# imkaywu/MVSKit

Hardware: AMD Instinct MI355X
Metric: patches/s (propagate+optim iteration), 12-view 1080p (higher is better)
Workload: dtype f32

## Files before the change

include/mvskit_engine.h:

```cpp
#ifndef MVSKIT_ENGINE_H
#define MVSKIT_ENGINE_H

#include <stddef.h>
#include <stdint.h>

#ifdef __cplusplus
extern "C" {
#endif

#ifndef MVS_MAX_IMAGES
#define MVS_MAX_IMAGES 32
#endif
#define MVS_LIST_CAP 16

typedef enum mvs_status {
    MVS_OK = 0,
    MVS_ERR_ARG = -1,
    MVS_ERR_STATE = -2,
    MVS_ERR_HIP = -3,
    MVS_ERR_CAPACITY = -4,
    MVS_ERR_NO_DEVICE = -5
} mvs_status;

typedef struct mvs_patch {
// ... 218 lines not shown
    int64_t neighbor_visited;
    int64_t neighbor_accepted;
    int64_t neighbor_retried;
    int64_t exchange_bytes;
} mvs_filter_stats;
int mvs_engine_filter_stats(mvs_engine* e, mvs_filter_stats* out);

int mvs_engine_pass(mvs_engine* e, int iter, int pass, mvs_counters* out);
int mvs_engine_export_counts(mvs_engine* e, int64_t* n_new, int64_t* n_kill, int32_t* per_view_new );
int mvs_engine_export_device(mvs_engine* e, void* d_new_records, int64_t cap_new, void* d_kill_ids, int64_t cap_kill);
int mvs_engine_commit_device(mvs_engine* e, const void* d_new_records, int64_t n_new, const void* d_kill_ids, int64_t n_kill);
int mvs_engine_commit_local(mvs_engine* e);

#define MVS_COMM_ID_BYTES 128
int mvs_comm_unique_id(void* id_out );
int mvs_engine_comm_init(mvs_engine* e, const void* id , int rank, int world);
int mvs_engine_comm_attach(mvs_engine* e, void* nccl_comm , int rank, int world);
int mvs_engine_comm_release(mvs_engine* e);
int mvs_engine_exchange(mvs_engine* e);
int mvs_engine_comm_info(mvs_engine* e, int* rank, int* world, int* comm_count, int* comm_rank);

int mvs_engine_depth_normal_map(mvs_engine* e, int view, int kind, float* depth, float* normal, int32_t* ids);

typedef enum mvs_probe_op {
    MVS_PROBE_NCC = 0,
    MVS_PROBE_PREPROCESS = 1,
    MVS_PROBE_REFINE = 2,
    MVS_PROBE_POSTPROCESS = 3,
    MVS_PROBE_COST = 4,
    MVS_PROBE_MATH = 5,
    MVS_PROBE_REFINE_X = 6
} mvs_probe_op;
int mvs_engine_probe(mvs_engine* e, int op, int64_t n, const mvs_patch* in_rec, const float* in_f,
                     mvs_patch* out_rec, float* out_f, int32_t* out_i);

typedef struct mvs_timing {
    float index_ms;
    float sweep_ms;
    float commit_ms;
    int32_t sweep_launches;
    float exchange_ms;
    int32_t sweep_jobs_listed;
    int64_t exchange_bytes;
    int64_t check_retried_cells;
} mvs_timing;
int mvs_engine_last_timing(mvs_engine* e, mvs_timing* t);

int mvs_engine_sweep_pairs(mvs_engine* e, int64_t out[6]);

int mvs_engine_sweep_repeats(mvs_engine* e, int64_t out[2]);

int mvs_engine_sweep_kernels(mvs_engine* e, int64_t out[2]);

#ifdef __cplusplus
}
#endif
#endif
```

mvskit_amd/csrc/mvs_device.cuh:

```cuda
#pragma once
#include <hip/hip_runtime.h>
#include <limits.h>
#include "mvs_types.h"

namespace mvsdev {

struct F3 { float x, y, z; };
struct F4 { float x, y, z, w; };

#define DEV __device__ __forceinline__

DEV int lane_id() { return (int)(threadIdx.x & 63u); }
DEV float fma_(float a, float b, float c) { return __builtin_fmaf(a, b, c); }
DEV int rli(int x, int l) { return __builtin_amdgcn_readlane(x, l); }
DEV float rlf(float x, int l) { return __int_as_float(__builtin_amdgcn_readlane(__float_as_int(x), l)); }
DEV int rfl(int x) { return __builtin_amdgcn_readfirstlane(x); }
DEV unsigned long long ballot(bool p) { return __ballot(p); }
#if MVS_LISTCAP > 32
typedef unsigned long long vmask_t;
DEV int vpop(vmask_t m) { return __popcll(m); }
#define MVS_VBITS 64
#else
typedef unsigned vmask_t;
DEV int vpop(vmask_t m) { return __popc(m); }
// ... 199 lines not shown
    const float fz = norm4(sub4(coord, ld4(vw->center)));
    const float ips = vw->ipscale;
    if (ips == 0.0f) return 1.0f;
    return div_rn(2.0f * fz * (float)(1 << prm.level), ips);
}
DEV void cell_of(const DParams& prm, const DView* vw, F4 coord, int& ix, int& iy) {
    float P[12];
    load_P(vw, prm.level, P);
    const F3 ic = project_regs(P, coord);
    ix = ((int)floorf(ic.x + 0.5f)) / prm.csize;
    iy = ((int)floorf(ic.y + 0.5f)) / prm.csize;
}
template <int LANE> DEV float row_bcast_f(float x) {
    return __int_as_float(__builtin_amdgcn_update_dpp(0, __float_as_int(x), 0x150 + LANE, 0xf, 0xf, false));
}
template <int LANE, int BANKS> DEV float row_bcast_banks_f(float old, float x) {
    return __int_as_float(__builtin_amdgcn_update_dpp(__float_as_int(old), __float_as_int(x), 0x150 + LANE, 0xf, BANKS, false));
}
template <int LANE, bool PAIR> DEV float half_bcast_f(float x) {
    if constexpr (PAIR) return row_bcast_banks_f<8 + LANE, 0xC>(row_bcast_banks_f<LANE, 0x3>(x, x), x);
    else return row_bcast_f<LANE>(x);
}
template <bool PAIR = false>
DEV void get_paxes(const DParams& prm, const DView* vw, F4 coord, F4 normal, F4& px, F4& py) {
    const F4 ctr = ld4(vw->center);
    const float ips = vw->ipscale;
    const F3 xax = ld3(vw->xaxis);
    float P[12];
    load_P(vw, prm.level, P);
    float pscale = 1.0f;
    if (ips != 0.0f) pscale = div_rn(2.0f * norm4(sub4(coord, ctr)) * (float)(1 << prm.level), ips);
    F3 n3{normal.x, normal.y, normal.z};
    F3 y3 = cross3(n3, xax);
    y3 = nrm3(y3);
    F3 x3 = cross3(y3, n3);
    px = {x3.x * pscale, x3.y * pscale, x3.z * pscale, 0.0f};
    py = {y3.x * pscale, y3.y * pscale, y3.z * pscale, 0.0f};
    const int j = lane_id() & (PAIR ? 7 : 15);
    const float a = j == 1 ? 1.0f : 0.0f, b = j == 2 ? 1.0f : 0.0f;
    const F4 X{fma_(b, py.x, fma_(a, px.x, coord.x)), fma_(b, py.y, fma_(a, px.y, coord.y)), fma_(b, py.z, fma_(a, px.z, coord.z)), coord.w};
    const F3 ic = project_regs(P, X);
    const F3 c0{half_bcast_f<0, PAIR>(ic.x), half_bcast_f<0, PAIR>(ic.y), half_bcast_f<0, PAIR>(ic.z)};
    const float inv = rcp_rn(norm3(sub3(ic, c0)));
    px = scl4(px, half_bcast_f<1, PAIR>(inv));
    py = scl4(py, half_bcast_f<2, PAIR>(inv));
}
DEV float robustincc(float incc) { return div_rn(incc, 1 + 3 * incc); }
DEV float unrobustincc(float r) { return div_rn(r, 1 - 3 * r); }

struct Frame {
    float tlx, tly, dxx, dxy, dyx, dyy;
    int w;
    int ok;
    unsigned img_lo, img_hi;
};
DEV int level_diff(const DParams& prm, float ratio) {
    static_assert(0x3504F3 == (0x3FB504F3 & 0x7FFFFF), "mantissa of 1.414213562373095f");
    const int k = ((__float_as_int(ratio) + (0x800000 - 0x3504F3)) >> 23) - 127;
    const int ld = max(-4, min(2, k));
    return max(-prm.level, min(2, ld));
}
DEV float pow2_level(int ld) { return __int_as_float((127 + ld) << 23); }
DEV Frame make_frame(const DParams& prm, F4 coord, F4 px, F4 py, F4 pz, int v, bool active) {
    const DView* vw = prm.views + (active ? v : 0);
    const F4 ctr = ld4(vw->center);
    float P[12];
#pragma unroll
    for (int k = 0; k < 12; ++k) P[k] = vw->P[prm.level][k];
    const int W0 = vw->W[0], H0 = vw->H[0];
    const unsigned long long base_level = (unsigned long long)vw->img[prm.level];
    const F4 ray = nrm4(sub4(ctr, coord));
    const float weight = fmaxf(0.0f, dot4(ray, pz));
    F3 center = project_regs(P, coord);
    F3 dx = sub3(project_regs(P, add4(coord, px)), center);
    F3 dy = sub3(project_regs(P, add4(coord, py)), center);
    const float ratio = (norm3(dx) + norm3(dy)) / 2.0f;
    const int ld = level_diff(prm, ratio);
    const float iscale = pow2_level(-ld);
    const int newLevel = prm.level + ld;
    const unsigned long long base_new = (unsigned long long)vw->img[newLevel];
    center = scl3(center, iscale);
    dx = scl3(dx, iscale);
    dy = scl3(dy, iscale);
    const float m = (float)(prm.wsize / 2);
    const float ax = dx.x * m, bx = dy.x * m, ay = dx.y * m, by = dy.y * m;
    const float tlx = (center.x - ax) - bx, tly = (center.y - ay) - by;
    const float minx = (center.x - fabsf(ax)) - fabsf(bx), maxx = (center.x + fabsf(ax)) + fabsf(bx);
    const float miny = (center.y - fabsf(ay)) - fabsf(by), maxy = (center.y + fabsf(ay)) + fabsf(by);
    const int margin2 = 2;
    const int W = W0 >> newLevel, H = H0 >> newLevel;
    const bool inside = !(minx < margin2 || W - 1 - margin2 <= maxx || miny < margin2 || H - 1 - margin2 <= maxy);
    const bool ok = active && !(weight < prm.cosAngle1) && inside;
    Frame f;
    f.tlx = ok ? tlx : 0.0f; f.tly = ok ? tly : 0.0f;
    f.dxx = ok ? dx.x : 0.0f; f.dxy = ok ? dx.y : 0.0f; f.dyx = ok ? dy.x : 0.0f; f.dyy = ok ? dy.y : 0.0f;
    f.w = ok ? W : (W0 >> prm.level);
    f.ok = ok ? 1 : 0;
    const unsigned long long a = ok ? base_new : base_level;
    f.img_lo = (unsigned)(a & 0xffffffffull); f.img_hi = (unsigned)(a >> 32);
    return f;
}

struct __attribute__((packed, aligned(4))) Texel2 { uint32_t a, b; };

struct ClsConst {
    unsigned cs[3];
    int fb;
    int xbase, nx;
    unsigned xcs;
};
struct ClsLayout { int njx, lim, xbase, nx; };
__host__ __device__ inline ClsLayout cls_layout(int wsz) {
    const int nj = wsz >> 4, rem = wsz & 15;
    return {nj + (rem > 1 ? 1 : 0), rem > 1 ? wsz : 16 * nj, 16 * nj, rem == 1 ? 1 : 0};
}
__host__ __device__ inline bool cls_full_window(int wsz) {
    const ClsLayout l = cls_layout(wsz);
    return l.njx >= 3 && l.lim >= 48 && l.nx == 1;
}
struct WaveCtx {
    int lane;
    ClsConst cc;
    unsigned evals, view_evals;
#ifdef MVS_STAGE_TIMING
    unsigned long long st_acc[8];
    unsigned long long st_t;
#endif
};
struct WaveCtxFull : WaveCtx {};
template <class WC> struct wc_full_window { static constexpr bool value = false; };
template <> struct wc_full_window<WaveCtxFull> { static constexpr bool value = true; };
#ifdef MVS_STAGE_TIMING
#define WC_T0(wc) { (wc).st_t = (unsigned long long)__builtin_amdgcn_s_memtime(); }
#define WC_ADD(wc, k) { const unsigned long long t1_ = (unsigned long long)__builtin_amdgcn_s_memtime(); (wc).st_acc[k] += t1_ - (wc).st_t; (wc).st_t = t1_; }
#else
#define WC_T0(wc)
#define WC_ADD(wc, k)
#endif

#define MVS_PIVOT_LDS4 192
#define MVS_FRAME_LDS_BYTES (64 * 48 + 16 * 16)
#define MVS_FRAME1_LDS_BYTES (48 * (MVS_LISTCAP > 16 ? MVS_LISTCAP : 16))
extern __shared__ float4 mvs_dyn_lds4[];
DEV void frames_publish(const WaveCtx& wc, const Frame& f, int nlanes) {
    __syncthreads();
    if (wc.lane < nlanes) {
        float4* d = mvs_dyn_lds4 + 3 * wc.lane;
        d[0] = make_float4(f.tlx, f.tly, f.dxx, f.dxy);
        d[1] = make_float4(f.dyx, f.dyy, __int_as_float(f.w), __int_as_float(f.ok));
        d[2] = make_float4(__int_as_float((int)f.img_lo), __int_as_float((int)f.img_hi), 0.0f, 0.0f);
    }
    __syncthreads();
}
DEV float inv_msd(const DParams& prm, float ssd) {
    float msd = sqrt_rn(ssd * prm.inv_3sz);
    if (msd == 0.0f) msd = 1.0f;
    return rcp_rn(msd);
}

struct ClsPend { Texel2 q0, q1; float dx1, dy1; };
DEV ClsConst make_cls(const DParams& prm, int lane) {
    ClsConst cc;
    const ClsLayout l = cls_layout(prm.wsz);
    const int row = lane >> 4, c = lane & 15;
    cc.fb = 16 * row;
#pragma unroll
    for (int j = 0; j < 3; ++j) {
        const int q = c + 16 * j;
        const bool valid = j < l.njx && q < l.lim;
        cc.cs[j] = valid ? (unsigned)(q % prm.wsize) | ((unsigned)(q / prm.wsize) << 8) | (1u << 16) : 0u;
    }
    cc.xbase = l.xbase; cc.nx = l.nx;
    cc.xcs = (unsigned)(l.xbase % prm.wsize) | ((unsigned)(l.xbase / prm.wsize) << 8) | (1u << 16);
    return cc;
}
DEV float cvt_ub0(unsigned x) { return (float)(x & 255u); }
DEV float cvt_ub1(unsigned x) { return (float)((x >> 8) & 255u); }
DEV float cvt_ub2(unsigned x) { return (float)((x >> 16) & 255u); }
DEV unsigned cls_opaque(unsigned x) { asm volatile("" : "+v"(x)); return x; }
struct ClsFrame { float tlx, tly, dxx, dxy, dyx, dyy; int w; unsigned long long base; };
DEV ClsFrame cls_frame(int fidx) {
    const float4* s = mvs_dyn_lds4 + 3 * fidx;
    const float4 A = s[0], B = s[1];
    const float2 Cc = *reinterpret_cast<const float2*>(s + 2);
    ClsFrame f;
    f.tlx = A.x; f.tly = A.y; f.dxx = A.z; f.dxy = A.w; f.dyx = B.x; f.dyy = B.y; f.w = __float_as_int(B.z);
    f.base = ((unsigned long long)(unsigned)__float_as_int(Cc.y) << 32) | (unsigned long long)(unsigned)__float_as_int(Cc.x);
    return f;
}
DEV ClsPend cls_issue(const ClsFrame& f, unsigned cs) {
    typedef const __attribute__((address_space(1))) uint32_t* GlobalTexels;
    const float fx = cvt_ub0(cs), fy = cvt_ub1(cs);
    const float sx = fma_(f.dyx, fy, fma_(f.dxx, fx, f.tlx));
    const float sy = fma_(f.dyy, fy, fma_(f.dxy, fx, f.tly));
    const int lx = (int)sx, ly = (int)sy;
    const unsigned long long a0 = f.base + 4ull * (unsigned long long)(unsigned)(ly * f.w + lx);
    const GlobalTexels t0 = (GlobalTexels)a0, t1 = (GlobalTexels)(a0 + 4ull * (unsigned long long)(unsigned)f.w);
    ClsPend p;
    p.q0.a = t0[0]; p.q0.b = t0[1];
    p.q1.a = t1[0]; p.q1.b = t1[1];
    p.dx1 = __builtin_amdgcn_fractf(sx); p.dy1 = __builtin_amdgcn_fractf(sy);
    return p;
}
template <bool FULL = false>
DEV void cls_colour(const ClsPend& p, unsigned cs, float pr, float pg, float pb, float& r, float& g, float& b) {
    const Texel2 q0 = p.q0, q1 = p.q1;
    const float fm = FULL ? 1.0f : cvt_ub2(cs);
    const float dx1 = FULL ? p.dx1 : p.dx1 * fm, dx0 = fm - dx1, dy1 = p.dy1, dy0 = 1.0f - dy1;
    const float f00 = dx0 * dy0, f01 = dx0 * dy1, f10 = dx1 * dy0, f11 = dx1 * dy1;
    r = fma_((float)(q1.b & 255u), f11, fma_((float)(q0.b & 255u), f10, fma_((float)(q1.a & 255u), f01, (float)(q0.a & 255u) * f00)));
    g = fma_((float)((q1.b >> 8) & 255u), f11, fma_((float)((q0.b >> 8) & 255u), f10, fma_((float)((q1.a >> 8) & 255u), f01, (float)((q0.a >> 8) & 255u) * f00)));
    b = fma_((float)((q1.b >> 16) & 255u), f11, fma_((float)((q0.b >> 16) & 255u), f10, fma_((float)((q1.a >> 16) & 255u), f01, (float)((q0.a >> 16) & 255u) * f00)));
    if (FULL) { r = r - pr; g = g - pg; b = b - pb; }
    else { r = fma_(-pr, fm, r); g = fma_(-pg, fm, g); b = fma_(-pb, fm, b); }
}
DEV float bperm_f(int addr, float x) { return __int_as_float(__builtin_amdgcn_ds_bpermute(addr, __float_as_int(x))); }
#define MVS_ROW_STEP(x, C) x = x + dpp_f<C>(x);
#define MVS_ROW_STEP5(C) { const float t0 = dpp0_f<C>(s1r), t1 = dpp0_f<C>(s1g), t2 = dpp0_f<C>(s1b), t3 = dpp0_f<C>(s2), t4 = dpp0_f<C>(s01); \
                           s1r = s1r + t0; s1g = s1g + t1; s1b = s1b + t2; s2 = s2 + t3; s01 = s01 + t4; }
#define MVS_ROW_STEP4(C) { const float t0 = dpp0_f<C>(s1r), t1 = dpp0_f<C>(s1g), t2 = dpp0_f<C>(s1b), t3 = dpp0_f<C>(s2); \
                           s1r = s1r + t0; s1g = s1g + t1; s1b = s1b + t2; s2 = s2 + t3; }
template <class WC>
DEV void eval_steps4(const DParams& prm, WC& wc, const ClsConst& cc, const Frame& f, int n, unsigned (&okm)[4], float& incc_l) {
    constexpr bool FULL = wc_full_window<WC>::value;
    const bool has_x = cc.nx > 0;
    frames_publish(wc, f, 64);
    const unsigned long long okb = ballot(f.ok != 0);
#pragma unroll
    for (int g = 0; g < 4; ++g) okm[g] = (unsigned)((okb >> (16 * g)) & 0xffffull);
#pragma unroll
    for (int g = 0; g < 4; ++g) wc.view_evals += (okm[g] & 1u) ? (unsigned)__popc(okm[g]) : 0u;
    const int fb = cc.fb;
    const int lc = wc.lane & 15;
    float c0[3][3];
    ClsPend pend[3];
    float P1r, P1g, P1b, P2, P01 = 0.0f;
    const int vlast = max(n - 1, 0);
    {
        const ClsFrame fr = cls_frame(fb);
#pragma unroll
        for (int j = 0; j < 3; ++j) pend[j] = cls_issue(fr, cls_opaque(cc.cs[j]));
    }
    {
        const float4 pv = mvs_dyn_lds4[MVS_PIVOT_LDS4];
        const ClsFrame fn = cls_frame(fb + min(1, vlast));
        float s1r = 0.0f, s1g = 0.0f, s1b = 0.0f, s2 = 0.0f;
#pragma unroll
        for (int j = 0; j < 3; ++j) {
            const unsigned cs = cls_opaque(cc.cs[j]);
            float r, g, b;
            cls_colour<FULL>(pend[j], cs, pv.x, pv.y, pv.z, r, g, b);
            pend[j] = cls_issue(fn, cs);
            c0[j][0] = r; c0[j][1] = g; c0[j][2] = b;
            s1r += r; s1g += g; s1b += b;
            s2 = fma_(r, r, s2); s2 = fma_(g, g, s2); s2 = fma_(b, b, s2);
        }
        MVS_ROW_STEP4(0xB1) MVS_ROW_STEP4(0x4E) MVS_ROW_STEP4(0x141) MVS_ROW_STEP4(0x140)
        P1r = s1r; P1g = s1g; P1b = s1b; P2 = s2;
    }
    for (int k = 1; k < n; ++k) {
        const float4 pv = mvs_dyn_lds4[MVS_PIVOT_LDS4 + k];
        const ClsFrame fn = cls_frame(fb + min(k + 1, vlast));
        float s1r = 0.0f, s1g = 0.0f, s1b = 0.0f, s2 = 0.0f, s01 = 0.0f;
#pragma unroll
        for (int j = 0; j < 3; ++j) {
            const unsigned cs = cls_opaque(cc.cs[j]);
            float r, g, b;
            cls_colour<FULL>(pend[j], cs, pv.x, pv.y, pv.z, r, g, b);
            pend[j] = cls_issue(fn, cs);
            s1r += r; s1g += g; s1b += b;
            s2 = fma_(r, r, s2); s2 = fma_(g, g, s2); s2 = fma_(b, b, s2);
            s01 = fma_(r, c0[j][0], s01); s01 = fma_(g, c0[j][1], s01); s01 = fma_(b, c0[j][2], s01);
        }
        MVS_ROW_STEP5(0xB1) MVS_ROW_STEP5(0x4E) MVS_ROW_STEP5(0x141) MVS_ROW_STEP5(0x140)
        if (lc == k) { P1r = s1r; P1g = s1g; P1b = s1b; P2 = s2; P01 = s01; }
    }
    const int a0 = (wc.lane & 48) << 2;
    if (has_x) {
        const float4 pv = mvs_dyn_lds4[MVS_PIVOT_LDS4 + lc];
        ClsFrame fr;
        fr.tlx = f.tlx; fr.tly = f.tly; fr.dxx = f.dxx; fr.dxy = f.dxy; fr.dyx = f.dyx; fr.dyy = f.dyy; fr.w = f.w;
        fr.base = ((unsigned long long)f.img_hi << 32) | (unsigned long long)f.img_lo;
        {
            const unsigned cs = cc.xcs;
            const ClsPend pe = cls_issue(fr, cs);
            float r, g, b;
            cls_colour<FULL>(pe, cs, pv.x, pv.y, pv.z, r, g, b);
            const float r0 = bperm_f(a0, r), g0 = bperm_f(a0, g), b0 = bperm_f(a0, b);
            P1r += r; P1g += g; P1b += b;
            P2 = fma_(r, r, P2); P2 = fma_(g, g, P2); P2 = fma_(b, b, P2);
            P01 = fma_(r, r0, P01); P01 = fma_(g, g0, P01); P01 = fma_(b, b0, P01);
        }
    }
    const float m_r = P1r * prm.inv_sz, m_g = P1g * prm.inv_sz, m_b = P1b * prm.inv_sz;
    const float ssd = fmaxf(P2 - fma_(P1b, m_b, fma_(P1g, m_g, P1r * m_r)), 0.0f);
    const float inv_l = inv_msd(prm, ssd);
    const float m0r = bperm_f(a0, m_r), m0g = bperm_f(a0, m_g), m0b = bperm_f(a0, m_b), inv0 = bperm_f(a0, inv_l);
    const float dot = P01 - fma_(P1b, m0b, fma_(P1g, m0g, P1r * m0r));
    incc_l = 1.0f - (dot * (inv0 * inv_l)) * prm.inv_3sz;
}

template <class WC>
DEV unsigned long long eval_steps4_pair(const DParams& prm, WC& wc, const ClsConst& cc, const Frame& f, int n0, int n1, unsigned (&okm)[2][4], float& incc_l) {
    constexpr bool FULL = wc_full_window<WC>::value;
    const bool has_x = FULL || cc.nx > 0;
    frames_publish(wc, f, 64);
    const unsigned long long okb = ballot(f.ok != 0);
#pragma unroll
    for (int g = 0; g < 4; ++g) { okm[0][g] = (unsigned)((okb >> (16 * g)) & 0xffull); okm[1][g] = (unsigned)((okb >> (16 * g + 8)) & 0xffull); }
#pragma unroll
    for (int g = 0; g < 4; ++g)
        wc.view_evals += ((okm[0][g] & 1u) ? (unsigned)__popc(okm[0][g]) : 0u) + ((okm[1][g] & 1u) ? (unsigned)__popc(okm[1][g]) : 0u);
    const int lc = wc.lane & 15;
    float P1r = 0.0f, P1g = 0.0f, P1b = 0.0f, P2 = 0.0f, P01 = 0.0f;
#pragma nounroll
    for (int s = 0; s < 2; ++s) {
        const int n = s ? n1 : n0;
        const int fb = cc.fb + 8 * s, pb = MVS_PIVOT_LDS4 + 8 * s, lb = 8 * s;
        float c0[3][3];
        ClsPend pend[3];
        const int vlast = max(n - 1, 0);
        {
            const ClsFrame fr = cls_frame(fb);
#pragma unroll
            for (int j = 0; j < 3; ++j) pend[j] = cls_issue(fr, cls_opaque(cc.cs[j]));
        }
        {
            const float4 pv = mvs_dyn_lds4[pb];
            const ClsFrame fn = cls_frame(fb + min(1, vlast));
            float s1r = 0.0f, s1g = 0.0f, s1b = 0.0f, s2 = 0.0f;
#pragma unroll
            for (int j = 0; j < 3; ++j) {
                const unsigned cs = cls_opaque(cc.cs[j]);
                float r, g, b;
                cls_colour<FULL>(pend[j], cs, pv.x, pv.y, pv.z, r, g, b);
                pend[j] = cls_issue(fn, cs);
                c0[j][0] = r; c0[j][1] = g; c0[j][2] = b;
                s1r += r; s1g += g; s1b += b;
                s2 = fma_(r, r, s2); s2 = fma_(g, g, s2); s2 = fma_(b, b, s2);
            }
            MVS_ROW_STEP4(0xB1) MVS_ROW_STEP4(0x4E) MVS_ROW_STEP4(0x141) MVS_ROW_STEP4(0x140)
            if (lc >= lb) { P1r = s1r; P1g = s1g; P1b = s1b; P2 = s2; }
        }
        for (int k = 1; k < n; ++k) {
            const float4 pv = mvs_dyn_lds4[pb + k];
            const ClsFrame fn = cls_frame(fb + min(k + 1, vlast));
            float s1r = 0.0f, s1g = 0.0f, s1b = 0.0f, s2 = 0.0f, s01 = 0.0f;
#pragma unroll
            for (int j = 0; j < 3; ++j) {
                const unsigned cs = cls_opaque(cc.cs[j]);
                float r, g, b;
                cls_colour<FULL>(pend[j], cs, pv.x, pv.y, pv.z, r, g, b);
                pend[j] = cls_issue(fn, cs);
                s1r += r; s1g += g; s1b += b;
                s2 = fma_(r, r, s2); s2 = fma_(g, g, s2); s2 = fma_(b, b, s2);
                s01 = fma_(r, c0[j][0], s01); s01 = fma_(g, c0[j][1], s01); s01 = fma_(b, c0[j][2], s01);
            }
            MVS_ROW_STEP5(0xB1) MVS_ROW_STEP5(0x4E) MVS_ROW_STEP5(0x141) MVS_ROW_STEP5(0x140)
            if (lc == lb + k) { P1r = s1r; P1g = s1g; P1b = s1b; P2 = s2; P01 = s01; }
        }
    }
    const int a0 = (wc.lane & 56) << 2;
    if (has_x) {
        const float4 pv = mvs_dyn_lds4[MVS_PIVOT_LDS4 + lc];
        ClsFrame fr;
        fr.tlx = f.tlx; fr.tly = f.tly; fr.dxx = f.dxx; fr.dxy = f.dxy; fr.dyx = f.dyx; fr.dyy = f.dyy; fr.w = f.w;
        fr.base = ((unsigned long long)f.img_hi << 32) | (unsigned long long)f.img_lo;
        {
            const unsigned cs = cc.xcs;
            const ClsPend pe = cls_issue(fr, cs);
            float r, g, b;
            cls_colour<FULL>(pe, cs, pv.x, pv.y, pv.z, r, g, b);
            const float r0 = bperm_f(a0, r), g0 = bperm_f(a0, g), b0 = bperm_f(a0, b);
            P1r += r; P1g += g; P1b += b;
            P2 = fma_(r, r, P2); P2 = fma_(g, g, P2); P2 = fma_(b, b, P2);
            P01 = fma_(r, r0, P01); P01 = fma_(g, g0, P01); P01 = fma_(b, b0, P01);
        }
    }
    const float m_r = P1r * prm.inv_sz, m_g = P1g * prm.inv_sz, m_b = P1b * prm.inv_sz;
    const float ssd = fmaxf(P2 - fma_(P1b, m_b, fma_(P1g, m_g, P1r * m_r)), 0.0f);
    const float inv_l = inv_msd(prm, ssd);
    const float m0r = bperm_f(a0, m_r), m0g = bperm_f(a0, m_g), m0b = bperm_f(a0, m_b), inv0 = bperm_f(a0, inv_l);
    const float dot = P01 - fma_(P1b, m0b, fma_(P1g, m0g, P1r * m0r));
    incc_l = 1.0f - (dot * (inv0 * inv_l)) * prm.inv_3sz;
    return okb;
}

template <bool FULL = false>
DEV void cls_raw(const ClsPend& p, unsigned cs, float& r, float& g, float& b) {
    const Texel2 q0 = p.q0, q1 = p.q1;
    const float fm = FULL ? 1.0f : cvt_ub2(cs);
    const float dx1 = FULL ? p.dx1 : p.dx1 * fm, dx0 = fm - dx1, dy1 = p.dy1, dy0 = 1.0f - dy1;
    const float f00 = dx0 * dy0, f01 = dx0 * dy1, f10 = dx1 * dy0, f11 = dx1 * dy1;
    r = fma_((float)(q1.b & 255u), f11, fma_((float)(q0.b & 255u), f10, fma_((float)(q1.a & 255u), f01, (float)(q0.a & 255u) * f00)));
    g = fma_((float)((q1.b >> 8) & 255u), f11, fma_((float)((q0.b >> 8) & 255u), f10, fma_((float)((q1.a >> 8) & 255u), f01, (float)((q0.a >> 8) & 255u) * f00)));
    b = fma_((float)((q1.b >> 16) & 255u), f11, fma_((float)((q0.b >> 16) & 255u), f10, fma_((float)((q1.a >> 16) & 255u), f01, (float)((q0.a >> 16) & 255u) * f00)));
}
#define MVS_ROW_STEP3(C) { const float t0 = dpp0_f<C>(s1r), t1 = dpp0_f<C>(s1g), t2 = dpp0_f<C>(s1b); s1r = s1r + t0; s1g = s1g + t1; s1b = s1b + t2; }
#define MVS_ROW_STEP2(C) { const float t0 = dpp0_f<C>(sq), t1 = dpp0_f<C>(dt); sq = sq + t0; dt = dt + t1; }

#define MVS_PAIR_MFMA (MVS_LISTCAP > 16)
#if MVS_PAIR_MFMA
#define MVS_GRAM_SCRATCH (MVS_LISTCAP > 32 ? 2 : 1)
#define MVS_GRAM_CH 16
#define MVS_GRAM_NCH (MVS_LISTCAP / 16)
#define MVS_GRAM_NT (MVS_GRAM_NCH * (MVS_GRAM_NCH + 1) / 2)
#define MVS_GRAM_KSP 40
#define MVS_GRAM_T(p, c) ((c) * ((c) + 1) / 2 + (p))
#define MVS_GRAM_KK 4
#define MVS_GRAM_KS ((147 + MVS_GRAM_KK - 1) / MVS_GRAM_KK)
#define MVS_GRAM_NACC 4
typedef float gram_acc_t __attribute__((ext_vector_type(MVS_GRAM_NACC)));
DEV gram_acc_t gram_mfma(float a, float b, gram_acc_t c) { return __builtin_amdgcn_mfma_f32_16x16x4f32(a, b, c, 0, 0, 0); }
DEV int gram_col(int lane) { return lane & 15; }
DEV int gram_row(int lane, int r) { return (lane >> 4) * 4 + r; }
template <int N> struct GramIC { static constexpr int value = N; };
#endif
template <bool PIV = false, class WC>
DEV void eval_views(const DParams& prm, WC& wc, const Frame& f, int n, vmask_t (&okm)[1], float& incc_l, float* piv = nullptr,
                    float* texs = nullptr, int tstride = 0, float* ssd_out = nullptr) {
#if MVS_PAIR_MFMA
#if MVS_GRAM_SCRATCH == 2
    float gops[MVS_GRAM_NCH * MVS_GRAM_KSP];
#elif MVS_GRAM_SCRATCH
    gram_acc_t gacc[MVS_GRAM_NT];
    float gops[(MVS_GRAM_NCH - 1) * MVS_GRAM_KSP];
#pragma unroll
    for (int q = 0; q < MVS_GRAM_NT; ++q)
#pragma unroll
        for (int r = 0; r < MVS_GRAM_NACC; ++r) gacc[q][r] = 0.0f;
#endif
    const int gK = 3 * prm.wsz, gtp = 3 * tstride;
    const int gk0 = wc.lane / MVS_GRAM_CH;
    const float* const grow = texs + (wc.lane & (MVS_GRAM_CH - 1)) * gtp;
#endif
    constexpr bool FULL = wc_full_window<WC>::value;
    const ClsConst& cc = wc.cc;
    const bool has_x = FULL || cc.nx > 0;
    frames_publish(wc, f, MVS_LISTCAP > 16 ? MVS_LISTCAP : 16);
    okm[0] = vballot(f.ok != 0);
    wc.view_evals += (okm[0] & 1u) ? (unsigned)vpop(okm[0]) : 0u;
    const int row = wc.lane >> 4, lc = wc.lane & 15;
    float fxr = 0.0f, fxg = 0.0f, fxb = 0.0f;
    unsigned xcs = 0u;
    ClsPend pe;
    if (has_x) {
        ClsFrame fr;
        fr.tlx = f.tlx; fr.tly = f.tly; fr.dxx = f.dxx; fr.dxy = f.dxy; fr.dyx = f.dyx; fr.dyy = f.dyy; fr.w = f.w;
        fr.base = ((unsigned long long)f.img_hi << 32) | (unsigned long long)f.img_lo;
        xcs = cc.xcs;
        pe = cls_issue(fr, xcs);
    }
    float d0[3][3], d0x[3] = {0.0f, 0.0f, 0.0f};
    float ssd_l = 1.0f, dot_l = 0.0f, mr_l = 128.0f, mg_l = 128.0f, mb_l = 128.0f;
    ClsPend pend[3];
    {
        const int last = max(n - 1, 0);
        const ClsFrame fr = cls_frame(min(row, last));
#pragma unroll
        for (int j = 0; j < 3; ++j) pend[j] = cls_issue(fr, cls_opaque(cc.cs[j]));
    }
    if (has_x) cls_raw<FULL>(pe, xcs, fxr, fxg, fxb);
    const int rounds = (n + 3) >> 2;
    auto round_body = [&](const int t) {
        const int v = 4 * t + row, vq = min(v, max(n - 1, 0));
        const ClsFrame fn = cls_frame(min(v + 4, max(n - 1, 0)));
        float cr[3], cg[3], cb[3];
        float s1r = 0.0f, s1g = 0.0f, s1b = 0.0f;
#pragma unroll
        for (int j = 0; j < 3; ++j) {
            const unsigned cs = cls_opaque(cc.cs[j]);
            cls_raw<FULL>(pend[j], cs, cr[j], cg[j], cb[j]);
            pend[j] = cls_issue(fn, cs);
            s1r += cr[j]; s1g += cg[j]; s1b += cb[j];
        }
        MVS_ROW_STEP3(0xB1) MVS_ROW_STEP3(0x4E) MVS_ROW_STEP3(0x141) MVS_ROW_STEP3(0x140)
        float xr = 0.0f, xg = 0.0f, xb = 0.0f;
        if (has_x) {
            xr = bperm_f(4 * vq, fxr); xg = bperm_f(4 * vq, fxg); xb = bperm_f(4 * vq, fxb);
            s1r += xr; s1g += xg; s1b += xb;
        }
        const float mr = s1r * prm.inv_sz, mg = s1g * prm.inv_sz, mb = s1b * prm.inv_sz;
        float er[3], eg[3], eb[3];
#pragma unroll
        for (int j = 0; j < 3; ++j) {
            if (FULL) { er[j] = cr[j] - mr; eg[j] = cg[j] - mg; eb[j] = cb[j] - mb; }
            else {
                const float fm = cvt_ub2(cls_opaque(cc.cs[j]));
                er[j] = fma_(-mr, fm, cr[j]); eg[j] = fma_(-mg, fm, cg[j]); eb[j] = fma_(-mb, fm, cb[j]);
            }
        }
        const float exr = xr - mr, exg = xg - mg, exb = xb - mb;
        if (t == 0) {
            const int a0 = 4 * lc;
#pragma unroll
            for (int j = 0; j < 3; ++j) { d0[j][0] = bperm_f(a0, er[j]); d0[j][1] = bperm_f(a0, eg[j]); d0[j][2] = bperm_f(a0, eb[j]); }
            if (has_x) { d0x[0] = bperm_f(0, exr); d0x[1] = bperm_f(0, exg); d0x[2] = bperm_f(0, exb); }
        }
        float sq = 0.0f, dt = 0.0f;
#pragma unroll
        for (int j = 0; j < 3; ++j) {
            sq += fma_(eb[j], eb[j], fma_(eg[j], eg[j], er[j] * er[j]));
            dt += fma_(d0[j][2], eb[j], fma_(d0[j][1], eg[j], d0[j][0] * er[j]));
        }
        MVS_ROW_STEP2(0xB1) MVS_ROW_STEP2(0x4E) MVS_ROW_STEP2(0x141) MVS_ROW_STEP2(0x140)
        if (has_x) {
            sq += fma_(exb, exb, fma_(exg, exg, exr * exr));
            dt += fma_(d0x[2], exb, fma_(d0x[1], exg, d0x[0] * exr));
        }
        if (lc == t) { ssd_l = sq; dot_l = dt; if (PIV) { mr_l = mr; mg_l = mg; mb_l = mb; } }
#if MVS_PAIR_MFMA
        if (texs) {
            float* tv = texs + (3 * (v & (MVS_GRAM_CH - 1))) * tstride;
            const bool have = v < n;
#pragma unroll
            for (int j = 0; j < 3; ++j)
                if (cc.cs[j] >> 16) { const int q = 3 * (lc + 16 * j); tv[q] = have ? er[j] : 0.0f; tv[q + 1] = have ? eg[j] : 0.0f; tv[q + 2] = have ? eb[j] : 0.0f; }
            if (has_x && lc == 0) { tv[3 * cc.xbase] = have ? exr : 0.0f; tv[3 * cc.xbase + 1] = have ? exg : 0.0f; tv[3 * cc.xbase + 2] = have ? exb : 0.0f; }
        }
#else
        if (texs && v < n) {
            float* tv = texs + (3 * v) * tstride;
#pragma unroll
            for (int j = 0; j < 3; ++j)
                if (cc.cs[j] >> 16) { const int q = 3 * (lc + 16 * j); tv[q] = er[j]; tv[q + 1] = eg[j]; tv[q + 2] = eb[j]; }
            if (has_x && lc == 0) { tv[3 * cc.xbase] = exr; tv[3 * cc.xbase + 1] = exg; tv[3 * cc.xbase + 2] = exb; }
// ... 126 lines not shown
        for (int t = 0; t < rounds; ++t) round_body(t);
#else
    for (int t = 0; t < rounds; ++t) round_body(t);
#endif
    const float inv_l = inv_msd(prm, ssd_l);
    const float inv0 = rlf(inv_l, 0);
    const float incc_v = 1.0f - (dot_l * (inv0 * inv_l)) * prm.inv_3sz;
    const int src = 4 * (16 * (wc.lane & 3) + ((wc.lane >> 2) & 15));
    incc_l = bperm_f(src, incc_v);
    if (ssd_out) *ssd_out = bperm_f(src, ssd_l);
    if (PIV) {
        const bool okk = (okm[0] >> (wc.lane & (MVS_VBITS - 1))) & 1u;
        const float a0 = bperm_f(src, mr_l), a1 = bperm_f(src, mg_l), a2 = bperm_f(src, mb_l);
        piv[0] = (wc.lane < MVS_VBITS && okk) ? a0 : 128.0f; piv[1] = (wc.lane < MVS_VBITS && okk) ? a1 : 128.0f; piv[2] = (wc.lane < MVS_VBITS && okk) ? a2 : 128.0f;
    }
}

struct Cand {
    F4 coord, normal;
    float ncc, dscale, ascale, tmp;
    int nimg, nvimg;
    int img, gx, gy;
    int vimg, vgx, vgy;
};

DEV float compute_weights(const DParams& prm, const WaveCtx& wc, F4 coord, F4 normal, int img, int n) {
    float unit = 1.0f;
    {
        const DView* vw = prm.views + (wc.lane < n ? img : 0);
        const F4 ctr = ld4(vw->center);
        const float ips = vw->ipscale;
        const F4 dc = sub4(coord, ctr);
        float u = 1.0f;
        if (ips != 0.0f) u = div_rn(2.0f * norm4(dc) * (float)(1 << prm.level), ips);
        const F4 ray = nrm4(sub4(ctr, coord));
        const float d = dot4(ray, normal);
        u = (0.0f < d) ? div_rn(u, d) : (float)(INT_MAX / 2);
        if (wc.lane < n) unit = u;
    }
    const float w0 = rlf(unit, 0);
    float w = fminf(1.0f, div_rn(w0, unit));
    if (wc.lane == 0) w = 1.0f;
    return w;
}

template <class WC>
DEV float compute_incc(const DParams& prm, WC& wc, F4 coord, F4 normal, int img, int n, float weights, int robust) {
    if (n < 2) return 2.0f;
    const int ref = rli(img, 0);
    F4 px, py;
    get_paxes(prm, prm.views + ref, coord, normal, px, py);
    const int sz = min(prm.tau, n);
    wc.evals++;
    const Frame f = make_frame(prm, coord, px, py, normal, img, wc.lane < sz);
    vmask_t okm[1];
    float incc_l;
    eval_views(prm, wc, f, sz, okm, incc_l);
    if (!(okm[0] & 1u)) return 2.0f;
    const float val_l = robust ? robustincc(incc_l) : incc_l;
    float score = 0.0f, total = 0.0f;
    for (int i = 1; i < sz; ++i) {
        if (!((okm[0] >> i) & 1u)) continue;
        const float w = rlf(weights, i);
        total += w;
        score += rlf(val_l, i) * w;
    }
    if (total == 0.0f) return 2.0f;
    return div_rn(score, total);
}
DEV float weighted_incc(const DParams& prm, vmask_t okm, float val_l, float weights, int n) {
    if (n < 2 || !(okm & 1u)) return 2.0f;
    const int sz = min(prm.tau, n);
    float score = 0.0f, total = 0.0f;
    for (int i = 1; i < sz; ++i) {
        if (!((okm >> i) & 1u)) continue;
        const float w = rlf(weights, i);
        total += w;
        score += rlf(val_l, i) * w;
    }
    if (total == 0.0f) return 2.0f;
    return div_rn(score, total);
}
template <class WC>
DEV float compute_ncc(const DParams& prm, WC& wc, F4 coord, F4 normal, int img, int n) {
    const float w = compute_weights(prm, wc, coord, normal, img, n);
    return 1.0f - unrobustincc(compute_incc(prm, wc, coord, normal, img, n, w, 1));
}

template <class WC>
DEV float set_inccs(const DParams& prm, WC& wc, F4 coord, F4 normal, int img, int n, int robust, vmask_t* okm_out = nullptr,
                    float* texs = nullptr, int tstride = 0, float* ssd_out = nullptr) {
    const int ref = rli(img, 0);
    F4 px, py;
    get_paxes(prm, prm.views + ref, coord, normal, px, py);
    wc.evals++;
    const Frame f = make_frame(prm, coord, px, py, normal, img, wc.lane < n);
    vmask_t okm[1];
    float incc_l;
    eval_views(prm, wc, f, n, okm, incc_l, nullptr, texs, tstride, ssd_out);
    if (okm_out) *okm_out = okm[0];
    if (!(okm[0] & 1u)) return 2.0f;
    float incc = robust ? robustincc(incc_l) : incc_l;
    if (wc.lane >= MVS_LISTCAP || !((okm[0] >> (wc.lane & (MVS_VBITS - 1))) & 1u)) incc = 2.0f;
    if (wc.lane == 0) incc = 0.0f;
    return incc;
}

DEV int compact1(int* scratch, const WaveCtx& wc, bool keep, int& a) {
    const unsigned long long m = ballot(keep);
    const int pos = __popcll(m & ((1ull << wc.lane) - 1ull));
    __syncthreads();
    if (keep) scratch[pos] = a;
    __syncthreads();
    a = scratch[wc.lane];
    return __popcll(m);
}

DEV void add_images(const DParams& prm, const WaveCtx& wc, int* scratch, Cand& c) {
    const int ref = rli(c.img, 0);
    bool visib = false;
    for (int j = 0; j < c.nimg; ++j) visib |= (rli(c.img, j) == wc.lane);
    bool q = false;
    if (wc.lane < prm.nviews && wc.lane != ref && !visib) {
        const DView* vw = prm.views + wc.lane;
        float P[12];
        load_P(vw, prm.level, P);
        const int W = vw->W[prm.level], H = vw->H[prm.level];
        const F4 ctr = ld4(vw->center);
        const F3 ic = project_regs(P, c.coord);
        const F4 ray = nrm4(sub4(ctr, c.coord));
        q = !(ic.x < 0.0f || W - 1 <= ic.x || ic.y < 0.0f || H - 1 <= ic.y) && prm.cosAngle0 <= dot4(ray, c.normal);
    }
    const unsigned long long m = ballot(q);
    const int pos = c.nimg + __popcll(m & ((1ull << wc.lane) - 1ull));
    __syncthreads();
    if (wc.lane < c.nimg) scratch[wc.lane] = c.img;
    if (q && pos < MVS_LISTCAP) scratch[pos] = wc.lane;
    __syncthreads();
    c.nimg = min(MVS_LISTCAP, c.nimg + (int)__popcll(m));
    c.img = scratch[wc.lane];
}

struct KeptTex {
    float* texs; int tstride;
    float ssd;
    vmask_t okm;
    int orig;
    int n_eval;
};
// ... 118 lines not shown
    if (cosb == 0.0f) a1 = 0.0f;
    else {
        const float sina = fx / cosb, cosa = -fz / cosb;
        a1 = pm_acosf(fmaxf(-1.0f, fminf(1.0f, cosa)));
        if (sina < 0.0f) a1 = -a1;
    }
    x[1] = a1 / rc.ascale;
    x[2] = a2 / rc.ascale;
}
DEV void decode(const DParams& prm, const RefineCtx& rc, float x0, float x1, float x2, F4& coord, F4& normal) {
    const float t = rc.dscale * x0;
    coord = {fma_(t, rc.ray.x, rc.center.x), fma_(t, rc.ray.y, rc.center.y), fma_(t, rc.ray.z, rc.center.z), fma_(t, rc.ray.w, rc.center.w)};
    const float angle1 = x1 * rc.ascale, angle2 = x2 * rc.ascale;
    float s1, c1, s2, c2;
    pm_sincosf(angle1, s1, c1);
    pm_sincosf(angle2, s2, c2);
    const float fx = s1 * c2, fy = s2, fz = -c1 * c2;
    const DView* vw = prm.views + rc.ref;
    normal = {fma_(vw->zaxis[0], fz, fma_(vw->yaxis[0], fy, vw->xaxis[0] * fx)),
              fma_(vw->zaxis[1], fz, fma_(vw->yaxis[1], fy, vw->xaxis[1] * fx)),
              fma_(vw->zaxis[2], fz, fma_(vw->yaxis[2], fy, vw->xaxis[2] * fx)), 0.0f};
}
DEV void sum_of_group(const WaveCtx& wc, unsigned okm, float val_l, int g, int sz, double& ans, int& denom) {
    ans = 0.0;
    denom = 0;
    for (int i = 1; i < sz; ++i) {
        if (!((okm >> i) & 1u)) continue;
        ans += (double)rlf(val_l, 16 * g + i);
        denom++;
    }
}
DEV double rld(double x, int l) {
    const long long b = __double_as_longlong(x);
    const unsigned lo = (unsigned)rli((int)(b & 0xffffffffll), l), hi = (unsigned)rli((int)(b >> 32), l);
    return __longlong_as_double((long long)(((unsigned long long)hi << 32) | lo));
}
DEV double cost_of_group(const DParams& prm, const WaveCtx& wc, unsigned okm, float val_l, int g, int sz, int minimum) {
    if (!(okm & 1u)) return 2.0;
    double ans;
    int denom;
    sum_of_group(wc, okm, val_l, g, sz, ans, denom);
    if (denom < minimum - 1) return 2.0;
    return ans / (double)denom;
}
template <class WC>
DEV void cost_func4(const DParams& prm, WC& wc, const RefineCtx& rc, int imgx, int n, bool four, float x0, float x1, float x2,
                    double (&fv)[4], float* piv = nullptr, const ClsConst* cc = nullptr, unsigned rows = 0xFu) {
    F4 coord, normal, px, py;
    decode(prm, rc, x0, x1, x2, coord, normal);
    get_paxes(prm, prm.views + rc.ref, coord, normal, px, py);
    const int sz = min(prm.tau, n);
    const int minimum = min(prm.minImageNum, sz);
    const int g = wc.lane >> 4, i = wc.lane & 15;
    const Frame f = make_frame(prm, coord, px, py, normal, imgx, (four ? ((rows >> g) & 1u) != 0u : g < 1) && i < sz);
    float incc_l;
    fv[1] = fv[2] = fv[3] = 2.0;
    if (four) {
        wc.evals += (unsigned)__popc(rows);
        unsigned okm[4];
        eval_steps4(prm, wc, *cc, f, sz, okm, incc_l);
        const float val_l = robustincc(incc_l);
        const int gl = wc.lane & 3;
        const unsigned okl = gl == 1 ? okm[1] : (gl == 2 ? okm[2] : (gl == 3 ? okm[3] : okm[0]));
        double num = 0.0;
        int den = 0;
        for (int i = 1; i < sz; ++i) {
            const float v = bperm_f(4 * (16 * gl + i), val_l);
            const bool ok = (okl >> i) & 1u;
            num = ok ? num + (double)v : num;
            den += ok ? 1 : 0;
        }
        const double q = num / (double)den;
#pragma unroll
        for (int j = 0; j < 4; ++j) fv[j] = ((okm[j] & 1u) && rli(den, j) >= minimum - 1) ? rld(q, j) : 2.0;
    } else {
        wc.evals += 1;
        vmask_t okm[1];
        if (piv) eval_views<true>(prm, wc, f, sz, okm, incc_l, piv);
        else eval_views(prm, wc, f, sz, okm, incc_l);
        const float val_l = robustincc(incc_l);
        fv[0] = cost_of_group(prm, wc, (unsigned)okm[0], val_l, 0, sz, minimum);
    }
}
template <class WC>
DEV void refine_patch(const DParams& prm, WC& wc, Cand& c, uint32_t k0, uint32_t k1, uint32_t k2, uint32_t k3, float* w_out = nullptr) {
    RefineCtx rc;
    rc.center = c.coord;
    rc.ref = rli(c.img, 0);
    rc.ray = nrm4(sub4(c.coord, ld4((prm.views + rc.ref)->center)));
    rc.dscale = c.dscale;
    rc.ascale = prm.ascaleConst;
    const float w = compute_weights(prm, wc, c.coord, c.normal, c.img, c.nimg);
    const int imgx = __shfl(c.img, wc.lane & 15);
    float x[3];
    encode(prm, rc, c.coord, c.normal, x);
    const float amin = -23.99999f, amax = 23.99999f;
    x[1] = fmaxf(fminf(x[1], amax), amin);
    x[2] = fmaxf(fminf(x[2], amax), amin);
    float bx0 = x[0], bx1 = x[1], bx2 = x[2];
    double fv[4];
    float piv[3] = {128.0f, 128.0f, 128.0f};
    cost_func4(prm, wc, rc, imgx, c.nimg, false, bx0, bx1, bx2, fv, piv);
    __syncthreads();
    if (wc.lane < 16) mvs_dyn_lds4[MVS_PIVOT_LDS4 + wc.lane] = make_float4(piv[0], piv[1], piv[2], 0.0f);
    __syncthreads();
    double fbest = fv[0];
    const ClsConst cc = wc.cc;
// ... 15 lines not shown
        }
        cost_func4(prm, wc, rc, imgx, c.nimg, true, cx0, cx1, cx2, fv, nullptr, &cc);
        int jb = 0;
        double fstep = fv[0];
#pragma unroll
        for (int j = 1; j < 4; ++j) if (fv[j] < fstep) { fstep = fv[j]; jb = j; }
        if (fstep < fbest) { fbest = fstep; bx0 = rlf(cx0, 16 * jb); bx1 = rlf(cx1, 16 * jb); bx2 = rlf(cx2, 16 * jb); }
        rd *= 0.5f; ra *= 0.5f;
    }
    x[0] = bx0; x[1] = bx1; x[2] = bx2;
    decode(prm, rc, x[0], x[1], x[2], c.coord, c.normal);
    c.normal.w = 0.0f;
    if (w_out) *w_out = w;
    else c.ncc = 1.0f - unrobustincc(compute_incc(prm, wc, c.coord, c.normal, c.img, c.nimg, w, 1));
}

#define MVS_PEND_IMG 16
#define MVS_PEND_GX 80
#define MVS_PEND_GY 144
#define MVS_PEND_W 208
#define MVS_PEND_CTX 272
#define MVS_PEND_XIMG 304
#define MVS_PEND_INTS 320
DEV float rff(float x) { return __int_as_float(rfl(__float_as_int(x))); }
DEV void pend_store(int* st, const WaveCtx& wc, const Cand& c, float w) {
    __syncthreads();
    if (wc.lane == 0) {
        float* f = reinterpret_cast<float*>(st);
        f[0] = c.coord.x; f[1] = c.coord.y; f[2] = c.coord.z; f[3] = c.coord.w;
        f[4] = c.normal.x; f[5] = c.normal.y; f[6] = c.normal.z; f[7] = c.normal.w;
        f[8] = c.ncc; f[9] = c.dscale; f[10] = c.ascale; f[11] = c.tmp;
        st[12] = c.nimg; st[13] = c.nvimg;
    }
    st[MVS_PEND_IMG + wc.lane] = c.img; st[MVS_PEND_GX + wc.lane] = c.gx; st[MVS_PEND_GY + wc.lane] = c.gy;
    st[MVS_PEND_W + wc.lane] = __float_as_int(w);
    __syncthreads();
}
DEV void pend_load(const int* st, const WaveCtx& wc, Cand& c, float& w) {
    const float* f = reinterpret_cast<const float*>(st);
    c.coord = {rff(f[0]), rff(f[1]), rff(f[2]), rff(f[3])};
    c.normal = {rff(f[4]), rff(f[5]), rff(f[6]), rff(f[7])};
    c.ncc = rff(f[8]); c.dscale = rff(f[9]); c.ascale = rff(f[10]); c.tmp = rff(f[11]);
    c.nimg = rfl(st[12]); c.nvimg = rfl(st[13]);
    c.img = st[MVS_PEND_IMG + wc.lane]; c.gx = st[MVS_PEND_GX + wc.lane]; c.gy = st[MVS_PEND_GY + wc.lane];
    c.vimg = 0; c.vgx = 0; c.vgy = 0;
    w = __int_as_float(st[MVS_PEND_W + wc.lane]);
}
template <class WC>
DEV void cost_func4_pair(const DParams& prm, WC& wc, const RefineCtx& rc, int imgx, int sz0, int sz1, int szl, float x0, float x1, float x2,
                         double (&fv)[2][4], const ClsConst& cc) {
    F4 coord, normal, px, py;
    decode(prm, rc, x0, x1, x2, coord, normal);
    get_paxes<true>(prm, prm.views + rc.ref, coord, normal, px, py);
    const Frame f = make_frame(prm, coord, px, py, normal, imgx, (wc.lane & 7) < szl);
    wc.evals += 8u;
    unsigned okm[2][4];
    float incc_l;
    const unsigned long long okb = eval_steps4_pair(prm, wc, cc, f, sz0, sz1, okm, incc_l);
    const float val_l = robustincc(incc_l);
    const int src = (int)(((cls_opaque((unsigned)wc.lane) & 3u) << 4) | ((cls_opaque((unsigned)wc.lane) & 4u) << 1));
    const unsigned okl = (unsigned)(okb >> src) & 0xffu;
    double num = 0.0;
    int den = 0;
    const int szm = max(sz0, sz1);
    for (int i = 1; i < szm; ++i) {
        const float v = bperm_f(4 * (src + i), val_l);
        const bool ok = (okl >> i) & 1u;
        num = ok ? num + (double)v : num;
        den += ok ? 1 : 0;
    }
    const double q = num / (double)den;
    const int min0 = min(prm.minImageNum, sz0), min1 = min(prm.minImageNum, sz1);
#pragma unroll
    for (int j = 0; j < 4; ++j) {
        fv[0][j] = ((okm[0][j] & 1u) && rli(den, j) >= min0 - 1) ? rld(q, j) : 2.0;
        fv[1][j] = ((okm[1][j] & 1u) && rli(den, 4 + j) >= min1 - 1) ? rld(q, 4 + j) : 2.0;
    }
}
template <class WC>
DEV void refine_patch_pair(const DParams& prm, WC& wc, int* st, Cand& c1, uint32_t k0, uint32_t k1, uint32_t k2, uint32_t k3a, uint32_t k3b, float& w1) {
    float* const ctx = reinterpret_cast<float*>(st + MVS_PEND_CTX);
    int* const ximg = st + MVS_PEND_XIMG;
    const float amin = -23.99999f, amax = 23.99999f;
    double fbest0 = 2.0, fbest1 = 2.0;
    int sz0 = 0, sz1 = 0;
    w1 = 0.0f;
#pragma nounroll
    for (int s = 0; s < 2; ++s) {
        F4 coord = c1.coord, normal = c1.normal;
        float dscale = c1.dscale;
        int img = c1.img, nimg = c1.nimg;
        if (s == 0) {
            const float* f = reinterpret_cast<const float*>(st);
            coord = {rff(f[0]), rff(f[1]), rff(f[2]), rff(f[3])};
            normal = {rff(f[4]), rff(f[5]), rff(f[6]), rff(f[7])};
            dscale = rff(f[9]); nimg = rfl(st[12]);
            img = st[MVS_PEND_IMG + wc.lane];
        }
        RefineCtx rc;
        rc.center = coord;
        rc.ref = rli(img, 0);
        rc.ray = nrm4(sub4(coord, ld4((prm.views + rc.ref)->center)));
        rc.dscale = dscale;
        rc.ascale = prm.ascaleConst;
        const float w = compute_weights(prm, wc, coord, normal, img, nimg);
        if (s == 0) st[MVS_PEND_W + wc.lane] = __float_as_int(w);
        else w1 = w;
// ... 179 lines not shown
        cost_func4(prm, wc, rc, imgx, c.nimg, true, vx0, vx1, vx2, fv, nullptr, &cc, 0xFu & ~(1u << b));
        evals += 3;
        if (g != b) vf = g == 0 ? fv[0] : (g == 1 ? fv[1] : (g == 2 ? fv[2] : fv[3]));
    }
    const float xb0 = rlf(vx0, 16 * b), xb1 = rlf(vx1, 16 * b), xb2 = rlf(vx2, 16 * b);
    if (x_out) { x_out[0] = xb0; x_out[1] = xb1; x_out[2] = xb2; }
    if (f_out) *f_out = rld(vf, 16 * b);
    if (ok) {
        decode(prm, rc, xb0, xb1, xb2, c.coord, c.normal);
        c.normal.w = 0.0f;
        if (!w_out) c.ncc = 1.0f - unrobustincc(compute_incc(prm, wc, c.coord, c.normal, c.img, c.nimg, w, 1));
    }
    if (w_out) *w_out = w;
    return ok ? evals : -evals;
}

DEV void filter_images_by_angle(const DParams& prm, const WaveCtx& wc, int* scratch, Cand& c, KeptTex* kt = nullptr) {
    bool bad = false;
    if (wc.lane < c.nimg) {
        const F4 ray = nrm4(sub4(ld4((prm.views + c.img)->center), c.coord));
        bad = dot4(ray, c.normal) < prm.cosAngle1;
    }
    const unsigned long long bm = ballot(bad);
    if (bm & 1ull) { c.nimg = 0; return; }
    if (kt) (void)compact1(scratch, wc, wc.lane < c.nimg && !bad, kt->orig);
    c.nimg = compact1(scratch, wc, wc.lane < c.nimg && !bad, c.img);
}
DEV void set_grids(const DParams& prm, const WaveCtx& wc, Cand& c) {
    c.gx = 0; c.gy = 0;
    if (wc.lane < c.nimg) cell_of(prm, prm.views + c.img, c.coord, c.gx, c.gy);
}
DEV int pair_index(int a, int b, int n) { return a * (2 * n - a - 1) / 2 + (b - a - 1); }
template <class WC>
DEV void set_ref_image(const DParams& prm, WC& wc, float* texs, int tstride, Cand& c, const KeptTex* kt = nullptr, const Frame* pre = nullptr) {
    if (c.nimg == 0) return;
    const int n = c.nimg;
    const int ref = rli(c.img, 0);
    WC_T0(wc)
    vmask_t okmask = 0;
    float ssd_l = 1.0f;
    int orig = wc.lane;
    if (kt) {
        texs = kt->texs;
        orig = wc.lane < n ? kt->orig : 0;
        ssd_l = __shfl(kt->ssd, orig);
        okmask = vballot(wc.lane < n && ((kt->okm >> orig) & 1u));
        __syncthreads();
    } else {
    Frame f;
    if (pre) f = *pre;
    else {
        F4 px, py;
        get_paxes(prm, prm.views + ref, c.coord, c.normal, px, py);
        f = make_frame(prm, c.coord, px, py, c.normal, c.img, wc.lane < n);
    }
    wc.evals++;
    WC_ADD(wc, 1)
    texs += MVS_FRAME1_LDS_BYTES / 4;
    vmask_t okm1[1];
    float incc_unused;
    eval_views(prm, wc, f, n, okm1, incc_unused, nullptr, texs, tstride, &ssd_l);
    okmask = okm1[0];
    if (!(okmask & 1u)) wc.view_evals += (unsigned)vpop(okmask);
    }
    const float inv_l = inv_msd(prm, ssd_l);
    WC_ADD(wc, 2)
    __syncthreads();
#if !MVS_PAIR_MFMA
    const int npairs = n * (n - 1) / 2;
    float* pairv = texs + prm.list_n * 3 * tstride;
#endif
#if MVS_PAIR_MFMA
    {
        const int MVS_GRAM_LD = prm.gram_ld;
        const int ne = kt ? kt->n_eval : n;
        const float inv_e = kt ? inv_msd(prm, kt->ssd) : inv_l;
        const vmask_t ok_e = kt ? kt->okm : okmask;
        const bool okb = wc.lane < ne && ((ok_e >> (wc.lane & (MVS_VBITS - 1))) & 1u);
        for (int a = 0; a + 1 < ne; ++a) {
            const float inva = rlf(inv_e, a);
            const bool oka = (ok_e >> a) & 1u;
            if (wc.lane > a && wc.lane < ne) {
                float val = robustincc(1.0f - (texs[a * MVS_GRAM_LD + wc.lane] * (inva * inv_e)) * prm.inv_3sz);
                if (!(oka && okb)) val = 2.0f;
                texs[a * MVS_GRAM_LD + wc.lane] = val;
                texs[wc.lane * MVS_GRAM_LD + a] = val;
            }
        }
    }
#else
    for (int r = 0; r * 64 < npairs; ++r) {
        const int q0 = wc.lane + 64 * r;
        int q = q0;
        const bool act = q < npairs;
        int a = 0;
        if (act) { while (q >= n - 1 - a) { q -= n - 1 - a; ++a; } }
        const int b = act ? a + 1 + q : 1;
        const float* ta = texs + (__shfl(orig, a) * 3) * tstride;
        const float* tb = texs + (__shfl(orig, b) * 3) * tstride;
        float acc = 0.0f;
        for (int i = 0; i < 3 * prm.wsz; i += 3) {
            acc = fma_(ta[i], tb[i], acc); acc = fma_(ta[i + 1], tb[i + 1], acc); acc = fma_(ta[i + 2], tb[i + 2], acc);
        }
        const float inva = __shfl(inv_l, a), invb = __shfl(inv_l, b);
        float val = robustincc(1.0f - (acc * (inva * invb)) * prm.inv_3sz);
        if (!(act && ((okmask >> a) & 1u) && ((okmask >> b) & 1u))) val = 2.0f;
        if (act) pairv[q0] = val;
// ... 178 lines not shown
```

mvskit_amd/csrc/mvs_engine.cpp:

```cpp
#include <dlfcn.h>

#include <cmath>
#include <cstring>

#include "mvs_engine_impl.h"

using namespace mvseng;

static_assert(sizeof(mvs_patch) == sizeof(DPatch), "mvs_patch and DPatch must be the same bytes");
static_assert((MVS_LISTCAP == 16 || MVS_LISTCAP == 32 || MVS_LISTCAP == 64) && MVS_LISTCAP <= MVS_MAXI && MVS_MAX_IMAGES == MVS_MAXI, "limits out of sync");

namespace mvseng {

thread_local std::string g_err;

Roctx& roctx() {
    static Roctx r;
    static bool tried = false;
    if (tried) return r;
    tried = true;
    void* h = nullptr;
    const char* names[] = {"libroctx64.so", "libroctx64.so.4", "/opt/rocm/lib/libroctx64.so.4"};
    for (const char* n : names) if (!h) h = dlopen(n, RTLD_NOW | RTLD_NOLOAD);
    for (const char* n : names) if (!h) h = dlopen(n, RTLD_NOW | RTLD_LOCAL);
    if (!h) return r;
    r.push = reinterpret_cast<int (*)(const char*)>(dlsym(h, "roctxRangePushA"));
    r.pop = reinterpret_cast<int (*)()>(dlsym(h, "roctxRangePop"));
    if (!r.push || !r.pop) { r.push = nullptr; r.pop = nullptr; }
    return r;
}

RefineSel refine_sel(const mvs_engine* e) {
    return RefineSel{e->refiner.mode == MVS_REFINE_CONVERGED ? 1 : 0, e->refiner.max_evals, e->refiner.xtol};
}

DParams current_params(mvs_engine* e) {
    DParams p = e->prm;
    p.views = e->dviews.p;
    p.pool = e->pool.p;
    p.pool_n = e->pool_n;
    p.total_cells = e->total_cells;
    p.csr_start = e->start.p; p.csr_cnt = e->cnt_alive.p; p.csr_key = e->key.p; p.csr_id32 = e->id32.p;
    p.vcsr_start = e->vstart.p; p.vcsr_cnt = e->vcnt_alive.p; p.vcsr_id32 = e->vid32.p;
    p.dpgrid = e->dpgrid.p;
    p.geo = e->geo_valid ? e->geo.p : nullptr;
    p.geo_ref = e->geo_valid ? e->geo_ref.p : nullptr;
    return p;
}

bool want_vgrid(const mvs_engine* e) { return e->prm.depth >= 2 && e->prm.enable_check; }

int need_state(const mvs_engine* e, Need need, const char* who) {
    if (!e) { g_err = std::string(who) + ": no engine"; return MVS_ERR_ARG; }
    if (need >= NEED_VIEWS && !e->have_views) { g_err = std::string(who) + ": views not set"; return MVS_ERR_STATE; }
    if (need >= NEED_IDLE && e->staged) { g_err = std::string(who) + ": a pass is waiting for its commit"; return MVS_ERR_STATE; }
    return MVS_OK;
}

int scan_total(mvs_engine* e, const int32_t* flags, int32_t* base, int32_t* scan, int64_t n, int64_t* count) {
    mvsk_exclusive_scan(flags, base, n, scan, e->stream);
    int32_t total = 0;
    if (int r = read_back(e, base + n, &total)) return r;
    HIPCHK(hipGetLastError());
    *count = total;
    return MVS_OK;
}

}

namespace {

void derive_params(mvs_engine* e) {
    const mvs_config& c = e->cfg;
    DParams& p = e->prm;
    p.nviews = c.nviews; p.level = c.level; p.csize = c.csize; p.wsize = c.wsize; p.wsz = c.wsize * c.wsize;
    p.minImageNum = c.minImageNum;
    p.tau = std::min(c.minImageNum * 2, c.nviews);
    p.max_propag = c.max_propag;
    p.cap = c.max_propag * c.csize * c.csize;
    p.depth = c.depth; p.enable_check = c.enable_check; p.view_propagation = c.view_propagation ? 1 : 0;
    p.seed = c.seed; p.refine_steps = c.refine_steps; p.rd0 = c.refine_rd0; p.ra0 = c.refine_ra0;
    p.nccThreshold = c.nccThreshold;
    p.nccThresholdBefore = c.nccThreshold - 0.3f;
    volatile float a0 = (float)(60.0f * M_PI / 180.0f), a1 = (float)(60.0f * M_PI / 180.0f);
    volatile double amin = (double)c.maxAngleThreshold, amax = (double)a1;
    volatile float typo = (float)(120.0f / M_PI * 180.0f);
    volatile double d120 = 120.0f * M_PI / 180.0f, d10 = 10.0f * M_PI / 180.0f;
    p.cosAngle0 = cosf(a0);
    p.cosAngle1 = cosf(a1);
    p.cosMinAngle = (float)cos(amin);
    p.cosMaxAngle = (float)cos(amax);
// ... 90 lines not shown
void mvs_default_config(mvs_config* c) {
    memset(c, 0, sizeof *c);
    c->level = 1; c->csize = 2; c->wsize = 7; c->minImageNum = 3; c->max_propag = 2;
    c->nccThreshold = 0.7f; c->maxAngleThreshold = (float)(10.0f * M_PI / 180.0f); c->quadThreshold = 2.5f;
    c->depth = 1; c->seed = 1; c->refine_steps = 6; c->refine_rd0 = 4.0f; c->refine_ra0 = 4.0f; c->enable_check = 1;
    c->view_begin = 0; c->view_stride = 1; c->device = 0; c->max_patches = 0;
}

int mvs_engine_create(const mvs_config* cfg, mvs_engine** out) {
    if (!cfg || !out) { g_err = "mvs_engine_create: null argument"; return MVS_ERR_ARG; }
    if (cfg->shard_count > 1 && (cfg->shard_index < 0 || cfg->shard_index >= cfg->shard_count)) { g_err = "mvs_engine_create: bad shard_index"; return MVS_ERR_ARG; }
    if (cfg->nviews < 1 || cfg->nviews > MVS_MAXVIEWS || cfg->wsize < 1 || cfg->wsize > 7 || cfg->csize < 1 || cfg->level < 0 ||
        cfg->level > 4 || cfg->max_propag < 1 || cfg->max_propag > 16 || cfg->max_propag * cfg->csize * cfg->csize > MVS_CAPMAX ||
        cfg->view_stride < 1 || cfg->view_begin < 0 || cfg->minImageNum < 1 ||
        std::min(cfg->minImageNum * 2, cfg->nviews) > 16 ) {
        g_err = "mvs_engine_create: configuration out of range (nviews <= 64, wsize <= 7, min(2 minImageNum, nviews) <= 16, max_propag*csize^2 <= 32)";
        return MVS_ERR_ARG;
    }
    int ndev = 0;
    if (hipGetDeviceCount(&ndev) != hipSuccess || ndev < 1) { g_err = "mvs_engine_create: no HIP device (the engine has no CPU path)"; return MVS_ERR_NO_DEVICE; }
    if (cfg->device < 0 || cfg->device >= ndev) { g_err = "mvs_engine_create: bad device ordinal"; return MVS_ERR_ARG; }
    HIPCHK(hipSetDevice(cfg->device));
    mvs_engine* e = new mvs_engine();
    e->cfg = *cfg;
    derive_params(e);
    hipError_t he = hipStreamCreate(&e->stream);
    if (he != hipSuccess) { g_err = std::string("hipStreamCreate: ") + hipGetErrorString(he); delete e; return MVS_ERR_HIP; }
    for (auto& ev : e->ev) (void)hipEventCreate(&ev);
    for (auto& ev : e->fev) (void)hipEventCreate(&ev);
    if (e->misc.ensure(misc::words) || e->counters.ensure(MVS_COUNTER_SLOTS) || e->error_flag.ensure(1)) { delete e; return MVS_ERR_HIP; }
    (void)hipMemset(e->misc.p, 0, misc::words * sizeof(unsigned long long));
    (void)hipMemset(e->error_flag.p, 0, sizeof(int32_t));
    *out = e;
    return MVS_OK;
}

int mvs_engine_destroy(mvs_engine* e) {
    if (!e) return MVS_OK;
    (void)hipSetDevice(e->cfg.device);
    (void)hipStreamSynchronize(e->stream);
    (void)mvs_engine_comm_release(e);
    for (auto& ev : e->ev) if (ev) (void)hipEventDestroy(ev);
    for (auto& ev : e->fev) if (ev) (void)hipEventDestroy(ev);
    (void)hipStreamDestroy(e->stream);
    delete e;
    return MVS_OK;
}

int mvs_engine_set_views(mvs_engine* e, int nviews, const mvs_view_desc* views) {
    if (!e || !views || nviews != e->cfg.nviews) { g_err = "mvs_engine_set_views: nviews must equal the configured number of views"; return MVS_ERR_ARG; }
    HIPCHK(hipSetDevice(e->cfg.device));
    hipStream_t st = e->stream;
    Range rg("mvs:set_views (upload + pyramids)");
    e->img_bufs.clear(); e->mask_bufs.clear();
    e->have_views = false;
    const int maxLevel = e->cfg.level + 3;
    e->hviews.assign(nviews, DView{});
    int cell_base = 0;
    size_t max_bytes = 0;
    for (int v = 0; v < nviews; ++v) {
        if (views[v].width < 8 || views[v].height < 8 || !views[v].rgb) { g_err = "mvs_engine_set_views: bad view"; return MVS_ERR_ARG; }
        max_bytes = std::max(max_bytes, (size_t)views[v].width * views[v].height * 3);
    }
    if (int r = e->tmp_bytes.ensure((int64_t)max_bytes)) return r;
    for (int v = 0; v < nviews; ++v) {
        DView& vw = e->hviews[v];
        vw.W[0] = views[v].width; vw.H[0] = views[v].height;
        for (int l = 1; l < maxLevel; ++l) { vw.W[l] = vw.W[l - 1] / 2; vw.H[l] = vw.H[l - 1] / 2; }
        setup_camera(e, vw, views[v].P);
        const size_t n0 = (size_t)vw.W[0] * vw.H[0];
        HIPCHK(hipMemcpyAsync(e->tmp_bytes.p, views[v].rgb, n0 * 3, hipMemcpyHostToDevice, st));
        for (int l = 0; l < maxLevel; ++l) {
            e->img_bufs.emplace_back();
            if (int r = e->img_bufs.back().ensure(std::max<int64_t>((int64_t)vw.W[l] * vw.H[l], 1))) return r;
            uint32_t* buf = e->img_bufs.back().p;
            vw.img[l] = buf;
            if (l == 0) mvsk_rgb_to_rgba(e->tmp_bytes.p, buf, (int64_t)n0, st);
            else mvsk_pyr_down(vw.img[l - 1], vw.W[l - 1], vw.H[l - 1], buf, vw.W[l], vw.H[l], st);
        }
        vw.mask = nullptr;
        if (views[v].mask) {
            HIPCHK(hipStreamSynchronize(st));
            uint8_t* prev = nullptr;
            for (int l = 0; l <= e->cfg.level; ++l) {
                e->mask_bufs.emplace_back();
                if (int r = e->mask_bufs.back().ensure(std::max<int64_t>((int64_t)vw.W[l] * vw.H[l], 1))) return r;
                uint8_t* m = e->mask_bufs.back().p;
                if (l == 0) {
                    HIPCHK(hipMemcpyAsync(m, views[v].mask, n0, hipMemcpyHostToDevice, st));
                    mvsk_mask_binarise(m, (int64_t)n0, st);
                } else mvsk_mask_down(prev, vw.W[l - 1], vw.H[l - 1], m, vw.W[l], vw.H[l], st);
                prev = m;
            }
            vw.mask = prev;
        }
        HIPCHK(hipStreamSynchronize(st));
        vw.gh = (vw.H[e->cfg.level] + e->cfg.csize - 1) / e->cfg.csize;
        vw.gw = (vw.W[e->cfg.level] + e->cfg.csize - 1) / e->cfg.csize;
        vw.cell_base = cell_base;
        cell_base += vw.gw * vw.gh;
    }
    e->total_cells = cell_base;
    if (int r = e->dviews.ensure(nviews)) return r;
    HIPCHK(hipMemcpyAsync(e->dviews.p, e->hviews.data(), sizeof(DView) * nviews, hipMemcpyHostToDevice, st));
    const int64_t nc = e->total_cells;
    if (e->cnt.ensure(nc + 2) || e->start.ensure(nc + 2) || e->cursor.ensure(nc + 2) || e->vcnt.ensure(nc + 2) || e->vstart.ensure(nc + 2) ||
        e->vcursor.ensure(nc + 2) || e->start_raw.ensure(nc + 2) || e->dpgrid.ensure(nc + 2) || e->best.ensure(nc + 2) || e->cnt_alive.ensure(nc + 2) || e->vcnt_alive.ensure(nc + 2))
        return MVS_ERR_HIP;
    int64_t pool_cap = e->cfg.max_patches > 0 ? e->cfg.max_patches : 4 * nc;
    if (e->cfg.max_patches <= 0) {
        size_t free_b = 0, total_b = 0;
        if (hipMemGetInfo(&free_b, &total_b) == hipSuccess && total_b > 0) {
            pool_cap = std::max<int64_t>(std::min<int64_t>(pool_cap, (int64_t)(total_b / 6 / sizeof(DPatch))), std::min<int64_t>(pool_cap, nc));
            const double per_patch = 2.5 * (double)sizeof(DPatch) + 17.0;
            const int64_t fit = (int64_t)(0.6 * (double)free_b / per_patch);
            if (fit < pool_cap) pool_cap = std::max<int64_t>(fit, std::min<int64_t>(pool_cap, nc / 4 + 1024));
        }
    }
    e->ids.headroom = e->key.headroom = e->id32.headroom = e->id32_raw.headroom = e->vid32.headroom = true;
    e->geo.headroom = e->geo_ref.headroom = true;
    if (e->pool.ensure(pool_cap) || e->pool_alt.ensure(pool_cap) || e->kill.ensure(pool_cap) || e->kill_cnt.ensure(pool_cap + 2) || e->kill_base.ensure(pool_cap + 2)) return MVS_ERR_HIP;
    HIPCHK(hipMemsetAsync(e->kill.p, 0, (size_t)pool_cap, st));
    int64_t njobs_max = 0;
    for (int v = 0; v < nviews; ++v) njobs_max += (int64_t)((e->hviews[v].gw + 1) / 2) * e->hviews[v].gh;
    const int maxstage = (e->prm.view_propagation ? 3 : 2) * e->prm.cap * e->prm.max_propag;
    if (e->job_stage.ensure(njobs_max * maxstage) || e->job_nstage.ensure(njobs_max + 2) || e->job_cnt.ensure(njobs_max + misc::job_list_pad) ||
        e->job_base_scan.ensure(njobs_max + misc::job_list_pad) || e->job_list.ensure(std::max<int64_t>(njobs_max, 16)))
        return MVS_ERR_HIP;
    const int64_t scan_n = std::max<int64_t>(std::max<int64_t>(nc, pool_cap), njobs_max);
// ... 88 lines not shown
        return MVS_OK;
    };
    if (take(e->ids, n + 16) || take(e->key, n + 16) || take(e->id32, n + 16) || take(e->id32_raw, n + 16) || take(e->vid32, n + 16)) return MVS_ERR_HIP;
    HIPCHK(hipStreamSynchronize(e->stream));
    return MVS_OK;
}

int mvs_engine_clear_patches(mvs_engine* e) {
    if (!e) return MVS_ERR_ARG;
    HIPCHK(hipSetDevice(e->cfg.device));
    if (e->kill.p) HIPCHK(hipMemsetAsync(e->kill.p, 0, (size_t)e->kill.cap, e->stream));
    e->pool_n = 0; e->staged = false; e->counted = false;
    return MVS_OK;
}

int mvs_engine_num_patches(mvs_engine* e, int64_t* n_alive) {
    if (!e || !n_alive) return MVS_ERR_ARG;
    HIPCHK(hipSetDevice(e->cfg.device));
    return count_pool(e, Count::alive, n_alive);
}

int mvs_engine_download_patches(mvs_engine* e, int64_t cap, mvs_patch* out, int64_t* n) {
    if (!e || !n) return MVS_ERR_ARG;
    int64_t alive = 0;
    if (int r = mvs_engine_num_patches(e, &alive)) return r;
    *n = alive;
    if (!out || alive == 0) return MVS_OK;
    const int64_t m = std::min(cap, alive);
    if (int r = e->tmp_rec_out.ensure(alive)) return r;
    mvsk_alive_gather(e->pool.p, e->pool_n, e->kill_base.p, e->tmp_rec_out.p, alive, e->stream);
    HIPCHK(hipMemcpyAsync(out, e->tmp_rec_out.p, (size_t)m * sizeof(mvs_patch), hipMemcpyDeviceToHost, e->stream));
    HIPCHK(hipStreamSynchronize(e->stream));
    return MVS_OK;
}

int mvs_engine_sweep_pairs(mvs_engine* e, int64_t out[6]) {
    if (!e || !out) return MVS_ERR_ARG;
    for (int k = 0; k < 6; ++k) out[k] = e->sweep_pairs[k];
    return MVS_OK;
}

int mvs_engine_sweep_repeats(mvs_engine* e, int64_t out[2]) {
    if (!e || !out) return MVS_ERR_ARG;
    for (int k = 0; k < 2; ++k) out[k] = e->sweep_repeats[k];
    return MVS_OK;
}

int mvs_engine_sweep_kernels(mvs_engine* e, int64_t out[2]) {
    if (!e || !out) return MVS_ERR_ARG;
    for (int k = 0; k < 2; ++k) out[k] = e->sweep_kernels[k];
    return MVS_OK;
}

int mvs_engine_last_timing(mvs_engine* e, mvs_timing* t) {
    if (!e || !t) return MVS_ERR_ARG;
    *t = e->timing;
    return MVS_OK;
}

int mvs_engine_depth_normal_map(mvs_engine* e, int view, int kind, float* depth, float* normal, int32_t* ids) {
    if (!e || !e->have_views || view < 0 || view >= e->cfg.nviews || kind < 0 || kind > 1) { g_err = "mvs_engine_depth_normal_map: bad argument"; return MVS_ERR_ARG; }
    HIPCHK(hipSetDevice(e->cfg.device));
    hipStream_t st = e->stream;
    const DView& vw = e->hviews[view];
    const int ncells = vw.gw * vw.gh;
    const DParams p = current_params(e);
    const unsigned long long* sel = nullptr;
    if (kind == 0) {
        HIPCHK(hipMemsetAsync(e->dpgrid.p, 0xff, (size_t)e->total_cells * sizeof(unsigned long long), st));
        mvsk_depth_maps(p, e->dpgrid.p, nullptr, st);
        sel = e->dpgrid.p + vw.cell_base;
    } else {
        HIPCHK(hipMemsetAsync(e->best.p, 0, (size_t)ncells * sizeof(unsigned long long), st));
        mvsk_best_ncc_map(p, view, e->best.p, st);
        sel = e->best.p;
    }
    if (e->tmp_f_out.ensure((int64_t)ncells * 4) || e->tmp_i.ensure(ncells)) return MVS_ERR_HIP;
    mvsk_map_extract(p, view, kind, sel, e->tmp_f_out.p, e->tmp_f_out.p + ncells, e->tmp_i.p, ncells, st);
    if (depth) HIPCHK(hipMemcpyAsync(depth, e->tmp_f_out.p, (size_t)ncells * sizeof(float), hipMemcpyDeviceToHost, st));
    if (normal) HIPCHK(hipMemcpyAsync(normal, e->tmp_f_out.p + ncells, (size_t)ncells * 3 * sizeof(float), hipMemcpyDeviceToHost, st));
    if (ids) HIPCHK(hipMemcpyAsync(ids, e->tmp_i.p, (size_t)ncells * sizeof(int32_t), hipMemcpyDeviceToHost, st));
    HIPCHK(hipStreamSynchronize(st));
    return MVS_OK;
}

int mvs_engine_probe(mvs_engine* e, int op, int64_t n, const mvs_patch* in_rec, const float* in_f, mvs_patch* out_rec, float* out_f, int32_t* out_i) {
    if (!e || !e->have_views || n < 0 || op < 0 || op > 6) { g_err = "mvs_engine_probe: bad argument / views not set"; return MVS_ERR_ARG; }
    const RefineSel rs = refine_sel(e);
    if (op == MVS_PROBE_REFINE_X && !rs.simplex) { g_err = "mvs_engine_probe: MVS_PROBE_REFINE_X needs the CONVERGED refiner"; return MVS_ERR_STATE; }
    if (n == 0) return MVS_OK;
    HIPCHK(hipSetDevice(e->cfg.device));
    hipStream_t st = e->stream;
    if (op == MVS_PROBE_POSTPROCESS && e->prm.depth > 0) if (int r = build_index(e, nullptr)) return r;
    const int64_t nf_out = op == MVS_PROBE_MATH ? 5 * n : ((op == MVS_PROBE_REFINE || op == MVS_PROBE_REFINE_X) && rs.simplex ? 4 * n : n);
    if (e->tmp_rec_in.ensure(n) || e->tmp_rec_out.ensure(n) || e->tmp_f_in.ensure(n) || e->tmp_f_out.ensure(nf_out) || e->tmp_i.ensure(n + 1)) return MVS_ERR_HIP;
    if (op == MVS_PROBE_MATH) {
        if (!in_f || !out_f) return MVS_ERR_ARG;
        HIPCHK(hipMemcpyAsync(e->tmp_f_in.p, in_f, (size_t)n * sizeof(float), hipMemcpyHostToDevice, st));
    } else {
        if (!in_rec) return MVS_ERR_ARG;
        HIPCHK(hipMemcpyAsync(e->tmp_rec_in.p, in_rec, (size_t)n * sizeof(mvs_patch), hipMemcpyHostToDevice, st));
    }
    HIPCHK(hipMemsetAsync(e->tmp_i.p, 0, (size_t)(n + 1) * sizeof(int32_t), st));
    const DParams p = current_params(e);
    mvsk_probe(p, op, n, e->tmp_rec_in.p, e->tmp_f_in.p, e->tmp_rec_out.p, e->tmp_f_out.p, e->tmp_i.p, rs, st);
    if (out_rec && (op == MVS_PROBE_PREPROCESS || op == MVS_PROBE_REFINE || op == MVS_PROBE_POSTPROCESS || op == MVS_PROBE_REFINE_X))
        HIPCHK(hipMemcpyAsync(out_rec, e->tmp_rec_out.p, (size_t)n * sizeof(mvs_patch), hipMemcpyDeviceToHost, st));
    if (out_f && (op == MVS_PROBE_NCC || op == MVS_PROBE_COST || op == MVS_PROBE_MATH || op == MVS_PROBE_REFINE_X))
        HIPCHK(hipMemcpyAsync(out_f, e->tmp_f_out.p, (size_t)nf_out * sizeof(float), hipMemcpyDeviceToHost, st));
    if (out_i) HIPCHK(hipMemcpyAsync(out_i, e->tmp_i.p, (size_t)n * sizeof(int32_t), hipMemcpyDeviceToHost, st));
    HIPCHK(hipStreamSynchronize(st));
    HIPCHK(hipGetLastError());
    return MVS_OK;
}

}
```

mvskit_amd/csrc/mvs_engine_impl.h:

```cpp
#pragma once
#include <hip/hip_runtime.h>
#include <rccl/rccl.h>

#include <algorithm>
#include <cstdint>
#include <string>
#include <vector>

#include "mvskit_engine.h"
#include "mvs_kernels.h"
#include "mvs_types.h"

namespace mvseng {
extern thread_local std::string g_err;
}

#define HIPCHK(expr)                                                                                       \
    do {                                                                                                   \
        hipError_t _e = (expr);                                                                            \
        if (_e != hipSuccess) {                                                                            \
            mvseng::g_err = std::string(#expr) + ": " + hipGetErrorString(_e);                             \
            return MVS_ERR_HIP;                                                                            \
        }                                                                                                  \
    } while (0)
// ... 44 lines not shown
constexpr int sweep_cursor_words = MVS_SWEEP_QUEUES * MVS_SWEEP_CURSOR_STRIDE * (int)sizeof(uint32_t) / (int)sizeof(unsigned long long);
constexpr int sweep_list_bounds = sweep_cursors + sweep_cursor_words;
constexpr int sweep_list_bound_words = (MVS_SWEEP_QUEUES + 1 + 1) / 2;
constexpr int words = sweep_list_bounds + sweep_list_bound_words;
constexpr int64_t job_list_pad = 1024 + 2;
}
namespace fstat {
constexpr int neighbor_parts = 0;
constexpr int neighbor_cycles = 4096;
constexpr int exact_evals = 4112;
constexpr int words = exact_evals + 2048;
}

struct Rccl {
    void* h = nullptr;
    ncclResult_t (*GetUniqueId)(ncclUniqueId*) = nullptr;
    ncclResult_t (*CommInitRank)(ncclComm_t*, int, ncclUniqueId, int) = nullptr;
    ncclResult_t (*CommDestroy)(ncclComm_t) = nullptr;
    ncclResult_t (*CommCount)(const ncclComm_t, int*) = nullptr;
    ncclResult_t (*CommUserRank)(const ncclComm_t, int*) = nullptr;
    ncclResult_t (*AllGather)(const void*, void*, size_t, ncclDataType_t, ncclComm_t, hipStream_t) = nullptr;
    ncclResult_t (*Broadcast)(const void*, void*, size_t, ncclDataType_t, int, ncclComm_t, hipStream_t) = nullptr;
    ncclResult_t (*GroupStart)() = nullptr;
    ncclResult_t (*GroupEnd)() = nullptr;
    const char* (*GetErrorString)(ncclResult_t) = nullptr;
    bool ok = false;
};
Rccl& rccl();

struct Roctx {
    int (*push)(const char*) = nullptr;
    int (*pop)() = nullptr;
};
Roctx& roctx();
struct Range {
    bool on;
    explicit Range(const char* name) : on(roctx().push != nullptr) { if (on) roctx().push(name); }
    ~Range() { if (on) roctx().pop(); }
    Range(const Range&) = delete;
    Range& operator=(const Range&) = delete;
};

}

using mvseng::DevBuf;
struct mvs_engine {
    mvs_config cfg{};
    mvs_refiner refiner{MVS_REFINE_HALVING, 500, 1e-4f};
    DParams prm{};
    hipStream_t stream = nullptr;
    bool have_views = false;
    std::vector<DView> hviews;
    DevBuf<DView> dviews;
    std::vector<DevBuf<uint32_t>> img_bufs;
    std::vector<DevBuf<uint8_t>> mask_bufs;
    int total_cells = 0;
    DevBuf<DPatch> pool, pool_alt;
    DevBuf<uint8_t> kill;
    int64_t pool_n = 0;
    bool ncc_dirty = false;
    DevBuf<int32_t> cnt, cursor, vcnt, vcursor;
    DevBuf<csr_off_t> start, vstart;
    DevBuf<csr_off_t> start_raw;
    DevBuf<int32_t> id32_raw;
    DevBuf<int64_t> scan_tmp;
    DevBuf<unsigned long long> ids;
    DevBuf<ListKey> key;
    DevBuf<int32_t> id32, vid32;
    DevBuf<int32_t> uf_parent, uf_size;
    DevBuf<int32_t> group_edges;
    DevBuf<int32_t> cnt_alive, vcnt_alive;
    DevBuf<unsigned long long> dpgrid, best;
    DevBuf<uint32_t> dirty;
    bool dirty_marked = false;
    DevBuf<float4> geo;
    DevBuf<uint8_t> geo_ref;
    bool geo_valid = false;
    bool lists_dense[2] = {false, false};
    DevBuf<DPatch> staging;
    DevBuf<int32_t> job_stage, job_nstage, job_cnt, job_base_scan, kill_cnt, kill_base;
    DevBuf<unsigned long long> misc;
    DevBuf<DCounters> counters;
    DevBuf<int32_t> error_flag;
    DevBuf<int32_t> big_tables, retry_jobs;
    DevBuf<int32_t> job_list;
    int64_t sweep_pairs[6] = {0, 0, 0, 0, 0, 0};
    int64_t sweep_repeats[2] = {0, 0};
    int64_t sweep_kernels[2] = {0, 0};
    int64_t retried_cells = 0;
    int64_t pass_retried = 0;
    SweepArgs sa{};
    bool staged = false;
    bool counted = false;
    int64_t n_new = 0, n_kill = 0;
    std::vector<int32_t> h_per_view;
    DevBuf<DPatch> tmp_rec_in, tmp_rec_out;
    DevBuf<float> tmp_f_in, tmp_f_out;
    DevBuf<int32_t> tmp_i;
    DevBuf<uint8_t> tmp_bytes;
    hipEvent_t ev[6] = {nullptr, nullptr, nullptr, nullptr, nullptr, nullptr};
    mvs_timing timing{};
    mvs_filter_stats fstats{};
    int64_t fstats_exchange_bytes = 0;
    DevBuf<unsigned long long> fstat_buf;
    hipEvent_t fev[10] = {nullptr, nullptr, nullptr, nullptr, nullptr, nullptr, nullptr, nullptr, nullptr, nullptr};
    ncclComm_t comm = nullptr;
    bool comm_owned = false;
    int comm_rank = 0, comm_world = 1;
    DevBuf<int64_t> comm_counts;
    DevBuf<int32_t> comm_kill_ids;
    int pass_status = MVS_OK;
    std::string pass_error;
    bool fault_fired = false;
};

namespace mvseng {

RefineSel refine_sel(const mvs_engine* e);
DParams current_params(mvs_engine* e);
bool want_vgrid(const mvs_engine* e);
enum Need { NEED_ENGINE, NEED_VIEWS, NEED_IDLE };
int need_state(const mvs_engine* e, Need need, const char* who);
int scan_total(mvs_engine* e, const int32_t* flags, int32_t* base, int32_t* scan, int64_t n, int64_t* count);

int build_list(mvs_engine* e, bool vgrid, bool trim, bool unordered = false);
int build_depth(mvs_engine* e);
int build_index(mvs_engine* e, unsigned long long* trimmed_out);
enum class Count { alive, kills, apply_kills };
int count_pool(mvs_engine* e, Count what, int64_t* total);
int ensure_counts(mvs_engine* e);
int compact_pool(mvs_engine* e);
void discard_pass(mvs_engine* e);

template <typename T> int read_back(mvs_engine* e, const T* dev, T* host) {
    HIPCHK(hipMemcpyAsync(host, dev, sizeof(T), hipMemcpyDeviceToHost, e->stream));
    HIPCHK(hipStreamSynchronize(e->stream));
    return MVS_OK;
}

template <typename Apply> int commit_pool(mvs_engine* e, Apply&& apply) {
    hipStream_t st = e->stream;
// ... 27 lines not shown
```

mvskit_amd/csrc/mvs_engine_pass.cpp:

```cpp
#include <climits>
#include <cstdio>
#include <cstdlib>
#include <cstring>

#include "mvs_engine_impl.h"

using namespace mvseng;

namespace mvseng {

int build_list(mvs_engine* e, bool vgrid, bool trim, bool unordered) {
    hipStream_t st = e->stream;
    const int64_t nc = e->total_cells;
    DParams p = current_params(e);
    DevBuf<int32_t>& cnt = vgrid ? e->vcnt : e->cnt;
    DevBuf<csr_off_t>& start = vgrid ? e->vstart : e->start;
    DevBuf<int32_t>& cursor = vgrid ? e->vcursor : e->cursor;
    DevBuf<unsigned long long>& ids = e->ids;
    DevBuf<int32_t>& id32 = vgrid ? e->vid32 : e->id32;
    DevBuf<int32_t>& cnt_alive = vgrid ? e->vcnt_alive : e->cnt_alive;
    HIPCHK(hipMemsetAsync(cnt.p, 0, (size_t)(nc + 1) * sizeof(int32_t), st));
    mvsk_index_count(p, vgrid ? nullptr : cnt.p, vgrid ? cnt.p : nullptr, nullptr, st);
    const bool direct = unordered && !trim;
    DevBuf<csr_off_t>& raw = e->start_raw;
// ... 151 lines not shown
        std::vector<int32_t> cuts(N + 1, -1);
        int64_t total_work = 0;
        if (split_mode > 0 && nj > 0) {
            const DParams p0 = current_params(e);
            int shift = 0;
            while ((((int64_t)3 * e->prm.cap * e->prm.max_propag * 32 * nj) >> shift) + nj >= (int64_t)INT32_MAX) ++shift;
            mvsk_job_work(p0, a, split_mode, shift, e->job_cnt.p, st);
            mvsk_exclusive_scan(e->job_cnt.p, e->job_base_scan.p, nj, reinterpret_cast<int32_t*>(e->scan_tmp.p), st);
            if (int r = e->tmp_i.ensure(N + 1)) return r;
            HIPCHK(hipMemsetAsync(e->tmp_i.p, 0xff, (size_t)(N + 1) * sizeof(int32_t), st));
            mvsk_job_cuts(e->job_base_scan.p, nj, N, e->tmp_i.p, st);
            int32_t tw = 0;
            HIPCHK(hipMemcpyAsync(cuts.data(), e->tmp_i.p, (size_t)(N + 1) * sizeof(int32_t), hipMemcpyDeviceToHost, st));
            HIPCHK(hipMemcpyAsync(&tw, e->job_base_scan.p + nj, sizeof tw, hipMemcpyDeviceToHost, st));
            HIPCHK(hipStreamSynchronize(st));
            total_work = tw;
        }
        cuts[0] = 0; cuts[N] = (int32_t)nj;
        for (int r = 1; r < N; ++r) {
            if (total_work <= 0 || cuts[r] < 0) cuts[r] = (int32_t)(nj * r / N);
            cuts[r] = std::max(cuts[r], cuts[r - 1]);
        }
        a.job_lo = cuts[R];
        a.job_hi = cuts[R + 1];
    }
    a.staging = e->staging.p; a.staging_cap = e->staging.cap;
    a.stage_counter = e->misc.p + misc::stage_counter;
    a.job_stage = e->job_stage.p; a.job_nstage = e->job_nstage.p;
    a.maxstage = (e->prm.view_propagation ? 3 : 2) * e->prm.cap * e->prm.max_propag;
    a.kill = e->kill.p;
    a.counters = e->counters.p;
    a.error_flag = e->error_flag.p;
    if (want_vgrid(e)) {
        if (int r = e->big_tables.ensure((int64_t)256 * 16384)) return r;
        if (int r = e->retry_jobs.ensure(std::max<int64_t>(nj, 16))) return r;
    }
    a.big_tables = e->big_tables.p; a.retry_jobs = e->retry_jobs.p; a.nretry = reinterpret_cast<int32_t*>(e->misc.p + misc::sweep_retry);
    HIPCHK(hipMemsetAsync(e->misc.p + misc::sweep_retry, 0, sizeof(unsigned long long), st));
    HIPCHK(hipMemsetAsync(e->misc.p + misc::stage_counter, 0, sizeof(unsigned long long), st));
    a.cursors = reinterpret_cast<uint32_t*>(e->misc.p + misc::sweep_cursors);
    HIPCHK(hipMemsetAsync(e->misc.p + misc::sweep_cursors, 0, (misc::sweep_cursor_words + misc::sweep_list_bound_words) * sizeof(unsigned long long), st));
    HIPCHK(hipMemsetAsync(e->counters.p, 0, MVS_COUNTER_SLOTS * sizeof(DCounters), st));
    HIPCHK(hipMemsetAsync(e->error_flag.p, 0, sizeof(int32_t), st));
    const DParams p = current_params(e);
    const RefineSel rs = refine_sel(e);
    if (int r = e->job_list.ensure(std::max<int64_t>(nj, 16))) return r;
    if (e->job_cnt.ensure(nj + misc::job_list_pad) || e->job_base_scan.ensure(nj + misc::job_list_pad)) return MVS_ERR_HIP;
    int32_t* list_bounds = reinterpret_cast<int32_t*>(e->misc.p + misc::sweep_list_bounds);
    a.job_list = e->job_list.p; a.list_bounds = list_bounds;
    mvsk_job_list(p, a, e->job_cnt.p, e->job_base_scan.p, reinterpret_cast<int32_t*>(e->scan_tmp.p), e->job_list.p, list_bounds, st);
    HIPCHK(hipEventRecord(e->ev[1], st));
    Range rg_sweep(pass & 1 ? "mvs:sweep colour 1" : "mvs:sweep colour 0");
    const int sweep_kernel = mvsk_sweep(p, a, rs, st);
    if (sweep_kernel >= 0) e->sweep_kernels[sweep_kernel] += 1;
    e->pass_retried = 0;
    if (want_vgrid(e)) {
        int32_t nretry = 0;
        if (int r = read_back(e, a.nretry, &nretry)) return r;
        e->pass_retried = nretry;
        if (nretry > 0) { mvsk_sweep_retry(p, a, nretry, rs, st); e->retried_cells += nretry; }
    }
    HIPCHK(hipEventRecord(e->ev[2], st));
    std::vector<DCounters> hcs(MVS_COUNTER_SLOTS);
    int32_t herr = 0;
    unsigned long long fill[2] = {0, 0};
    HIPCHK(hipMemcpyAsync(fill, e->misc.p + misc::fill_evals, sizeof fill, hipMemcpyDeviceToHost, st));
    HIPCHK(hipMemcpyAsync(hcs.data(), e->counters.p, hcs.size() * sizeof(DCounters), hipMemcpyDeviceToHost, st));
    HIPCHK(hipMemcpyAsync(&herr, e->error_flag.p, sizeof herr, hipMemcpyDeviceToHost, st));
    int32_t hbounds[MVS_SWEEP_QUEUES + 1];
    HIPCHK(hipMemcpyAsync(hbounds, list_bounds, sizeof hbounds, hipMemcpyDeviceToHost, st));
    HIPCHK(hipStreamSynchronize(st));
    HIPCHK(hipGetLastError());
    mvs_counters sum{};
    for (const DCounters& c : hcs) {
        add_counters(sum, c);
        for (int k = 0; k < 6; ++k) e->sweep_pairs[k] += (int64_t)c.pair[k];
        for (int k = 0; k < 2; ++k) e->sweep_repeats[k] += (int64_t)c.repeats[k];
    }
    sum.evals += fill[0]; sum.view_evals += fill[1]; sum.trimmed = (int64_t)trimmed;
    float ms = 0.0f;
    (void)hipEventElapsedTime(&ms, e->ev[0], e->ev[1]); e->timing.index_ms = ms;
    (void)hipEventElapsedTime(&ms, e->ev[1], e->ev[2]); e->timing.sweep_ms = ms;
    e->timing.commit_ms = 0.0f; e->timing.sweep_launches = 1; e->timing.exchange_ms = 0.0f; e->timing.exchange_bytes = 0;
    e->timing.check_retried_cells = e->pass_retried;
    e->timing.sweep_jobs_listed = hbounds[MVS_SWEEP_QUEUES];
    e->staged = true; e->counted = false;
    if (out) *out = sum;
#ifdef MVS_JOBLIST_COUNTS
    fprintf(stderr, "[job list] iter %d colour %d: jobs %lld, with any source entry %llu, listed %llu\n", iter, pass & 1, (long long)(a.job_hi - a.job_lo),
            hcs[0].stage[0], hcs[0].stage[1]);
#endif
#ifdef MVS_STAGE_TIMING
    {
        unsigned long long stage[16] = {0};
        for (const DCounters& c : hcs)
            for (int k = 0; k < 16; ++k) stage[k] = (k == 12 || k == 13) ? std::max(stage[k], c.stage[k]) : stage[k] + c.stage[k];
        static const char* nm[8] = {"wave", "generate", "pre", "refine", "post", "check", "stage", "prologue"};
        fprintf(stderr, "[stage cycles]");
        for (int k = 0; k < 8; ++k) fprintf(stderr, " %s %.1f%%", nm[k], 100.0 * (double)stage[k] / (double)(stage[0] ? stage[0] : 1));
        static const char* nm2[4] = {"gain", "search", "sort", "quad"};
        for (int k = 0; k < 4; ++k) fprintf(stderr, " %s %.1f%%", nm2[k], 100.0 * (double)stage[8 + k] / (double)(stage[0] ? stage[0] : 1));
        fprintf(stderr, " setRefImage pairs %.1f%% choice %.1f%%", 100.0 * (double)stage[14] / (double)(stage[0] ? stage[0] : 1), 100.0 * (double)stage[15] / (double)(stage[0] ? stage[0] : 1));
        fprintf(stderr, "  (wave cycles %.3e; max visited %llu, max neighbours %llu)\n", (double)stage[0], stage[12], stage[13]);
    }
#endif
#ifdef MVS_FAULT_INJECTION
    if (const char* f = getenv("MVS_FAULT_PASS")) {
// ... 92 lines not shown
```

mvskit_amd/csrc/mvs_kernels.h:

```cpp
#pragma once
#include <hip/hip_runtime.h>
#include "mvs_types.h"

void mvsk_rgb_to_rgba(const uint8_t* rgb, uint32_t* out, int64_t n, hipStream_t st);
void mvsk_rgba_to_rgb(const uint32_t* in, uint8_t* rgb, int64_t n, hipStream_t st);
void mvsk_pyr_down(const uint32_t* src, int pw, int ph, uint32_t* dst, int w, int h, hipStream_t st);
void mvsk_mask_down(const uint8_t* src, int pw, int ph, uint8_t* dst, int w, int h, hipStream_t st);
void mvsk_mask_binarise(uint8_t* m, int64_t n, hipStream_t st);
void mvsk_exclusive_scan(const int32_t* in, int32_t* out, int64_t n, int32_t* tmp, hipStream_t st);
void mvsk_index_count(const DParams& prm, int32_t* cnt, int32_t* vcnt, unsigned long long* total, hipStream_t st);
void mvsk_exclusive_scan_off(const int32_t* in, csr_off_t* out, int64_t n, csr_off_t* tmp, hipStream_t st);
void mvsk_index_fill(const DParams& prm, int vgrid, const csr_off_t* start, int32_t* cursor, unsigned long long* ids, hipStream_t st);
void mvsk_index_fill_direct(const DParams& prm, int vgrid, const csr_off_t* start, int32_t* cursor, int32_t* id32, hipStream_t st);
void mvsk_index_sort_trim(const DParams& prm, const csr_off_t* start, unsigned long long* ids, int do_trim, unsigned long long* trimmed, hipStream_t st);
void mvsk_index_finalize(const DParams& prm, int vgrid, const csr_off_t* start, unsigned long long* ids, int32_t* id32, int32_t* cnt_alive, hipStream_t st);
void mvsk_index_pack(const DParams& prm, const csr_off_t* start, const csr_off_t* start2, const int32_t* cnt_alive, const unsigned long long* ids, const int32_t* id32_in,
                     ListKey* key, int32_t* id32_out, hipStream_t st);
void mvsk_depth_maps(const DParams& prm, unsigned long long* dp, const uint32_t* dirty, hipStream_t st);
void mvsk_depth_mark_dirty(const DParams& prm, const uint8_t* kill, unsigned long long* dp, uint32_t* dirty, hipStream_t st);
void mvsk_best_ncc_map(const DParams& prm, int view, unsigned long long* best, hipStream_t st);
void mvsk_map_extract(const DParams& prm, int view, int kind, const unsigned long long* sel, float* depth, float* normal, int32_t* ids, int ncells, hipStream_t st);
void mvsk_fill_ncc(const DParams& prm, unsigned long long* evals, hipStream_t st);
struct RefineSel { int simplex; int max_evals; float xtol; };
size_t mvsk_sweep_lds_bytes(const DParams& prm);
int mvsk_sweep(const DParams& prm, const SweepArgs& a, const RefineSel& rs, hipStream_t st);
void mvsk_sweep_retry(const DParams& prm, const SweepArgs& a, int nretry, const RefineSel& rs, hipStream_t st);
void mvsk_job_work(const DParams& prm, const SweepArgs& a, int mode, int shift, int32_t* work, hipStream_t st);
int mvsk_job_list_seg(const SweepArgs& a);
void mvsk_job_list(const DParams& prm, const SweepArgs& a, int32_t* flags, int32_t* scan, int32_t* scan_tmp, int32_t* list, int32_t* bounds, hipStream_t st);
void mvsk_job_cuts(const int32_t* scan, int64_t njobs, int n, int32_t* cuts, hipStream_t st);
void mvsk_commit_count(const SweepArgs& a, int32_t* cnt, hipStream_t st);
void mvsk_commit_copy(const SweepArgs& a, const int32_t* base, DPatch* dst, int64_t dst_cap, int32_t* per_view, int keep_key, hipStream_t st);
void mvsk_kill_count(const uint8_t* kill, int64_t n, int32_t* cnt, hipStream_t st);
void mvsk_kill_export(const uint8_t* kill, int64_t n, const int32_t* base, int32_t* ids, int64_t cap, hipStream_t st);
void mvsk_apply_kill_flags(DPatch* pool, uint8_t* kill, int64_t n, hipStream_t st);
void mvsk_apply_kill_ids(DPatch* pool, const int32_t* ids, int64_t n, int64_t pool_n, hipStream_t st);
void mvsk_append_records(DPatch* pool, int64_t pool_n, const DPatch* recs, int64_t n, hipStream_t st);
void mvsk_alive_count(const DPatch* pool, int64_t n, int32_t* cnt, hipStream_t st);
void mvsk_alive_gather(const DPatch* pool, int64_t n, const int32_t* base, DPatch* out, int64_t cap, hipStream_t st);
void mvsk_filter_vimages(const DParams& prm, int additive, int64_t first, int64_t last, const uint32_t* dirty, hipStream_t st);
void mvsk_geo_pack(const DPatch* pool, int64_t n, float4* geo, uint8_t* ref, int* bad, hipStream_t st);
void mvsk_filter_outside(const DParams& prm, uint8_t* kill, int64_t first, int64_t last, hipStream_t st);
void mvsk_filter_exact(const DParams& prm, uint8_t* kill, unsigned long long* evals, unsigned long long* stage, int64_t first, int64_t last, hipStream_t st);
void mvsk_filter_neighbor(const DParams& prm, uint8_t* kill, int32_t* retry, int32_t* nretry, int32_t* overflow, unsigned long long* stats, int64_t first, int64_t last, hipStream_t st);
void mvsk_filter_neighbor_retry(const DParams& prm, uint8_t* kill, const int32_t* todo, int32_t ntodo, int32_t* overflow, unsigned long long* stats, hipStream_t st);
void mvsk_groups(const DParams& prm, int* parent, int* size, int threshold, uint8_t* kill, hipStream_t st);
void mvsk_groups_literal_edges(const DParams& prm, int* parent, int* size, int* edges2, int* nedges, int cap, hipStream_t st);
void mvsk_gather_i32(const int32_t* src, const int32_t* idx, int32_t* out, int64_t n, hipStream_t st);
void mvsk_scatter_i32(int32_t* dst, const int32_t* idx, const int32_t* val, int64_t n, hipStream_t st);
void mvsk_groups_kill(const DParams& prm, const int* parent, const int* size, int threshold, uint8_t* kill, hipStream_t st);
void mvsk_probe(const DParams& prm, int op, int64_t n, const DPatch* in, const float* in_f, DPatch* out, float* out_f, int32_t* out_i, const RefineSel& rs,
                hipStream_t st);
void mvsk_ply_select(const DPatch* pool, const int32_t* base, int64_t i0, int64_t i1, int32_t* idx, hipStream_t st);
void mvsk_ply_colour(const DPatch* pool, const int32_t* idx, int64_t n, const DView* views, int nviews, int level, int ascii, uint32_t* rgb, int32_t* len,
                     hipStream_t st);
void mvsk_ply_emit(const DPatch* pool, const int32_t* idx, int64_t n, const uint32_t* rgb, const int64_t* off, uint8_t* out, hipStream_t st);
struct SeedView { float P[12]; int32_t W, H, view; };
struct SeedCam { float center[4]; float ipscale; };
void mvsk_seed_accumulate(const SeedView& sv, const float* map, const uint8_t* mask, const float* xyz, int64_t n, float* sum, unsigned long long* bits,
                          hipStream_t st);
void mvsk_seed_flags(const SeedCam* cams, int level, const float* xyz, const float* sum, const unsigned long long* bits, int64_t n, int32_t* keep,
                     hipStream_t st);
void mvsk_seed_emit(const SeedCam* cams, int nviews, int level, float thr, float tmp_unit, const float* xyz, const float* sum, const unsigned long long* bits,
                    const int32_t* keep, const int32_t* base, int64_t n, DPatch* dst, hipStream_t st);
struct SeedRandomArgs { SeedChainArgs chain; uint32_t seed; float max_tilt; int32_t view; float dmin, dmax; };
size_t mvsk_texs_lds_bytes(const DParams& prm);
void mvsk_seed_random_hypotheses(const DParams& prm, const SeedRandomArgs& a, int64_t ncells, const int32_t* cells, DPatch* out, hipStream_t st);
void mvsk_seed_random(const DParams& prm, const SeedRandomArgs& a, int ncells, DPatch* stage, int32_t* keep, hipStream_t st);
void mvsk_seed_gather(const DPatch* stage, const int32_t* keep, const int32_t* base, int n, DPatch* dst, int32_t id0, hipStream_t st);
void mvsk_seed_points_hypotheses(const DParams& prm, int K, int64_t n, const float* xyz, DPatch* out, int32_t* count, hipStream_t st);
void mvsk_seed_points(const DParams& prm, const SeedPointsArgs& a, const float* xyz, DPatch* stage, int32_t* keep, hipStream_t st);
void mvsk_depth_ranges(const DParams& prm, int64_t n, const float* xyz, uint32_t* lo, uint32_t* hi, unsigned long long* cnt, hipStream_t st);
struct MapsArgs { int64_t pix_base[MVS_MAXVIEWS + 1]; float depth_tol, normal_cos; };
void mvsk_maps_select(const DParams& prm, unsigned long long* sel, hipStream_t st);
void mvsk_maps_render(const DParams& prm, int view, int W, int H, int source, const unsigned long long* sel, int32_t* ids, float* pts, hipStream_t st);
void mvsk_maps_agree(const DParams& prm, const MapsArgs& a, int view, int64_t npix, const int32_t* ids, const float* pts, unsigned long long* agree,
                     float* depth, float* normal, float* conf, hipStream_t st);
void mvsk_maps_flag(int64_t npix, int view, const int32_t* ids, const unsigned long long* agree, int min_consistent, int dedupe, int32_t* flag,
                    uint8_t* flag8, hipStream_t st);
void mvsk_maps_expand(int64_t npix, const uint8_t* flag8, int32_t* flag, hipStream_t st);
void mvsk_maps_gather(const DParams& prm, int view, int64_t npix, const int32_t* ids, const float* pts, const int32_t* flag, const int32_t* base,
                      void* out, int64_t cap, hipStream_t st);
struct MeshVol { float origin[3]; float voxel; int32_t nx, ny, nz; float trunc; int32_t min_count; };
inline int64_t mesh_npoints(const MeshVol& vol) { return (int64_t)vol.nx * vol.ny * vol.nz; }
void mvsk_mesh_tsdf(const DParams& prm, const MapsArgs& a, const MeshVol& vol, const int32_t* ids, const uint8_t* usable, float* tsdf, int32_t* count,
                    hipStream_t st);
void mvsk_mesh_state(const MeshVol& vol, const float* tsdf, const int32_t* count, uint8_t* state, hipStream_t st);
void mvsk_mesh_edges(const MeshVol& vol, const uint8_t* state, uint8_t* mask, int32_t* cnt, hipStream_t st);
void mvsk_mesh_verts(const MeshVol& vol, const float* tsdf, const uint8_t* mask, const int32_t* vbase, float* verts, int64_t cap_v, hipStream_t st);
void mvsk_mesh_tcount(const MeshVol& vol, const uint8_t* state, int32_t* cnt, hipStream_t st);
void mvsk_mesh_tris(const MeshVol& vol, const uint8_t* state, const uint8_t* mask, const int32_t* vbase, const int64_t* tbase, int32_t* tris,
                    int64_t cap_t, hipStream_t st);
void mvsk_mesh_normals_scan(int64_t n_v, const float* verts, int64_t n_t, const int32_t* tris, uint32_t* mbits, uint32_t* bad, hipStream_t st);
void mvsk_mesh_normals_accum(const float* verts, int64_t n_t, const int32_t* tris, const uint32_t* mbits, long long* acc, hipStream_t st);
void mvsk_mesh_normals_finish(int64_t n_v, const long long* acc, float* normals, hipStream_t st);
struct MeshColourArgs { float occl_tol, min_cos; };
void mvsk_mesh_colours(const DParams& prm, const MapsArgs& a, const MeshColourArgs& m, int64_t n_v, const float* verts, const float* normals,
                       const int32_t* ids, const uint8_t* usable, uint8_t* rgb, uint8_t* used, hipStream_t st);
void mvsk_mesh_check_ids(int64_t n_v, int64_t n_t, const int32_t* tris, uint32_t* bad, hipStream_t st);
void mvsk_mesh_components(int64_t n_v, int64_t n_t, const int32_t* tris, int32_t* parent, int32_t* size, unsigned long long* ncomp, hipStream_t st);
void mvsk_mesh_largest(int64_t n_v, const int32_t* parent, const int32_t* size, unsigned long long* best, hipStream_t st);
void mvsk_mesh_keep(int64_t n_t, const int32_t* tris, const int32_t* parent, const int32_t* size, int64_t min_triangles, int largest_only,
                    const unsigned long long* best, int32_t* tflag, int32_t* vflag, hipStream_t st);
void mvsk_mesh_gather(int64_t n_v, const float* verts, int32_t* vflag, const int32_t* vbase, float* out_verts, int64_t cap_v, int64_t n_t, const int32_t* tris,
// ... 15 lines not shown
```

mvskit_amd/csrc/mvs_kernels.hip:

```cpp
#include <hip/hip_runtime.h>
#include <algorithm>
#include "mvs_device.cuh"
#include "mvs_check.cuh"
#include "mvs_kernels.h"

using namespace mvsdev;

__global__ void k_rgb_to_rgba(const uint8_t* __restrict__ rgb, uint32_t* __restrict__ out, int64_t n) {
    const int64_t i = (int64_t)blockIdx.x * blockDim.x + threadIdx.x;
    if (i >= n) return;
    const uint8_t* p = rgb + 3 * i;
    out[i] = (uint32_t)p[0] | ((uint32_t)p[1] << 8) | ((uint32_t)p[2] << 16);
}
__global__ void k_rgba_to_rgb(const uint32_t* __restrict__ in, uint8_t* __restrict__ rgb, int64_t n) {
    const int64_t i = (int64_t)blockIdx.x * blockDim.x + threadIdx.x;
    if (i >= n) return;
    const uint32_t t = in[i];
    rgb[3 * i] = t & 255u; rgb[3 * i + 1] = (t >> 8) & 255u; rgb[3 * i + 2] = (t >> 16) & 255u;
}
__global__ void k_pyr_down(const uint32_t* __restrict__ src, int pw, int ph, uint32_t* __restrict__ dst, int w, int h) {
    const int x = blockIdx.x * blockDim.x + threadIdx.x, y = blockIdx.y * blockDim.y + threadIdx.y;
    if (x >= w || y >= h) return;
    const float base[4] = {1.0f, 3.0f, 3.0f, 1.0f};
    float c0 = 0.0f, c1 = 0.0f, c2 = 0.0f;
// ... 640 lines not shown
        if (wc.lane == 0) { a.job_nstage[job] = 0; a.retry_jobs[atomicAdd(a.nretry, 1)] = (int32_t)job; }
        return;
    }
    if (wc.lane == 0) a.job_nstage[job] = ns;
    {
        acc->cand += n_cand; acc->pref += n_pref; acc->patch += n_patch; acc->f0 += n_f0; acc->f1 += n_f1; acc->ins += n_ins; acc->rep += n_rep;
        acc->evals += wc.evals; acc->view_evals += wc.view_evals;
        acc->pair[0] += n_pair; acc->pair[5] += n_elig;
        acc->pair[1] += n_last; acc->pair[2] += n_noroom; acc->pair[3] += n_lost; acc->pair[4] += n_long;
        acc->skip += n_skip;
#ifdef MVS_STAGE_TIMING
        st_acc[0] = ST_NOW() - st_begin;
        for (int k = 0; k < 12; ++k) acc->stage[k] += st_acc[k];
        acc->stage[12] = max(acc->stage[12], st_acc[12]); acc->stage[13] = max(acc->stage[13], st_acc[13]);
        acc->stage[14] += wc.st_acc[3]; acc->stage[15] += wc.st_acc[4];
#endif
    }
}

template <bool SIMPLEX, class WC = WaveCtx>
DEV void sweep_resident(const DParams& prm, const SweepArgs& a, int* s_scratch, int* s_pend, float* s_texs, int max_evals, float xtol) {
    WC wc;
    static_cast<WaveCtx&>(wc) = make_wave_ctx(prm);
    SweepAcc acc = sweep_acc_zero();
    for (unsigned step = 0; step < MVS_SWEEP_QUEUES; ++step) {
        const unsigned q = (blockIdx.x + step) & (MVS_SWEEP_QUEUES - 1u);
        const int32_t qbegin = a.list_bounds[q];
        const unsigned ntake = (unsigned)(a.list_bounds[q + 1] - qbegin);
        if (ntake == 0u) continue;
        for (;;) {
            unsigned k = 0;
            if (wc.lane == 0) k = atomicAdd(a.cursors + q * MVS_SWEEP_CURSOR_STRIDE, 1u);
            k = (unsigned)rfl((int)k);
            if (k >= ntake) break;
            const int64_t job = a.job_list[qbegin + (int32_t)k];
            __syncthreads();
            sweep_cell<false, SIMPLEX>(prm, a, wc, &acc, job, s_scratch, s_pend, s_texs, nullptr, max_evals, xtol);
        }
    }
    if (wc.lane == 0) sweep_acc_flush(a, acc, blockIdx.x & (MVS_COUNTER_SLOTS - 1));
}
__global__ __launch_bounds__(64, MVS_SWEEP_WAVES) void k_sweep(DParams prm, SweepArgs a) {
    __shared__ int s_scratch[192];
    __shared__ __attribute__((aligned(16))) int s_pend[MVS_PEND_INTS];
    extern __shared__ float s_texs[];
    sweep_resident<false>(prm, a, s_scratch, s_pend, s_texs, 0, 0.0f);
}
__global__ __launch_bounds__(64, MVS_SWEEP_WAVES) void k_sweep_full(DParams prm, SweepArgs a) {
    __shared__ int s_scratch[192];
    __shared__ __attribute__((aligned(16))) int s_pend[MVS_PEND_INTS];
    extern __shared__ float s_texs[];
    sweep_resident<false, WaveCtxFull>(prm, a, s_scratch, s_pend, s_texs, 0, 0.0f);
}
__global__ __launch_bounds__(64, MVS_SWEEP_WAVES) void k_sweep_simplex(DParams prm, SweepArgs a, int max_evals, float xtol) {
    __shared__ int s_scratch[192];
    __shared__ __attribute__((aligned(16))) int s_pend[MVS_PEND_INTS];
    extern __shared__ float s_texs[];
    sweep_resident<true>(prm, a, s_scratch, s_pend, s_texs, max_evals, xtol);
}
template <bool SIMPLEX>
DEV void sweep_retry_cell(const DParams& prm, const SweepArgs& a, const int64_t job, int* s_scratch, int* s_pend, float* s_texs, int* big_table, int max_evals, float xtol) {
    WaveCtx wc = make_wave_ctx(prm);
    SweepAcc acc = sweep_acc_zero();
    sweep_cell<true, SIMPLEX>(prm, a, wc, &acc, job, s_scratch, s_pend, s_texs, big_table, max_evals, xtol);
    if (wc.lane == 0) sweep_acc_flush(a, acc, (unsigned)(job & (MVS_COUNTER_SLOTS - 1)));
}
__global__ __launch_bounds__(64, 1) void k_sweep_retry(DParams prm, SweepArgs a, int nretry) {
    __shared__ int s_scratch[192];
    __shared__ __attribute__((aligned(16))) int s_pend[MVS_PEND_INTS];
    extern __shared__ float s_texs[];
    int* big_table = a.big_tables + (size_t)blockIdx.x * MVS_FILTER2_HASH_CAP;
    for (int k = blockIdx.x; k < nretry; k += gridDim.x) {
        __syncthreads();
        sweep_retry_cell<false>(prm, a, (int64_t)a.retry_jobs[k], s_scratch, s_pend, s_texs, big_table, 0, 0.0f);
    }
}
__global__ __launch_bounds__(64, 1) void k_sweep_retry_simplex(DParams prm, SweepArgs a, int nretry, int max_evals, float xtol) {
    __shared__ int s_scratch[192];
    __shared__ __attribute__((aligned(16))) int s_pend[MVS_PEND_INTS];
    extern __shared__ float s_texs[];
    int* big_table = a.big_tables + (size_t)blockIdx.x * MVS_FILTER2_HASH_CAP;
    for (int k = blockIdx.x; k < nretry; k += gridDim.x) {
        __syncthreads();
        sweep_retry_cell<true>(prm, a, (int64_t)a.retry_jobs[k], s_scratch, s_pend, s_texs, big_table, max_evals, xtol);
    }
}

__global__ void k_commit_count(SweepArgs a, int32_t* __restrict__ cnt) {
    const int64_t job = (int64_t)blockIdx.x * blockDim.x + threadIdx.x;
    if (job >= a.njobs) return;
    const int ns = a.job_nstage[job];
    int c = 0;
    for (int k = 0; k < ns; ++k) c += a.staging[a.job_stage[job * a.maxstage + k]].flags & 1;
    cnt[job] = c;
}
__global__ void k_commit_copy(SweepArgs a, const int32_t* __restrict__ base, DPatch* __restrict__ dst, int64_t dst_cap, int32_t* __restrict__ per_view,
                              int keep_key) {
    const int64_t job = (int64_t)blockIdx.x * blockDim.x + threadIdx.x;
    if (job >= a.njobs) return;
    const int ns = a.job_nstage[job];
    int r = 0;
    for (int k = 0; k < ns; ++k) {
        const DPatch* sp = a.staging + a.job_stage[job * a.maxstage + k];
        if (!(sp->flags & 1)) continue;
        const int64_t o = (int64_t)base[job] + r++;
        if (o >= dst_cap) { atomicOr(a.error_flag, 2); return; }
// ... 171 lines not shown
        for (int k = 0; k < 5; ++k) {
            const float diff = dot4(ray, sub4(coord, qc[k]));
            const bool vis = prm.depth == 0 || dp[k] == ~0ull || diff < rhs;
            safe |= ok[k] && vis;
        }
    }
    WC_ADD(wc, 6)
    const unsigned long long safe_b = ballot(safe);
    const unsigned long long alive_b = ballot(alive_l);
    const int tstride = prm.wsz;
    Frame fpre = {};
    {
        const unsigned long long gbits = MVS_FE_LANES == 64 ? ~0ull : ((1ull << (MVS_FE_LANES & 63)) - 1ull) << ((MVS_FE_LANES * q) & 63);
        const bool skip_l = (pl->flags & MVS_FLAG_SETTLED) && (int)__popcll(safe_b & gbits) == nimg_l;
        if (ballot(alive_l && !skip_l)) {
            int vmin = safe ? image : INT_MAX;
            for (int d = 1; d < MVS_FE_LANES; d <<= 1) vmin = min(vmin, __shfl_xor(vmin, d));
            F4 px, py;
            get_paxes(prm, prm.views + (vmin == INT_MAX ? 0 : vmin), coord, normal, px, py);
            fpre = make_frame(prm, coord, px, py, normal, image, safe);
        }
    }
    WC_ADD(wc, 1)
    for (int g = 0; g < MVS_FE_PATCHES; ++g) {
        if (!((alive_b >> ((MVS_FE_LANES * g) & 63)) & 1ull)) continue;
        DPatch* p = prm.pool + (first + (int64_t)blockIdx.x * MVS_FE_PATCHES + g);
        const int pflags = p->flags;
        Cand c;
        load_cand(p, wc, c);
        const vmask_t sm = (vmask_t)((safe_b >> ((MVS_FE_LANES * g) & 63)) & (MVS_FE_LANES == 64 ? ~0ull : (1ull << (MVS_FE_LANES & 63)) - 1ull));
        if ((pflags & MVS_FLAG_SETTLED) && (int)vpop(sm) == c.nimg) continue;
        __syncthreads();
        if (wc.lane < MVS_MAXVIEWS) s_scratch[wc.lane] = 0;
        __syncthreads();
        if (wc.lane < c.nimg && ((sm >> wc.lane) & 1u)) s_scratch[c.img] = 1 + MVS_FE_LANES * g + wc.lane;
        __syncthreads();
        const int src1 = s_scratch[wc.lane];
        const bool present = src1 != 0;
        const unsigned long long pm = ballot(present);
        const int pos = __popcll(pm & ((1ull << wc.lane) - 1ull));
        __syncthreads();
        if (present && pos < MVS_LISTCAP) { s_scratch[64 + pos] = wc.lane; s_scratch[128 + pos] = src1 - 1; }
        __syncthreads();
        c.nimg = min((int)__popcll(pm), MVS_LISTCAP);
        c.img = s_scratch[64 + wc.lane];
        if (prm.minImageNum <= c.nimg) {
            Frame f;
            {
                const bool mine = wc.lane < c.nimg;
                const int src = mine ? s_scratch[128 + wc.lane] : MVS_FE_LANES * g;
                f.tlx = __shfl(fpre.tlx, src); f.tly = __shfl(fpre.tly, src);
                f.dxx = __shfl(fpre.dxx, src); f.dxy = __shfl(fpre.dxy, src); f.dyx = __shfl(fpre.dyx, src); f.dyy = __shfl(fpre.dyy, src);
                f.w = __shfl(fpre.w, src); f.ok = __shfl(fpre.ok, src);
                f.img_lo = (unsigned)__shfl((int)fpre.img_lo, src); f.img_hi = (unsigned)__shfl((int)fpre.img_hi, src);
                if (!mine) { f.tlx = f.tly = f.dxx = f.dxy = f.dyx = f.dyy = 0.0f; f.ok = 0; }
            }
            WC_ADD(wc, 7)
            set_ref_image(prm, wc, s_texs, tstride, c, nullptr, &f);
            store_lists(p, wc, c);
            if (wc.lane == 0) p->flags = pflags | MVS_FLAG_SETTLED;
            WC_ADD(wc, 7)
        } else {
            if (wc.lane == 0) kill[first + (int64_t)blockIdx.x * MVS_FE_PATCHES + g] = 1;
        }
    }
    if (wc.lane == 0 && wc.evals) { atomicAdd(evals + 2 * (blockIdx.x & 1023u), (unsigned long long)wc.evals); atomicAdd(evals + 2 * (blockIdx.x & 1023u) + 1, (unsigned long long)wc.view_evals); }
#ifdef MVS_STAGE_TIMING
    if (stage && wc.lane == 0) {
        atomicAdd(stage, (unsigned long long)__builtin_amdgcn_s_memtime() - fe_begin);
        for (int k = 1; k < 8; ++k) atomicAdd(stage + k, wc.st_acc[k]);
    }
#endif
}
template <int HCAP, int RCAP>
__global__ __launch_bounds__(64) void k_filter_neighbor(DParams prm, uint8_t* kill, const int32_t* todo, int32_t ntodo, int32_t* retry, int32_t* nretry,
                                                        int32_t* overflow, unsigned long long* stats , int64_t first) {
    extern __shared__ float s_lds[];
    int* const s_dummy = reinterpret_cast<int*>(s_lds);
    const int64_t id = todo ? (blockIdx.x < (unsigned)ntodo ? todo[blockIdx.x] : -1) : first + (int64_t)blockIdx.x;
    if (id < 0 || id >= prm.pool_n) return;
    const DPatch* p = prm.pool + id;
    if (!(p->flags & 1)) return;
    WaveCtx wc = make_wave_ctx(prm);
#ifdef MVS_STAGE_TIMING
    unsigned long long st_acc[16] = {0, 0, 0, 0, 0, 0, 0, 0, 0, 0, 0, 0, 0, 0, 0, 0};
    const unsigned long long st_begin = CK_NOW();
    auto st_flush = [&]() { st_acc[0] = CK_NOW() - st_begin; if (wc.lane == 0) for (int k = 0; k < 12; ++k) if (st_acc[k]) atomicAdd(stats + 4096 + k, st_acc[k]); };
#endif
    Cand c;
    load_cand(p, wc, c);
    set_grids(prm, wc, c);
#ifdef MVS_STAGE_TIMING
    const CheckCtx cx{prm.pool, -1, -1, 0, s_dummy, st_acc};
    st_acc[1] = CK_NOW() - st_begin;
#else
    const CheckCtx cx{prm.pool, -1, -1, 0, s_dummy, nullptr};
#endif
    int* table = reinterpret_cast<int*>(s_lds);
    unsigned st4[4] = {0u, 0u, 0u, 0u};
    const bool pk = prm.geo != nullptr;
    constexpr bool MK = HCAP == MVS_FILTER_HASH_CAP;
    int* const marks = reinterpret_cast<int*>(s_lds) + MVS_SET_LDS_FLOATS(HCAP, RCAP);
    const int n = pk ? find_neighbors<HCAP, false, true, MK>(prm, wc, cx, c, table, 4.0f, 2, st4, marks) : find_neighbors<HCAP, false, false, MK>(prm, wc, cx, c, table, 4.0f, 2, st4, marks);
    if (n < 0 || n > RCAP) {
        if (wc.lane == 0) {
            if (retry) retry[atomicAdd(nretry, 1)] = (int32_t)id;
            else atomicOr(overflow, 4);
// ... 131 lines not shown
    const int tstride = prm.wsz;
    if (op == 5) {
        if (wc.lane == 0) {
            const float x = in_f[i];
            out_f[5 * i] = pm_sinf(x); out_f[5 * i + 1] = pm_cosf(x); out_f[5 * i + 2] = pm_asinf(x); out_f[5 * i + 3] = pm_acosf(x);
            out_f[5 * i + 4] = pm_atanf(x);
        }
        return;
    }
    Cand c;
    load_cand(in + i, wc, c);
    if (op == 0) {
        const float ncc = compute_ncc(prm, wc, c.coord, c.normal, c.img, c.nimg);
        if (wc.lane == 0) out_f[i] = ncc;
    } else if (op == 1) {
        const int f = pre_process(prm, wc, s_scratch, c);
        store_cand(out + i, wc, c, 1, (int)i);
        if (wc.lane == 0) out_i[i] = f;
    } else if (op == 2) {
        refine_patch(prm, wc, c, 0u, 0u, (uint32_t)i, 0u);
        store_cand(out + i, wc, c, 1, (int)i);
    } else if (op == 3) {
        int f = post_process(prm, wc, s_scratch, s_texs, tstride, c);
        if (f == 0 && prm.depth >= 2 && prm.enable_check) {
            const CheckCtx cx{in, -1, -1, 0, s_scratch, nullptr};
            const int chk = check_patch(prm, wc, cx, c, s_texs, out_i + n);
            if (chk < 0) { if (wc.lane == 0) atomicOr(out_i + n, 4); }
            else if (chk) f = -1;
        }
        store_cand(out + i, wc, c, 1, (int)i);
        if (wc.lane == 0) out_i[i] = f;
    } else if (op == 4) {
        RefineCtx rc;
        rc.center = c.coord; rc.ref = rli(c.img, 0);
        rc.ray = nrm4(sub4(c.coord, ld4((prm.views + rc.ref)->center)));
        rc.dscale = c.dscale; rc.ascale = prm.ascaleConst;
        float x[3];
        encode(prm, rc, c.coord, c.normal, x);
        double fv[4];
        cost_func4(prm, wc, rc, __shfl(c.img, wc.lane & 15), c.nimg, false, x[0], x[1], x[2], fv);
        if (wc.lane == 0) out_f[i] = (float)fv[0];
    }
}

__global__ __launch_bounds__(64, MVS_SWEEP_WAVES) void k_probe_refine(DParams prm, int64_t n, const DPatch* __restrict__ in, DPatch* __restrict__ out) {
    const int64_t i = blockIdx.x;
    if (i >= n) return;
    WaveCtx wc = make_wave_ctx(prm);
    Cand c;
    load_cand(in + i, wc, c);
    refine_patch(prm, wc, c, 0u, 0u, (uint32_t)i, 0u);
    store_cand(out + i, wc, c, 1, (int)i);
}
__global__ __launch_bounds__(64, MVS_SWEEP_WAVES) void k_probe_refine_simplex(DParams prm, int64_t n, const DPatch* __restrict__ in, DPatch* __restrict__ out,
                                                                              float* __restrict__ out_f, int32_t* __restrict__ out_i, int max_evals, float xtol) {
    const int64_t i = blockIdx.x;
    if (i >= n) return;
    WaveCtx wc = make_wave_ctx(prm);
    Cand c;
    load_cand(in + i, wc, c);
    float x[3];
    double f;
    const int r = refine_patch_simplex(prm, wc, c, max_evals, xtol, nullptr, x, &f);
    store_cand(out + i, wc, c, 1, (int)i);
    if (wc.lane == 0) {
        out_f[4 * i] = x[0]; out_f[4 * i + 1] = x[1]; out_f[4 * i + 2] = x[2]; out_f[4 * i + 3] = (float)f;
        out_i[i] = r;
    }
}

static inline unsigned nblk(int64_t n, int b) { return (unsigned)((n + b - 1) / b); }

void mvsk_rgb_to_rgba(const uint8_t* rgb, uint32_t* out, int64_t n, hipStream_t st) { hipLaunchKernelGGL(k_rgb_to_rgba, dim3(nblk(n, 256)), dim3(256), 0, st, rgb, out, n); }
void mvsk_rgba_to_rgb(const uint32_t* in, uint8_t* rgb, int64_t n, hipStream_t st) { hipLaunchKernelGGL(k_rgba_to_rgb, dim3(nblk(n, 256)), dim3(256), 0, st, in, rgb, n); }
void mvsk_pyr_down(const uint32_t* src, int pw, int ph, uint32_t* dst, int w, int h, hipStream_t st) {
    hipLaunchKernelGGL(k_pyr_down, dim3((w + 63) / 64, (h + 3) / 4), dim3(64, 4), 0, st, src, pw, ph, dst, w, h);
}
void mvsk_mask_down(const uint8_t* src, int pw, int ph, uint8_t* dst, int w, int h, hipStream_t st) {
    hipLaunchKernelGGL(k_mask_down, dim3((w + 63) / 64, (h + 3) / 4), dim3(64, 4), 0, st, src, pw, ph, dst, w, h);
}
void mvsk_mask_binarise(uint8_t* m, int64_t n, hipStream_t st) { hipLaunchKernelGGL(k_mask_binarise, dim3(nblk(n, 256)), dim3(256), 0, st, m, n); }
void mvsk_exclusive_scan(const int32_t* in, int32_t* out, int64_t n, int32_t* tmp, hipStream_t st) { launch_exclusive_scan<int32_t, int32_t>(in, out, n, tmp, st); }
void mvsk_exclusive_scan_off(const int32_t* in, csr_off_t* out, int64_t n, csr_off_t* tmp, hipStream_t st) { launch_exclusive_scan<int32_t, csr_off_t>(in, out, n, tmp, st); }
void mvsk_index_count(const DParams& prm, int32_t* cnt, int32_t* vcnt, unsigned long long* total, hipStream_t st) {
    if (prm.pool_n > 0) hipLaunchKernelGGL(k_index_count, dim3(nblk(prm.pool_n, 256)), dim3(256), 0, st, prm, cnt, vcnt, total);
}
void mvsk_index_fill(const DParams& prm, int vgrid, const csr_off_t* start, int32_t* cursor, unsigned long long* ids, hipStream_t st) {
    if (prm.pool_n > 0) hipLaunchKernelGGL(k_index_fill, dim3(nblk(prm.pool_n, 256)), dim3(256), 0, st, prm, vgrid, start, cursor, ids);
}
void mvsk_index_fill_direct(const DParams& prm, int vgrid, const csr_off_t* start, int32_t* cursor, int32_t* id32, hipStream_t st) {
    if (prm.pool_n > 0) hipLaunchKernelGGL(k_index_fill_direct, dim3(nblk(prm.pool_n, 256)), dim3(256), 0, st, prm, vgrid, start, cursor, id32);
}
void mvsk_index_sort_trim(const DParams& prm, const csr_off_t* start, unsigned long long* ids, int do_trim, unsigned long long* trimmed, hipStream_t st) {
    hipLaunchKernelGGL(k_index_sort_trim, dim3(nblk(prm.total_cells, 256)), dim3(256), 0, st, prm, start, ids, do_trim, trimmed);
}
void mvsk_index_finalize(const DParams& prm, int vgrid, const csr_off_t* start, unsigned long long* ids, int32_t* id32, int32_t* cnt_alive, hipStream_t st) {
    hipLaunchKernelGGL(k_index_finalize, dim3(nblk(prm.total_cells, 256)), dim3(256), 0, st, prm, vgrid, start, ids, id32, cnt_alive);
}
void mvsk_index_pack(const DParams& prm, const csr_off_t* start, const csr_off_t* start2, const int32_t* cnt_alive, const unsigned long long* ids, const int32_t* id32_in,
                     ListKey* key, int32_t* id32_out, hipStream_t st) {
    hipLaunchKernelGGL(k_index_pack, dim3(nblk(prm.total_cells, 256)), dim3(256), 0, st, prm, start, start2, cnt_alive, ids, id32_in, key, id32_out);
}
void mvsk_depth_maps(const DParams& prm, unsigned long long* dp, const uint32_t* dirty, hipStream_t st) {
    if (prm.pool_n > 0) hipLaunchKernelGGL(k_depth_maps, dim3(nblk(prm.pool_n, 64)), dim3(256), 0, st, prm, dp, dirty);
}
void mvsk_depth_mark_dirty(const DParams& prm, const uint8_t* kill, unsigned long long* dp, uint32_t* dirty, hipStream_t st) {
    if (prm.pool_n > 0) hipLaunchKernelGGL(k_depth_mark_dirty, dim3(nblk(prm.pool_n, 64)), dim3(256), 0, st, prm, kill, dp, dirty);
}
void mvsk_best_ncc_map(const DParams& prm, int view, unsigned long long* best, hipStream_t st) {
    if (prm.pool_n > 0) hipLaunchKernelGGL(k_best_ncc_map, dim3(nblk(prm.pool_n, 256)), dim3(256), 0, st, prm, view, best);
}
void mvsk_map_extract(const DParams& prm, int view, int kind, const unsigned long long* sel, float* depth, float* normal, int32_t* ids, int ncells, hipStream_t st) {
    hipLaunchKernelGGL(k_map_extract, dim3(nblk(ncells, 256)), dim3(256), 0, st, prm, view, kind, sel, depth, normal, ids, ncells);
}
void mvsk_fill_ncc(const DParams& prm, unsigned long long* evals, hipStream_t st) {
    if (prm.pool_n > 0) hipLaunchKernelGGL(k_fill_ncc, dim3((unsigned)((prm.pool_n + 63) / 64)), dim3(64), MVS_FRAME_LDS_BYTES, st, prm, evals);
}
size_t mvsk_sweep_lds_bytes(const DParams& prm) {
#if MVS_PAIR_MFMA
    const size_t tex_f = (size_t)MVS_GRAM_CH * 3 * prm.wsz, gram_f = (size_t)prm.gram_ld * prm.gram_ld;
    const size_t texs = MVS_FRAME1_LDS_BYTES + (tex_f > gram_f ? tex_f : gram_f) * sizeof(float);
#else
    const size_t ln = (size_t)prm.list_n;
    const size_t texs = MVS_FRAME1_LDS_BYTES + (ln * 3 * prm.wsz + ln * (ln - 1) / 2) * sizeof(float);
#endif
    const size_t chk = (size_t)MVS_CHECK_LDS_FLOATS * sizeof(float);
    const size_t need = texs > chk ? texs : chk;
    return need > (size_t)MVS_FRAME_LDS_BYTES ? need : (size_t)MVS_FRAME_LDS_BYTES;
}
static SweepArgs sweep_args_with_switches(const SweepArgs& a) {
    SweepArgs b = a;
    const char* p = getenv("MVS_SWEEP_PAIR");
    b.pair = (p && atoi(p) == 0) ? 0 : 1;
    return b;
}
static bool sweep_full_window(const DParams& prm) {
    const char* p = getenv("MVS_SWEEP_FULLWINDOW");
    return cls_full_window(prm.wsz) && !(p && atoi(p) == 0);
}
int mvsk_sweep(const DParams& prm, const SweepArgs& a, const RefineSel& rs, hipStream_t st) {
    const int64_t nloc = a.job_hi - a.job_lo;
    if (nloc <= 0) return -1;
    static const size_t pad = getenv("MVS_SWEEP_LDS_PAD") ? (size_t)atol(getenv("MVS_SWEEP_LDS_PAD")) : 0;
    const size_t lds = mvsk_sweep_lds_bytes(prm) + pad;
    int dev = 0, cus = 0;
    (void)hipGetDevice(&dev);
    if (hipDeviceGetAttribute(&cus, hipDeviceAttributeMultiprocessorCount, dev) != hipSuccess || cus <= 0) { (void)hipGetLastError(); cus = 256; }
    int64_t nblocks = (int64_t)cus * 4 * MVS_SWEEP_WAVES;
    nblocks = std::min(nblocks, nloc);
    if (const char* g = getenv("MVS_SWEEP_GRID")) {
        const long cap = atol(g);
        if (cap > 0) nblocks = std::min<int64_t>(nblocks, cap);
    }
    const SweepArgs b = sweep_args_with_switches(a);
    if (rs.simplex) hipLaunchKernelGGL(k_sweep_simplex, dim3((unsigned)nblocks), dim3(64), lds, st, prm, b, rs.max_evals, rs.xtol);
    else if (sweep_full_window(prm)) { hipLaunchKernelGGL(k_sweep_full, dim3((unsigned)nblocks), dim3(64), lds, st, prm, b); return 1; }
    else hipLaunchKernelGGL(k_sweep, dim3((unsigned)nblocks), dim3(64), lds, st, prm, b);
    return 0;
}
void mvsk_job_work(const DParams& prm, const SweepArgs& a, int mode, int shift, int32_t* work, hipStream_t st) {
    if (a.njobs > 0) hipLaunchKernelGGL(k_job_work, dim3(nblk(a.njobs, 256)), dim3(256), 0, st, prm, a, mode, shift, work);
}
int mvsk_job_list_seg(const SweepArgs& a) {
    const int64_t nchunks = (std::max<int64_t>(a.job_hi - a.job_lo, 0) + MVS_XCD_CHUNK - 1) / MVS_XCD_CHUNK;
    return (int)((nchunks + MVS_SWEEP_QUEUES - 1) / MVS_SWEEP_QUEUES) * MVS_XCD_CHUNK;
}
void mvsk_job_list(const DParams& prm, const SweepArgs& a, int32_t* flags, int32_t* scan, int32_t* scan_tmp, int32_t* list, int32_t* bounds, hipStream_t st) {
    const int seg = mvsk_job_list_seg(a);
    const int64_t nslots = (int64_t)MVS_SWEEP_QUEUES * seg, nthreads = std::max(nslots, a.njobs);
    if (nthreads <= 0) return;
    hipLaunchKernelGGL(k_job_list, dim3(nblk(nthreads, 256)), dim3(256), 0, st, prm, a, seg, flags);
    if (nslots <= 0) return;
    launch_exclusive_scan<int32_t, int32_t>(flags, scan, nslots, scan_tmp, st);
    hipLaunchKernelGGL(k_job_scatter, dim3(nblk(nslots, 256)), dim3(256), 0, st, a, seg, scan, list, bounds);
}
void mvsk_job_cuts(const int32_t* scan, int64_t njobs, int n, int32_t* cuts, hipStream_t st) {
    if (njobs > 0) hipLaunchKernelGGL(k_job_cuts, dim3(nblk(njobs, 256)), dim3(256), 0, st, scan, njobs, n, cuts);
}
void mvsk_sweep_retry(const DParams& prm, const SweepArgs& a, int nretry, const RefineSel& rs, hipStream_t st) {
    if (nretry <= 0) return;
    const dim3 grid((unsigned)std::min(nretry, MVS_BIG_SLOTS));
    const SweepArgs b = sweep_args_with_switches(a);
    if (rs.simplex) hipLaunchKernelGGL(k_sweep_retry_simplex, grid, dim3(64), mvsk_sweep_lds_bytes(prm), st, prm, b, nretry, rs.max_evals, rs.xtol);
    else hipLaunchKernelGGL(k_sweep_retry, grid, dim3(64), mvsk_sweep_lds_bytes(prm), st, prm, b, nretry);
}
void mvsk_commit_count(const SweepArgs& a, int32_t* cnt, hipStream_t st) { hipLaunchKernelGGL(k_commit_count, dim3(nblk(a.njobs, 256)), dim3(256), 0, st, a, cnt); }
void mvsk_commit_copy(const SweepArgs& a, const int32_t* base, DPatch* dst, int64_t dst_cap, int32_t* per_view, int keep_key, hipStream_t st) {
    hipLaunchKernelGGL(k_commit_copy, dim3(nblk(a.njobs, 256)), dim3(256), 0, st, a, base, dst, dst_cap, per_view, keep_key);
}
void mvsk_kill_count(const uint8_t* kill, int64_t n, int32_t* cnt, hipStream_t st) { if (n > 0) hipLaunchKernelGGL(k_kill_count, dim3(nblk(n, 256)), dim3(256), 0, st, kill, n, cnt); }
void mvsk_kill_export(const uint8_t* kill, int64_t n, const int32_t* base, int32_t* ids, int64_t cap, hipStream_t st) {
    if (n > 0) hipLaunchKernelGGL(k_kill_export, dim3(nblk(n, 256)), dim3(256), 0, st, kill, n, base, ids, cap);
}
void mvsk_apply_kill_flags(DPatch* pool, uint8_t* kill, int64_t n, hipStream_t st) { if (n > 0) hipLaunchKernelGGL(k_apply_kill_flags, dim3(nblk(n, 256)), dim3(256), 0, st, pool, kill, n); }
void mvsk_apply_kill_ids(DPatch* pool, const int32_t* ids, int64_t n, int64_t pool_n, hipStream_t st) {
    if (n > 0) hipLaunchKernelGGL(k_apply_kill_ids, dim3(nblk(n, 256)), dim3(256), 0, st, pool, ids, n, pool_n);
}
void mvsk_append_records(DPatch* pool, int64_t pool_n, const DPatch* recs, int64_t n, hipStream_t st) {
    if (n > 0) hipLaunchKernelGGL(k_append_records, dim3(nblk(n, 256)), dim3(256), 0, st, pool, pool_n, recs, n);
}
void mvsk_alive_count(const DPatch* pool, int64_t n, int32_t* cnt, hipStream_t st) { if (n > 0) hipLaunchKernelGGL(k_alive_count, dim3(nblk(n, 256)), dim3(256), 0, st, pool, n, cnt); }
void mvsk_alive_gather(const DPatch* pool, int64_t n, const int32_t* base, DPatch* out, int64_t cap, hipStream_t st) {
    if (n > 0) hipLaunchKernelGGL(k_alive_gather, dim3(nblk(n, 256)), dim3(256), 0, st, pool, n, base, out, cap);
}
void mvsk_filter_vimages(const DParams& prm, int additive, int64_t first, int64_t last, const uint32_t* dirty, hipStream_t st) {
    if (last <= first) return;
    const int gl = std::max(prm.nviews <= 16 ? 16 : (prm.nviews <= 32 ? 32 : 64), (int)MVS_LISTCAP);
    const unsigned nb = (unsigned)((last - first + 64 / gl - 1) / (64 / gl));
    if (gl == 16) hipLaunchKernelGGL(k_filter_vimages<16>, dim3(nb), dim3(64), 0, st, prm, additive, first, last, dirty);
// ... 7 lines not shown
void mvsk_filter_outside(const DParams& prm, uint8_t* kill, int64_t first, int64_t last, hipStream_t st) {
    if (last > first) hipLaunchKernelGGL(k_filter_outside, dim3((unsigned)(last - first)), dim3(64), 0, st, prm, kill, first);
}
size_t mvsk_texs_lds_bytes(const DParams& prm) {
#if MVS_PAIR_MFMA
    const size_t tex_f = (size_t)MVS_GRAM_CH * 3 * prm.wsz, gram_f = (size_t)prm.gram_ld * prm.gram_ld;
    const size_t texs = MVS_FRAME1_LDS_BYTES + (tex_f > gram_f ? tex_f : gram_f) * sizeof(float);
#else
    const size_t ln = (size_t)prm.list_n;
    const size_t texs = MVS_FRAME1_LDS_BYTES + (ln * 3 * prm.wsz + ln * (ln - 1) / 2) * sizeof(float);
#endif
    return texs > (size_t)MVS_FRAME_LDS_BYTES ? texs : (size_t)MVS_FRAME_LDS_BYTES;
}
void mvsk_filter_exact(const DParams& prm, uint8_t* kill, unsigned long long* evals, unsigned long long* stage, int64_t first, int64_t last, hipStream_t st) {
    if (last > first) hipLaunchKernelGGL(k_filter_exact, dim3((unsigned)((last - first + MVS_FE_PATCHES - 1) / MVS_FE_PATCHES)), dim3(64), mvsk_texs_lds_bytes(prm), st, prm, kill, evals, stage, first, last);
}
void mvsk_filter_neighbor(const DParams& prm, uint8_t* kill, int32_t* retry, int32_t* nretry, int32_t* overflow, unsigned long long* stats, int64_t first, int64_t last, hipStream_t st) {
    if (last <= first) return;
    hipLaunchKernelGGL((k_filter_neighbor<MVS_FILTER_HASH_CAP, MVS_FILTER_ROW_CAP>), dim3((unsigned)(last - first)), dim3(64),
                       (size_t)(MVS_SET_LDS_FLOATS(MVS_FILTER_HASH_CAP, MVS_FILTER_ROW_CAP) + 64) * sizeof(float), st, prm, kill, (const int32_t*)nullptr, 0, retry, nretry, overflow, stats, first);
}
void mvsk_filter_neighbor_retry(const DParams& prm, uint8_t* kill, const int32_t* todo, int32_t ntodo, int32_t* overflow, unsigned long long* stats, hipStream_t st) {
    if (ntodo <= 0) return;
    hipLaunchKernelGGL((k_filter_neighbor<MVS_FILTER2_HASH_CAP, MVS_FILTER2_ROW_CAP>), dim3((unsigned)ntodo), dim3(64),
                       (size_t)MVS_SET_LDS_FLOATS(MVS_FILTER2_HASH_CAP, MVS_FILTER2_ROW_CAP) * sizeof(float), st, prm, kill, todo, ntodo, (int32_t*)nullptr, (int32_t*)nullptr, overflow, stats, (int64_t)0);
}
void mvsk_groups(const DParams& prm, int* parent, int* size, int threshold, uint8_t* kill, hipStream_t st) {
    if (prm.pool_n <= 0) return;
    hipLaunchKernelGGL(k_groups_init, dim3(nblk(prm.pool_n, 256)), dim3(256), 0, st, parent, size, prm.pool_n);
    hipLaunchKernelGGL(k_groups_edges<0>, dim3(nblk(prm.pool_n, 4)), dim3(256), 0, st, prm, parent, (int2*)nullptr, (int*)nullptr, 0);
    hipLaunchKernelGGL(k_groups_count, dim3(nblk(prm.pool_n, 256)), dim3(256), 0, st, prm, parent, size, threshold);
    hipLaunchKernelGGL(k_groups_kill, dim3(nblk(prm.pool_n, 256)), dim3(256), 0, st, prm, parent, size, threshold, kill);
}
void mvsk_groups_literal_edges(const DParams& prm, int* parent, int* size, int* edges2, int* nedges, int cap, hipStream_t st) {
    if (prm.pool_n <= 0) return;
    hipLaunchKernelGGL(k_groups_init, dim3(nblk(prm.pool_n, 256)), dim3(256), 0, st, parent, size, prm.pool_n);
    hipLaunchKernelGGL(k_groups_edges<1>, dim3(nblk(prm.pool_n, 4)), dim3(256), 0, st, prm, parent, (int2*)nullptr, (int*)nullptr, 0);
    hipLaunchKernelGGL(k_groups_count, dim3(nblk(prm.pool_n, 256)), dim3(256), 0, st, prm, parent, size, INT_MAX);
    hipLaunchKernelGGL(k_groups_edges<2>, dim3(nblk(prm.pool_n, 4)), dim3(256), 0, st, prm, parent, reinterpret_cast<int2*>(edges2), nedges, cap);
}
__global__ void k_gather_i32(const int32_t* __restrict__ src, const int32_t* __restrict__ idx, int32_t* __restrict__ out, int64_t n) {
    const int64_t i = (int64_t)blockIdx.x * blockDim.x + threadIdx.x;
    if (i < n) out[i] = src[idx[i]];
}
__global__ void k_scatter_i32(int32_t* __restrict__ dst, const int32_t* __restrict__ idx, const int32_t* __restrict__ val, int64_t n) {
    const int64_t i = (int64_t)blockIdx.x * blockDim.x + threadIdx.x;
    if (i < n) dst[idx[i]] = val[i];
}
void mvsk_gather_i32(const int32_t* src, const int32_t* idx, int32_t* out, int64_t n, hipStream_t st) { if (n > 0) hipLaunchKernelGGL(k_gather_i32, dim3(nblk(n, 256)), dim3(256), 0, st, src, idx, out, n); }
void mvsk_scatter_i32(int32_t* dst, const int32_t* idx, const int32_t* val, int64_t n, hipStream_t st) { if (n > 0) hipLaunchKernelGGL(k_scatter_i32, dim3(nblk(n, 256)), dim3(256), 0, st, dst, idx, val, n); }
void mvsk_groups_kill(const DParams& prm, const int* parent, const int* size, int threshold, uint8_t* kill, hipStream_t st) {
    if (prm.pool_n > 0) hipLaunchKernelGGL(k_groups_kill, dim3(nblk(prm.pool_n, 256)), dim3(256), 0, st, prm, parent, size, threshold, kill);
}
void mvsk_probe(const DParams& prm, int op, int64_t n, const DPatch* in, const float* in_f, DPatch* out, float* out_f, int32_t* out_i, const RefineSel& rs,
                hipStream_t st) {
    if (n > 0 && (op == 2 || op == 6) && rs.simplex) {
        hipLaunchKernelGGL(k_probe_refine_simplex, dim3((unsigned)n), dim3(64), MVS_FRAME_LDS_BYTES, st, prm, n, in, out, out_f, out_i, rs.max_evals, rs.xtol);
        return;
    }
    if (n > 0 && op == 2) { hipLaunchKernelGGL(k_probe_refine, dim3((unsigned)n), dim3(64), MVS_FRAME_LDS_BYTES, st, prm, n, in, out); return; }
    if (n > 0) hipLaunchKernelGGL(k_probe, dim3((unsigned)n), dim3(64), mvsk_sweep_lds_bytes(prm), st, prm, op, n, in, in_f, out, out_f, out_i);
}
```

mvskit_amd/csrc/mvs_types.h:

```cpp
#pragma once
#include <stdint.h>

#define MVS_WAVE 64
#define MVS_MAXLEV 7
#ifndef MVS_LISTCAP
#define MVS_LISTCAP 16
#endif
#if MVS_LISTCAP > 32
#define MVS_MAXI 64
#else
#define MVS_MAXI 32
#endif
#define MVS_MAXVIEWS 64
#define MVS_CAPMAX 32
#define MVS_NEWBASE 0x40000000

#define MVS_FLAG_ALIVE 1
#define MVS_FLAG_SETTLED 2
struct DPatch {
    float coord[4];
    float normal[4];
    float ncc, dscale, ascale, tmp;
    int32_t nimages, nvimages, flags, id;
    uint8_t images[MVS_MAXI];
    uint8_t vimages[MVS_MAXI];
};
static_assert(sizeof(DPatch) == 64 + 2 * MVS_MAXI, "record is 128 bytes (192 in the 64-view build)");
#define MVS_REC_U4 (sizeof(DPatch) / 16)

typedef int64_t csr_off_t;
struct ListKey {
    float ncc;
    int32_t ref;
};
static_assert(sizeof(ListKey) == 8, "list key is 8 bytes");

struct DView {
    float P[MVS_MAXLEV][12];
    float Minv[9];
    float center[4];
    float oaxis[4];
    float xaxis[3], yaxis[3], zaxis[3];
    float ipscale;
    int32_t W[MVS_MAXLEV], H[MVS_MAXLEV];
    const uint32_t* img[MVS_MAXLEV];
    const uint8_t* mask;
    int32_t gw, gh;
    int32_t cell_base;
    int32_t pad;
};

struct DParams {
    int32_t nviews, level, csize, wsize, wsz, minImageNum, tau, cap, max_propag, depth, enable_check, view_propagation;
    uint32_t seed;
    int32_t refine_steps;
    float rd0, ra0;
    float nccThreshold, nccThresholdBefore;
    float cosAngle0, cosAngle1, cosMinAngle, cosMaxAngle, cosNeighborTypo, cosNeighbor120;
    float sortThreshold, ascaleConst, neighborThreshold, neighborThreshold1, quadThreshold;
    float inv_sz, inv_3sz;
    int32_t total_cells;
    int32_t list_n;
    int32_t gram_ld;
    const DView* views;
    DPatch* pool;
    int64_t pool_n;
    const csr_off_t* csr_start;
    const int32_t* csr_cnt;
    const ListKey* csr_key;
    const int32_t* csr_id32;
    const csr_off_t* vcsr_start;
    const int32_t* vcsr_cnt;
    const int32_t* vcsr_id32;
    const float4* geo;
    const uint8_t* geo_ref;
    const unsigned long long* dpgrid;
};

#ifndef MVS_COUNTER_SLOTS
#define MVS_COUNTER_SLOTS 256
#endif
#define MVS_SWEEP_QUEUES 8
#define MVS_SWEEP_CURSOR_STRIDE 32
struct DCounters {
    unsigned long long candidates, prefiltered, patches, fail0, fail1, inserted, replaced, evals, view_evals, trimmed;
    unsigned long long stage[16];
    unsigned long long pair[6];
    unsigned long long repeats[2];
};

struct SweepArgs {
    int32_t iter, inc, colour;
    int32_t nsweep_views;
    int32_t sweep_views[MVS_MAXVIEWS];
    int32_t job_base[MVS_MAXVIEWS];
    int32_t halfw_max, gh_max;
    int64_t njobs;
    int64_t job_lo, job_hi;
    DPatch* staging;
    int64_t staging_cap;
    unsigned long long* stage_counter;
    int32_t* job_stage;
    int32_t* job_nstage;
    int32_t maxstage;
    uint8_t* kill;
    DCounters* counters;
    int32_t* error_flag;
    int32_t* big_tables;
    int32_t* retry_jobs;
    int32_t* nretry;
    uint32_t* cursors;
    const int32_t* job_list;
    const int32_t* list_bounds;
    int32_t pair;
};

struct SeedChainArgs {
    int32_t K;
    float min_ncc;
    int32_t simplex, max_evals;
    float xtol;
};

struct SeedPointsArgs {
    SeedChainArgs chain;
    int64_t first;
    int32_t n;
};
```

mvskit_amd/engine.py:

```python
from __future__ import annotations

import ctypes as C
import math
import os

import numpy as np

from . import build
from . import synth
from .synth import MAX_IMAGES, PATCH_DTYPE

PROBE_NCC, PROBE_PREPROCESS, PROBE_REFINE, PROBE_POSTPROCESS, PROBE_COST, PROBE_MATH, PROBE_REFINE_X = range(7)
REFINE_HALVING, REFINE_CONVERGED = 0, 1
MVS_OK, MVS_ERR_ARG, MVS_ERR_STATE, MVS_ERR_HIP, MVS_ERR_CAPACITY, MVS_ERR_NO_DEVICE = 0, -1, -2, -3, -4, -5

EXPORTS = [
    "mvs_last_error", "mvs_device_count", "mvs_default_config", "mvs_engine_create", "mvs_engine_destroy",
    "mvs_engine_set_views", "mvs_engine_grid_dims", "mvs_engine_get_pyramid", "mvs_engine_set_thresholds",
    "mvs_engine_get_thresholds", "mvs_engine_update_threshold", "mvs_engine_upload_patches",
    "mvs_engine_clear_patches", "mvs_engine_num_patches", "mvs_engine_download_patches", "mvs_engine_propagate",
    "mvs_engine_pass", "mvs_engine_export_counts", "mvs_engine_export_device", "mvs_engine_commit_device",
    "mvs_engine_commit_local", "mvs_engine_depth_normal_map", "mvs_engine_probe", "mvs_engine_last_timing",
    "mvs_engine_filter", "mvs_comm_unique_id", "mvs_engine_comm_init", "mvs_engine_comm_attach", "mvs_engine_comm_release",
    "mvs_engine_exchange", "mvs_list_cap", "mvs_engine_filter_stats", "mvs_patch_bytes", "mvs_engine_reserve", "mvs_engine_comm_info",
    "mvs_default_refiner", "mvs_engine_set_refiner", "mvs_engine_export_ply", "mvs_engine_seed_patches",
    "mvs_default_seed_random", "mvs_engine_seed_random", "mvs_engine_seed_random_hypotheses",
    "mvs_default_seed_points", "mvs_engine_seed_points", "mvs_engine_seed_points_hypotheses", "mvs_engine_depth_ranges",
    "mvs_default_maps_config", "mvs_engine_render_maps", "mvs_engine_fused_points",
    "mvs_engine_tsdf", "mvs_engine_extract_mesh", "mvs_engine_mesh", "mvs_engine_sweep_pairs", "mvs_engine_sweep_repeats", "mvs_engine_sweep_kernels",
    "mvs_default_mesh_colouring", "mvs_engine_mesh_normals", "mvs_engine_mesh_colours",
    "mvs_default_mesh_pruning", "mvs_default_mesh_smoothing", "mvs_engine_mesh_components", "mvs_engine_mesh_prune", "mvs_engine_mesh_smooth",
    "mvs_default_mesh_decimation", "mvs_engine_mesh_decimate",
]
PLY_ASCII, PLY_BINARY_LE = 0, 1
PLY_VERTEX_DTYPE = np.dtype([("xyz", "<f4", (3,)), ("normal", "<f4", (3,)), ("rgb", "u1", (3,))])
FUSED_POINT_DTYPE = np.dtype([("xyz", "<f4", (3,)), ("normal", "<f4", (3,)), ("conf", "<f4"), ("rgb", "u1", (3,)), ("view", "u1")])


class Config(C.Structure):
    _fields_ = [("nviews", C.c_int32), ("level", C.c_int32), ("csize", C.c_int32), ("wsize", C.c_int32),
                ("minImageNum", C.c_int32), ("max_propag", C.c_int32), ("nccThreshold", C.c_float),
                ("maxAngleThreshold", C.c_float), ("quadThreshold", C.c_float), ("depth", C.c_int32),
                ("seed", C.c_uint32), ("refine_steps", C.c_int32), ("refine_rd0", C.c_float), ("refine_ra0", C.c_float),
                ("enable_check", C.c_int32), ("view_begin", C.c_int32), ("view_stride", C.c_int32),
                ("device", C.c_int32), ("view_propagation", C.c_int32), ("shard_index", C.c_int32), ("shard_count", C.c_int32),
                ("literal_groups", C.c_int32), ("max_patches", C.c_int64)]


class Refiner(C.Structure):
    _fields_ = [("mode", C.c_int32), ("max_evals", C.c_int32), ("xtol", C.c_float)]


class ViewDesc(C.Structure):
    _fields_ = [("width", C.c_int32), ("height", C.c_int32), ("P", C.c_float * 12), ("rgb", C.c_void_p),
                ("mask", C.c_void_p)]


class SeedView(C.Structure):
    _fields_ = [("normals", C.c_void_p), ("mask", C.c_void_p)]


class SeedRandom(C.Structure):
    _fields_ = [("hypotheses", C.c_int32), ("seed", C.c_uint32), ("max_tilt", C.c_float), ("min_ncc", C.c_float),
                ("depth_min", C.c_void_p), ("depth_max", C.c_void_p)]


class SeedPoints(C.Structure):
    _fields_ = [("hypotheses", C.c_int32), ("min_ncc", C.c_float)]


class MapsConfig(C.Structure):
    _fields_ = [("source", C.c_int32), ("min_consistent", C.c_int32), ("depth_tol", C.c_float), ("normal_cos", C.c_float),
                ("dedupe", C.c_int32), ("pad", C.c_int32)]


class ViewMaps(C.Structure):
    _fields_ = [("depth", C.c_void_p), ("normal", C.c_void_p), ("conf", C.c_void_p), ("ids", C.c_void_p), ("agree", C.c_void_p)]


class Volume(C.Structure):
    _fields_ = [("origin", C.c_float * 3), ("voxel", C.c_float), ("dims", C.c_int32 * 3), ("trunc", C.c_float), ("min_count", C.c_int32),
                ("pad", C.c_int32)]
# ... 76 lines not shown
    L.mvs_engine_upload_patches.argtypes = [vp, C.c_int64, vp]
    L.mvs_engine_clear_patches.argtypes = [vp]
    L.mvs_engine_num_patches.argtypes = [vp, C.POINTER(C.c_int64)]
    L.mvs_engine_download_patches.argtypes = [vp, C.c_int64, vp, C.POINTER(C.c_int64)]
    L.mvs_engine_propagate.argtypes = [vp, C.c_int, C.POINTER(Counters)]
    L.mvs_engine_pass.argtypes = [vp, C.c_int, C.c_int, C.POINTER(Counters)]
    L.mvs_engine_export_counts.argtypes = [vp, C.POINTER(C.c_int64), C.POINTER(C.c_int64), vp]
    L.mvs_engine_export_device.argtypes = [vp, vp, C.c_int64, vp, C.c_int64]
    L.mvs_engine_commit_device.argtypes = [vp, vp, C.c_int64, vp, C.c_int64]
    L.mvs_engine_commit_local.argtypes = [vp]
    L.mvs_engine_depth_normal_map.argtypes = [vp, C.c_int, C.c_int, vp, vp, vp]
    L.mvs_engine_probe.argtypes = [vp, C.c_int, C.c_int64, vp, vp, vp, vp, vp]
    L.mvs_engine_last_timing.argtypes = [vp, C.POINTER(Timing)]
    L.mvs_engine_filter.argtypes = [vp, vp]
    L.mvs_comm_unique_id.argtypes = [vp]
    L.mvs_engine_comm_init.argtypes = [vp, vp, C.c_int, C.c_int]
    L.mvs_engine_comm_attach.argtypes = [vp, vp, C.c_int, C.c_int]
    L.mvs_engine_comm_release.argtypes = [vp]
    L.mvs_engine_exchange.argtypes = [vp]
    L.mvs_list_cap.restype = C.c_int
    L.mvs_patch_bytes.restype = C.c_int
    L.mvs_engine_reserve.argtypes = [vp, C.c_int64]
    L.mvs_engine_filter_stats.argtypes = [vp, C.POINTER(FilterStats)]
    if hasattr(L, "mvs_engine_set_refiner"):
        L.mvs_default_refiner.argtypes = [C.POINTER(Refiner)]
        L.mvs_default_refiner.restype = None
        L.mvs_engine_set_refiner.argtypes = [vp, C.POINTER(Refiner)]
    if hasattr(L, "mvs_engine_export_ply"):
        L.mvs_engine_export_ply.argtypes = [vp, C.c_int, C.c_int64, vp, C.POINTER(C.c_int64)]
    if hasattr(L, "mvs_engine_seed_patches"):
        L.mvs_engine_seed_patches.argtypes = [vp, C.c_int64, vp, C.POINTER(SeedView), C.POINTER(C.c_int64)]
    if hasattr(L, "mvs_engine_seed_random"):
        L.mvs_default_seed_random.argtypes = [C.POINTER(SeedRandom)]
        L.mvs_default_seed_random.restype = None
        L.mvs_engine_seed_random.argtypes = [vp, C.POINTER(SeedRandom), C.POINTER(C.c_int64)]
        L.mvs_engine_seed_random_hypotheses.argtypes = [vp, C.POINTER(SeedRandom), C.c_int, C.c_int64, vp, vp]
    if hasattr(L, "mvs_engine_seed_points"):
        L.mvs_default_seed_points.argtypes = [C.POINTER(SeedPoints)]
        L.mvs_default_seed_points.restype = None
        L.mvs_engine_seed_points.argtypes = [vp, C.POINTER(SeedPoints), C.c_int64, vp, C.POINTER(C.c_int64)]
        L.mvs_engine_seed_points_hypotheses.argtypes = [vp, C.POINTER(SeedPoints), C.c_int64, vp, vp, vp]
        L.mvs_engine_depth_ranges.argtypes = [vp, C.c_int64, vp, C.c_float, vp, vp, vp]
    if hasattr(L, "mvs_engine_render_maps"):
        L.mvs_default_maps_config.argtypes = [C.POINTER(MapsConfig)]
        L.mvs_default_maps_config.restype = None
        L.mvs_engine_render_maps.argtypes = [vp, C.POINTER(MapsConfig), C.POINTER(ViewMaps), vp]
        L.mvs_engine_fused_points.argtypes = [vp, C.POINTER(MapsConfig), C.c_int64, vp, C.POINTER(C.c_int64)]
    if hasattr(L, "mvs_engine_sweep_pairs"):
        L.mvs_engine_sweep_pairs.argtypes = [vp, C.POINTER(C.c_int64)]
    if hasattr(L, "mvs_engine_sweep_repeats"):
        L.mvs_engine_sweep_repeats.argtypes = [vp, C.POINTER(C.c_int64)]
    if hasattr(L, "mvs_engine_sweep_kernels"):
        L.mvs_engine_sweep_kernels.argtypes = [vp, C.POINTER(C.c_int64)]
    if hasattr(L, "mvs_engine_tsdf"):
        L.mvs_engine_tsdf.argtypes = [vp, C.POINTER(MapsConfig), C.POINTER(Volume), vp, vp]
        L.mvs_engine_extract_mesh.argtypes = [vp, C.POINTER(Volume), vp, vp, C.c_int64, vp, C.c_int64, vp, C.POINTER(C.c_int64), C.POINTER(C.c_int64)]
        L.mvs_engine_mesh.argtypes = [vp, C.POINTER(MapsConfig), C.POINTER(Volume), C.c_int64, vp, C.c_int64, vp, C.POINTER(C.c_int64), C.POINTER(C.c_int64)]
    if hasattr(L, "mvs_engine_mesh_normals"):
        L.mvs_default_mesh_colouring.argtypes = [C.POINTER(MeshColouring)]
        L.mvs_default_mesh_colouring.restype = None
        L.mvs_engine_mesh_normals.argtypes = [vp, C.c_int64, vp, C.c_int64, vp, vp]
        L.mvs_engine_mesh_colours.argtypes = [vp, C.POINTER(MapsConfig), C.POINTER(MeshColouring), C.c_int64, vp, vp, vp, vp]
    if hasattr(L, "mvs_engine_mesh_components"):
        L.mvs_default_mesh_pruning.argtypes = [C.POINTER(MeshPruning)]
        L.mvs_default_mesh_pruning.restype = None
        L.mvs_default_mesh_smoothing.argtypes = [C.POINTER(MeshSmoothing)]
        L.mvs_default_mesh_smoothing.restype = None
        L.mvs_engine_mesh_components.argtypes = [vp, C.c_int64, C.c_int64, vp, vp, vp, C.POINTER(C.c_int64)]
        L.mvs_engine_mesh_prune.argtypes = [vp, C.POINTER(MeshPruning), C.c_int64, vp, C.c_int64, vp, C.c_int64, vp, C.c_int64, vp, vp,
                                            C.POINTER(C.c_int64), C.POINTER(C.c_int64)]
        L.mvs_engine_mesh_smooth.argtypes = [vp, C.POINTER(MeshSmoothing), C.c_int64, vp, C.c_int64, vp, vp]
    if hasattr(L, "mvs_engine_mesh_decimate"):
        L.mvs_default_mesh_decimation.argtypes = [C.POINTER(MeshDecimation)]
        L.mvs_default_mesh_decimation.restype = None
        L.mvs_engine_mesh_decimate.argtypes = [vp, C.POINTER(MeshDecimation), C.c_int64, vp, C.c_int64, vp, C.c_int64, vp, C.c_int64, vp, vp,
                                               C.POINTER(C.c_int64), C.POINTER(C.c_int64)]
    _libs[LIB_PATH] = L
    return L


def _ptr(a):
    return a.ctypes.data_as(C.c_void_p) if a is not None else None


class Engine:

    def __init__(self, nviews, list_cap=None, **kw):
        if list_cap is None:
            list_cap = 16 if nviews <= 16 else (32 if nviews <= 32 else 64)
        self.L = load_library(cap=list_cap)
        self.list_cap = self.L.mvs_list_cap()
        self.dtype = synth.patch_dtype((self.L.mvs_patch_bytes() - 64) // 2)
        self.cfg = Config()
        self.L.mvs_default_config(C.byref(self.cfg))
        self.cfg.nviews = nviews
        for k, v in kw.items():
            if not hasattr(self.cfg, k):
                raise AttributeError(k)
            setattr(self.cfg, k, v)
        self.h = C.c_void_p()
        self._check(self.L.mvs_engine_create(C.byref(self.cfg), C.byref(self.h)))
        self._keep = None

    def _check(self, status):
        if status != 0:
            raise EngineError(f"mvskit engine error {status}: {self.L.mvs_last_error().decode()}", status)
# ... 362 lines not shown
    def commit_local(self):
        self._check(self.L.mvs_engine_commit_local(self.h))

    COMM_ID_BYTES = 128

    def comm_unique_id(self):
        buf = C.create_string_buffer(self.COMM_ID_BYTES)
        self._check(self.L.mvs_comm_unique_id(buf))
        return buf.raw

    def comm_init(self, uid: bytes, rank: int, world: int):
        assert len(uid) == self.COMM_ID_BYTES
        self._check(self.L.mvs_engine_comm_init(self.h, C.c_char_p(uid), rank, world))

    def comm_info(self):
        r, w, cc, cr = C.c_int(), C.c_int(), C.c_int(), C.c_int()
        self.L.mvs_engine_comm_info.argtypes = [C.c_void_p] + [C.POINTER(C.c_int)] * 4
        self._check(self.L.mvs_engine_comm_info(self.h, C.byref(r), C.byref(w), C.byref(cc), C.byref(cr)))
        return {"rank": r.value, "world": w.value, "comm_count": cc.value, "comm_rank": cr.value}

    def comm_release(self):
        self._check(self.L.mvs_engine_comm_release(self.h))

    def exchange(self):
        self._check(self.L.mvs_engine_exchange(self.h))

    def timing(self):
        t = Timing()
        self._check(self.L.mvs_engine_last_timing(self.h, C.byref(t)))
        return {"index_ms": t.index_ms, "sweep_ms": t.sweep_ms, "commit_ms": t.commit_ms, "sweep_launches": t.sweep_launches,
                "exchange_ms": t.exchange_ms, "exchange_bytes": int(t.exchange_bytes), "check_retried_cells": int(t.check_retried_cells),
                "sweep_jobs_listed": int(t.sweep_jobs_listed)}

    SWEEP_PAIR_KEYS = ("paired", "alone_no_partner", "alone_no_room", "alone_partner_failed", "alone_long_list", "can_pair")

    def sweep_pairs(self):
        out = (C.c_int64 * 6)()
        self._check(self.L.mvs_engine_sweep_pairs(self.h, out))
        return dict(zip(self.SWEEP_PAIR_KEYS, (int(x) for x in out)))

    SWEEP_REPEAT_KEYS = ("skipped", "from_stash")

    def sweep_repeats(self):
        out = (C.c_int64 * 2)()
        self._check(self.L.mvs_engine_sweep_repeats(self.h, out))
        return dict(zip(self.SWEEP_REPEAT_KEYS, (int(x) for x in out)))

    SWEEP_KERNEL_KEYS = ("generic", "full_window")

    def sweep_kernels(self):
        out = (C.c_int64 * 2)()
        self._check(self.L.mvs_engine_sweep_kernels(self.h, out))
        return dict(zip(self.SWEEP_KERNEL_KEYS, (int(x) for x in out)))

    def depth_normal_map(self, view, kind):
        gw, gh = self.grid_dims(view)
        d = np.zeros((gh, gw), np.float32)
        n = np.zeros((gh, gw, 3), np.float32)
        ids = np.zeros((gh, gw), np.int32)
        self._check(self.L.mvs_engine_depth_normal_map(self.h, view, kind, _ptr(d), _ptr(n), _ptr(ids)))
        return d, n, ids

    def probe(self, op, recs=None, values=None):
        if op == PROBE_MATH:
            x = np.ascontiguousarray(values, dtype=np.float32)
            out = np.zeros((x.shape[0], 5), np.float32)
            self._check(self.L.mvs_engine_probe(self.h, op, x.shape[0], None, _ptr(x), None, _ptr(out), None))
            return out
        recs = synth.convert_records(recs, self.dtype)
        n = recs.shape[0]
        out_rec = np.zeros(n, dtype=self.dtype)
        out_f = np.zeros((n, 4) if op == PROBE_REFINE_X else n, np.float32)
        out_i = np.zeros(n, np.int32)
        self._check(self.L.mvs_engine_probe(self.h, op, n, _ptr(recs), None, _ptr(out_rec), _ptr(out_f), _ptr(out_i)))
        return out_rec, out_f, out_i


def make_volume(origin, voxel, dims, trunc, min_count=1):
    v = Volume()
    for k in range(3):
        v.origin[k], v.dims[k] = float(origin[k]), int(dims[k])
    v.voxel, v.trunc, v.min_count, v.pad = float(voxel), float(trunc), int(min_count), 0
    return v


def decimation_origin(volume):
    half = np.float32(volume.voxel) / np.float32(2)
    return tuple(float(np.float32(volume.origin[k]) - half) for k in range(3))


def volume_around(xyz, voxel, trunc_voxels=4, pad_voxels=2, min_count=1):
    xyz = np.asarray(xyz, dtype=np.float64).reshape(-1, 3)
    if xyz.shape[0] == 0 or not np.isfinite(xyz).all() or not voxel > 0:
        raise ValueError("volume_around: needs finite points and a positive voxel")
    lo = xyz.min(axis=0) - pad_voxels * voxel
    dims = np.ceil((xyz.max(axis=0) + pad_voxels * voxel - lo) / voxel).astype(np.int64) + 1
    if (dims < 2).any() or (dims > 1024).any() or int(np.prod(dims)) > 1 << 28:
        raise ValueError(f"volume_around: {dims.tolist()} lattice points: each dimension must lie in 2..1024, their product must not exceed 2^28")
    return make_volume(lo, voxel, dims, trunc_voxels * voxel, min_count)


def write_mesh_ply(path, verts, tris, binary=True, normals=None, colours=None):
    verts = np.ascontiguousarray(verts, dtype="<f4").reshape(-1, 3)
    tris = np.ascontiguousarray(tris, dtype="<i4").reshape(-1, 3)
    fields, props = [("xyz", "<f4", (3,))], "property float x\nproperty float y\nproperty float z\n"
    cols = [verts]
# ... 29 lines not shown
```

Measured before the change: 32.62 million.

## Pack image pyramids into one buffer and sample with 32-bit offsets

All view pyramid levels are placed in a single contiguous device allocation, and per-level byte offsets are stored in each view. A new narrow full-window sweep kernel and refine probe compute texel addresses with 32-bit offset arithmetic (umul24 plus a base pointer) instead of 64-bit pointer math. This is meant to cut VALU address-calculation work and register pressure in the sampling inner loop. It adds kernel variants, launch counters and an environment switch, and it depends on the packed pyramid staying under 4 GB.

```diff
diff --git a/include/mvskit_engine.h b/include/mvskit_engine.h
--- a/include/mvskit_engine.h
+++ b/include/mvskit_engine.h
@@ -294,6 +294,8 @@
 
 int mvs_engine_sweep_kernels(mvs_engine* e, int64_t out[2]);
 
+int mvs_engine_sampler_launches(mvs_engine* e, int64_t out[4]);
+
 #ifdef __cplusplus
 }
 #endif
diff --git a/mvskit_amd/csrc/mvs_device.cuh b/mvskit_amd/csrc/mvs_device.cuh
--- a/mvskit_amd/csrc/mvs_device.cuh
+++ b/mvskit_amd/csrc/mvs_device.cuh
@@ -275,7 +275,7 @@
     float tlx, tly, dxx, dxy, dyx, dyy;
     int w;
     int ok;
-    unsigned img_lo, img_hi;
+    unsigned a_lo, a_hi;
 };
 DEV int level_diff(const DParams& prm, float ratio) {
     static_assert(0x3504F3 == (0x3FB504F3 & 0x7FFFFF), "mantissa of 1.414213562373095f");
@@ -284,6 +284,7 @@
     return max(-prm.level, min(2, ld));
 }
 DEV float pow2_level(int ld) { return __int_as_float((127 + ld) << 23); }
+template <bool NARROW = false>
 DEV Frame make_frame(const DParams& prm, F4 coord, F4 px, F4 py, F4 pz, int v, bool active) {
     const DView* vw = prm.views + (active ? v : 0);
     const F4 ctr = ld4(vw->center);
@@ -291,7 +292,7 @@
 #pragma unroll
     for (int k = 0; k < 12; ++k) P[k] = vw->P[prm.level][k];
     const int W0 = vw->W[0], H0 = vw->H[0];
-    const unsigned long long base_level = (unsigned long long)vw->img[prm.level];
+    const unsigned long long base_level = NARROW ? (unsigned long long)vw->img_off[prm.level] : (unsigned long long)vw->img[prm.level];
     const F4 ray = nrm4(sub4(ctr, coord));
     const float weight = fmaxf(0.0f, dot4(ray, pz));
     F3 center = project_regs(P, coord);
@@ -301,7 +302,7 @@
     const int ld = level_diff(prm, ratio);
     const float iscale = pow2_level(-ld);
     const int newLevel = prm.level + ld;
-    const unsigned long long base_new = (unsigned long long)vw->img[newLevel];
+    const unsigned long long base_new = NARROW ? (unsigned long long)vw->img_off[newLevel] : (unsigned long long)vw->img[newLevel];
     center = scl3(center, iscale);
     dx = scl3(dx, iscale);
     dy = scl3(dy, iscale);
@@ -320,7 +321,8 @@
     f.w = ok ? W : (W0 >> prm.level);
     f.ok = ok ? 1 : 0;
     const unsigned long long a = ok ? base_new : base_level;
-    f.img_lo = (unsigned)(a & 0xffffffffull); f.img_hi = (unsigned)(a >> 32);
+    f.a_lo = (unsigned)(a & 0xffffffffull);
+    f.a_hi = NARROW ? 4u * (unsigned)f.w : (unsigned)(a >> 32);
     return f;
 }
 
@@ -353,6 +355,12 @@
 struct WaveCtxFull : WaveCtx {};
 template <class WC> struct wc_full_window { static constexpr bool value = false; };
 template <> struct wc_full_window<WaveCtxFull> { static constexpr bool value = true; };
+struct WaveCtxOfs : WaveCtx {};
+struct WaveCtxFullOfs : WaveCtx {};
+template <> struct wc_full_window<WaveCtxFullOfs> { static constexpr bool value = true; };
+template <class WC> struct wc_narrow { static constexpr bool value = false; };
+template <> struct wc_narrow<WaveCtxOfs> { static constexpr bool value = true; };
+template <> struct wc_narrow<WaveCtxFullOfs> { static constexpr bool value = true; };
 #ifdef MVS_STAGE_TIMING
 #define WC_T0(wc) { (wc).st_t = (unsigned long long)__builtin_amdgcn_s_memtime(); }
 #define WC_ADD(wc, k) { const unsigned long long t1_ = (unsigned long long)__builtin_amdgcn_s_memtime(); (wc).st_acc[k] += t1_ - (wc).st_t; (wc).st_t = t1_; }
@@ -371,7 +379,7 @@
         float4* d = mvs_dyn_lds4 + 3 * wc.lane;
         d[0] = make_float4(f.tlx, f.tly, f.dxx, f.dxy);
         d[1] = make_float4(f.dyx, f.dyy, __int_as_float(f.w), __int_as_float(f.ok));
-        d[2] = make_float4(__int_as_float((int)f.img_lo), __int_as_float((int)f.img_hi), 0.0f, 0.0f);
+        d[2] = make_float4(__int_as_float((int)f.a_lo), __int_as_float((int)f.a_hi), 0.0f, 0.0f);
     }
     __syncthreads();
 }
@@ -401,24 +409,42 @@
 DEV float cvt_ub1(unsigned x) { return (float)((x >> 8) & 255u); }
 DEV float cvt_ub2(unsigned x) { return (float)((x >> 16) & 255u); }
 DEV unsigned cls_opaque(unsigned x) { asm volatile("" : "+v"(x)); return x; }
-struct ClsFrame { float tlx, tly, dxx, dxy, dyx, dyy; int w; unsigned long long base; };
+struct ClsFrame { float tlx, tly, dxx, dxy, dyx, dyy; int w; unsigned a_lo, a_hi; };
 DEV ClsFrame cls_frame(int fidx) {
     const float4* s = mvs_dyn_lds4 + 3 * fidx;
     const float4 A = s[0], B = s[1];
     const float2 Cc = *reinterpret_cast<const float2*>(s + 2);
     ClsFrame f;
     f.tlx = A.x; f.tly = A.y; f.dxx = A.z; f.dxy = A.w; f.dyx = B.x; f.dyy = B.y; f.w = __float_as_int(B.z);
-    f.base = ((unsigned long long)(unsigned)__float_as_int(Cc.y) << 32) | (unsigned long long)(unsigned)__float_as_int(Cc.x);
+    f.a_lo = (unsigned)__float_as_int(Cc.x); f.a_hi = (unsigned)__float_as_int(Cc.y);
     return f;
 }
-DEV ClsPend cls_issue(const ClsFrame& f, unsigned cs) {
+DEV ClsFrame cls_frame_of(const Frame& f) {
+    ClsFrame fr;
+    fr.tlx = f.tlx; fr.tly = f.tly; fr.dxx = f.dxx; fr.dxy = f.dxy; fr.dyx = f.dyx; fr.dyy = f.dyy; fr.w = f.w;
+    fr.a_lo = f.a_lo; fr.a_hi = f.a_hi;
+    return fr;
+}
+template <bool NARROW> DEV const uint8_t* sampler_base(const DParams& prm) { return NARROW ? prm.pyr32 : nullptr; }
+template <bool NARROW>
+DEV ClsPend cls_issue(const uint8_t* pyr, const ClsFrame& f, unsigned cs) {
     typedef const __attribute__((address_space(1))) uint32_t* GlobalTexels;
+    typedef const __attribute__((address_space(1))) uint8_t* GlobalBytes;
     const float fx = cvt_ub0(cs), fy = cvt_ub1(cs);
     const float sx = fma_(f.dyx, fy, fma_(f.dxx, fx, f.tlx));
     const float sy = fma_(f.dyy, fy, fma_(f.dxy, fx, f.tly));
     const int lx = (int)sx, ly = (int)sy;
-    const unsigned long long a0 = f.base + 4ull * (unsigned long long)(unsigned)(ly * f.w + lx);
-    const GlobalTexels t0 = (GlobalTexels)a0, t1 = (GlobalTexels)(a0 + 4ull * (unsigned long long)(unsigned)f.w);
+    GlobalTexels t0, t1;
+    if (NARROW) {
+        unsigned row = __umul24((unsigned)ly, f.a_hi) + f.a_lo;
+        asm("" : "+v"(row));
+        const unsigned o0 = row + ((unsigned)lx << 2), o1 = o0 + f.a_hi;
+        t0 = (GlobalTexels)((GlobalBytes)pyr + (unsigned long long)o0); t1 = (GlobalTexels)((GlobalBytes)pyr + (unsigned long long)o1);
+    } else {
+        const unsigned long long base = ((unsigned long long)f.a_hi << 32) | (unsigned long long)f.a_lo;
+        const unsigned long long a0 = base + 4ull * (unsigned long long)(unsigned)(ly * f.w + lx);
+        t0 = (GlobalTexels)a0; t1 = (GlobalTexels)(a0 + 4ull * (unsigned long long)(unsigned)f.w);
+    }
     ClsPend p;
     p.q0.a = t0[0]; p.q0.b = t0[1];
     p.q1.a = t1[0]; p.q1.b = t1[1];
@@ -445,7 +471,8 @@
                            s1r = s1r + t0; s1g = s1g + t1; s1b = s1b + t2; s2 = s2 + t3; }
 template <class WC>
 DEV void eval_steps4(const DParams& prm, WC& wc, const ClsConst& cc, const Frame& f, int n, unsigned (&okm)[4], float& incc_l) {
-    constexpr bool FULL = wc_full_window<WC>::value;
+    constexpr bool FULL = wc_full_window<WC>::value, NARROW = wc_narrow<WC>::value;
+    const uint8_t* const pyr = sampler_base<NARROW>(prm);
     const bool has_x = cc.nx > 0;
     frames_publish(wc, f, 64);
     const unsigned long long okb = ballot(f.ok != 0);
@@ -462,7 +489,7 @@
     {
         const ClsFrame fr = cls_frame(fb);
 #pragma unroll
-        for (int j = 0; j < 3; ++j) pend[j] = cls_issue(fr, cls_opaque(cc.cs[j]));
+        for (int j = 0; j < 3; ++j) pend[j] = cls_issue<NARROW>(pyr, fr, cls_opaque(cc.cs[j]));
     }
     {
         const float4 pv = mvs_dyn_lds4[MVS_PIVOT_LDS4];
@@ -473,7 +500,7 @@
             const unsigned cs = cls_opaque(cc.cs[j]);
             float r, g, b;
             cls_colour<FULL>(pend[j], cs, pv.x, pv.y, pv.z, r, g, b);
-            pend[j] = cls_issue(fn, cs);
+            pend[j] = cls_issue<NARROW>(pyr, fn, cs);
             c0[j][0] = r; c0[j][1] = g; c0[j][2] = b;
             s1r += r; s1g += g; s1b += b;
             s2 = fma_(r, r, s2); s2 = fma_(g, g, s2); s2 = fma_(b, b, s2);
@@ -490,7 +517,7 @@
             const unsigned cs = cls_opaque(cc.cs[j]);
             float r, g, b;
             cls_colour<FULL>(pend[j], cs, pv.x, pv.y, pv.z, r, g, b);
-            pend[j] = cls_issue(fn, cs);
+            pend[j] = cls_issue<NARROW>(pyr, fn, cs);
             s1r += r; s1g += g; s1b += b;
             s2 = fma_(r, r, s2); s2 = fma_(g, g, s2); s2 = fma_(b, b, s2);
             s01 = fma_(r, c0[j][0], s01); s01 = fma_(g, c0[j][1], s01); s01 = fma_(b, c0[j][2], s01);
@@ -501,12 +528,10 @@
     const int a0 = (wc.lane & 48) << 2;
     if (has_x) {
         const float4 pv = mvs_dyn_lds4[MVS_PIVOT_LDS4 + lc];
-        ClsFrame fr;
-        fr.tlx = f.tlx; fr.tly = f.tly; fr.dxx = f.dxx; fr.dxy = f.dxy; fr.dyx = f.dyx; fr.dyy = f.dyy; fr.w = f.w;
-        fr.base = ((unsigned long long)f.img_hi << 32) | (unsigned long long)f.img_lo;
+        const ClsFrame fr = cls_frame_of(f);
         {
             const unsigned cs = cc.xcs;
-            const ClsPend pe = cls_issue(fr, cs);
+            const ClsPend pe = cls_issue<NARROW>(pyr, fr, cs);
             float r, g, b;
             cls_colour<FULL>(pe, cs, pv.x, pv.y, pv.z, r, g, b);
             const float r0 = bperm_f(a0, r), g0 = bperm_f(a0, g), b0 = bperm_f(a0, b);
@@ -525,7 +550,8 @@
 
 template <class WC>
 DEV unsigned long long eval_steps4_pair(const DParams& prm, WC& wc, const ClsConst& cc, const Frame& f, int n0, int n1, unsigned (&okm)[2][4], float& incc_l) {
-    constexpr bool FULL = wc_full_window<WC>::value;
+    constexpr bool FULL = wc_full_window<WC>::value, NARROW = wc_narrow<WC>::value;
+    const uint8_t* const pyr = sampler_base<NARROW>(prm);
     const bool has_x = FULL || cc.nx > 0;
     frames_publish(wc, f, 64);
     const unsigned long long okb = ballot(f.ok != 0);
@@ -546,7 +572,7 @@
         {
             const ClsFrame fr = cls_frame(fb);
 #pragma unroll
-            for (int j = 0; j < 3; ++j) pend[j] = cls_issue(fr, cls_opaque(cc.cs[j]));
+            for (int j = 0; j < 3; ++j) pend[j] = cls_issue<NARROW>(pyr, fr, cls_opaque(cc.cs[j]));
         }
         {
             const float4 pv = mvs_dyn_lds4[pb];
@@ -557,7 +583,7 @@
                 const unsigned cs = cls_opaque(cc.cs[j]);
                 float r, g, b;
                 cls_colour<FULL>(pend[j], cs, pv.x, pv.y, pv.z, r, g, b);
-                pend[j] = cls_issue(fn, cs);
+                pend[j] = cls_issue<NARROW>(pyr, fn, cs);
                 c0[j][0] = r; c0[j][1] = g; c0[j][2] = b;
                 s1r += r; s1g += g; s1b += b;
                 s2 = fma_(r, r, s2); s2 = fma_(g, g, s2); s2 = fma_(b, b, s2);
@@ -574,7 +600,7 @@
                 const unsigned cs = cls_opaque(cc.cs[j]);
                 float r, g, b;
                 cls_colour<FULL>(pend[j], cs, pv.x, pv.y, pv.z, r, g, b);
-                pend[j] = cls_issue(fn, cs);
+                pend[j] = cls_issue<NARROW>(pyr, fn, cs);
                 s1r += r; s1g += g; s1b += b;
                 s2 = fma_(r, r, s2); s2 = fma_(g, g, s2); s2 = fma_(b, b, s2);
                 s01 = fma_(r, c0[j][0], s01); s01 = fma_(g, c0[j][1], s01); s01 = fma_(b, c0[j][2], s01);
@@ -586,12 +612,10 @@
     const int a0 = (wc.lane & 56) << 2;
     if (has_x) {
         const float4 pv = mvs_dyn_lds4[MVS_PIVOT_LDS4 + lc];
-        ClsFrame fr;
-        fr.tlx = f.tlx; fr.tly = f.tly; fr.dxx = f.dxx; fr.dxy = f.dxy; fr.dyx = f.dyx; fr.dyy = f.dyy; fr.w = f.w;
-        fr.base = ((unsigned long long)f.img_hi << 32) | (unsigned long long)f.img_lo;
+        const ClsFrame fr = cls_frame_of(f);
         {
             const unsigned cs = cc.xcs;
-            const ClsPend pe = cls_issue(fr, cs);
+            const ClsPend pe = cls_issue<NARROW>(pyr, fr, cs);
             float r, g, b;
             cls_colour<FULL>(pe, cs, pv.x, pv.y, pv.z, r, g, b);
             const float r0 = bperm_f(a0, r), g0 = bperm_f(a0, g), b0 = bperm_f(a0, b);
@@ -657,7 +681,8 @@
     const int gk0 = wc.lane / MVS_GRAM_CH;
     const float* const grow = texs + (wc.lane & (MVS_GRAM_CH - 1)) * gtp;
 #endif
-    constexpr bool FULL = wc_full_window<WC>::value;
+    constexpr bool FULL = wc_full_window<WC>::value, NARROW = wc_narrow<WC>::value;
+    const uint8_t* const pyr = sampler_base<NARROW>(prm);
     const ClsConst& cc = wc.cc;
     const bool has_x = FULL || cc.nx > 0;
     frames_publish(wc, f, MVS_LISTCAP > 16 ? MVS_LISTCAP : 16);
@@ -668,11 +693,9 @@
     unsigned xcs = 0u;
     ClsPend pe;
     if (has_x) {
-        ClsFrame fr;
-        fr.tlx = f.tlx; fr.tly = f.tly; fr.dxx = f.dxx; fr.dxy = f.dxy; fr.dyx = f.dyx; fr.dyy = f.dyy; fr.w = f.w;
-        fr.base = ((unsigned long long)f.img_hi << 32) | (unsigned long long)f.img_lo;
+        const ClsFrame fr = cls_frame_of(f);
         xcs = cc.xcs;
-        pe = cls_issue(fr, xcs);
+        pe = cls_issue<NARROW>(pyr, fr, xcs);
     }
     float d0[3][3], d0x[3] = {0.0f, 0.0f, 0.0f};
     float ssd_l = 1.0f, dot_l = 0.0f, mr_l = 128.0f, mg_l = 128.0f, mb_l = 128.0f;
@@ -681,7 +704,7 @@
         const int last = max(n - 1, 0);
         const ClsFrame fr = cls_frame(min(row, last));
 #pragma unroll
-        for (int j = 0; j < 3; ++j) pend[j] = cls_issue(fr, cls_opaque(cc.cs[j]));
+        for (int j = 0; j < 3; ++j) pend[j] = cls_issue<NARROW>(pyr, fr, cls_opaque(cc.cs[j]));
     }
     if (has_x) cls_raw<FULL>(pe, xcs, fxr, fxg, fxb);
     const int rounds = (n + 3) >> 2;
@@ -694,7 +717,7 @@
         for (int j = 0; j < 3; ++j) {
             const unsigned cs = cls_opaque(cc.cs[j]);
             cls_raw<FULL>(pend[j], cs, cr[j], cg[j], cb[j]);
-            pend[j] = cls_issue(fn, cs);
+            pend[j] = cls_issue<NARROW>(pyr, fn, cs);
             s1r += cr[j]; s1g += cg[j]; s1b += cb[j];
         }
         MVS_ROW_STEP3(0xB1) MVS_ROW_STEP3(0x4E) MVS_ROW_STEP3(0x141) MVS_ROW_STEP3(0x140)
@@ -927,7 +950,7 @@
     get_paxes(prm, prm.views + ref, coord, normal, px, py);
     const int sz = min(prm.tau, n);
     wc.evals++;
-    const Frame f = make_frame(prm, coord, px, py, normal, img, wc.lane < sz);
+    const Frame f = make_frame<wc_narrow<WC>::value>(prm, coord, px, py, normal, img, wc.lane < sz);
     vmask_t okm[1];
     float incc_l;
     eval_views(prm, wc, f, sz, okm, incc_l);
@@ -969,7 +992,7 @@
     F4 px, py;
     get_paxes(prm, prm.views + ref, coord, normal, px, py);
     wc.evals++;
-    const Frame f = make_frame(prm, coord, px, py, normal, img, wc.lane < n);
+    const Frame f = make_frame<wc_narrow<WC>::value>(prm, coord, px, py, normal, img, wc.lane < n);
     vmask_t okm[1];
     float incc_l;
     eval_views(prm, wc, f, n, okm, incc_l, nullptr, texs, tstride, ssd_out);
@@ -1194,7 +1217,7 @@
     const int sz = min(prm.tau, n);
     const int minimum = min(prm.minImageNum, sz);
     const int g = wc.lane >> 4, i = wc.lane & 15;
-    const Frame f = make_frame(prm, coord, px, py, normal, imgx, (four ? ((rows >> g) & 1u) != 0u : g < 1) && i < sz);
+    const Frame f = make_frame<wc_narrow<WC>::value>(prm, coord, px, py, normal, imgx, (four ? ((rows >> g) & 1u) != 0u : g < 1) && i < sz);
     float incc_l;
     fv[1] = fv[2] = fv[3] = 2.0;
     if (four) {
@@ -1316,7 +1339,7 @@
     F4 coord, normal, px, py;
     decode(prm, rc, x0, x1, x2, coord, normal);
     get_paxes<true>(prm, prm.views + rc.ref, coord, normal, px, py);
-    const Frame f = make_frame(prm, coord, px, py, normal, imgx, (wc.lane & 7) < szl);
+    const Frame f = make_frame<wc_narrow<WC>::value>(prm, coord, px, py, normal, imgx, (wc.lane & 7) < szl);
     wc.evals += 8u;
     unsigned okm[2][4];
     float incc_l;
@@ -1602,7 +1625,7 @@
     else {
         F4 px, py;
         get_paxes(prm, prm.views + ref, c.coord, c.normal, px, py);
-        f = make_frame(prm, c.coord, px, py, c.normal, c.img, wc.lane < n);
+        f = make_frame<wc_narrow<WC>::value>(prm, c.coord, px, py, c.normal, c.img, wc.lane < n);
     }
     wc.evals++;
     WC_ADD(wc, 1)
diff --git a/mvskit_amd/csrc/mvs_engine.cpp b/mvskit_amd/csrc/mvs_engine.cpp
--- a/mvskit_amd/csrc/mvs_engine.cpp
+++ b/mvskit_amd/csrc/mvs_engine.cpp
@@ -37,6 +37,7 @@
 DParams current_params(mvs_engine* e) {
     DParams p = e->prm;
     p.views = e->dviews.p;
+    p.pyr32 = e->pyr_narrow ? e->pyr.p : nullptr;
     p.pool = e->pool.p;
     p.pool_n = e->pool_n;
     p.total_cells = e->total_cells;
@@ -233,7 +234,7 @@
     HIPCHK(hipSetDevice(e->cfg.device));
     hipStream_t st = e->stream;
     Range rg("mvs:set_views (upload + pyramids)");
-    e->img_bufs.clear(); e->mask_bufs.clear();
+    e->mask_bufs.clear();
     e->have_views = false;
     const int maxLevel = e->cfg.level + 3;
     e->hviews.assign(nviews, DView{});
@@ -244,18 +245,32 @@
         max_bytes = std::max(max_bytes, (size_t)views[v].width * views[v].height * 3);
     }
     if (int r = e->tmp_bytes.ensure((int64_t)max_bytes)) return r;
+    std::vector<uint64_t> level_off((size_t)nviews * maxLevel);
+    uint64_t pyr_bytes = 0;
+    bool narrow = true;
     for (int v = 0; v < nviews; ++v) {
         DView& vw = e->hviews[v];
         vw.W[0] = views[v].width; vw.H[0] = views[v].height;
         for (int l = 1; l < maxLevel; ++l) { vw.W[l] = vw.W[l - 1] / 2; vw.H[l] = vw.H[l - 1] / 2; }
+        for (int l = 0; l < maxLevel; ++l) {
+            level_off[(size_t)v * maxLevel + l] = pyr_bytes;
+            pyr_bytes += (std::max<uint64_t>((uint64_t)vw.W[l] * vw.H[l], 1) * 4 + 255) / 256 * 256;
+        }
+        if ((int64_t)vw.W[0] * 4 >= (1 << 24) || vw.H[0] >= (1 << 24)) narrow = false;
+    }
+    if (pyr_bytes >= (1ull << 32)) narrow = false;
+    if (int r = e->pyr.ensure((int64_t)pyr_bytes)) return r;
+    e->pyr_narrow = narrow;
+    for (int v = 0; v < nviews; ++v) {
+        DView& vw = e->hviews[v];
         setup_camera(e, vw, views[v].P);
         const size_t n0 = (size_t)vw.W[0] * vw.H[0];
         HIPCHK(hipMemcpyAsync(e->tmp_bytes.p, views[v].rgb, n0 * 3, hipMemcpyHostToDevice, st));
         for (int l = 0; l < maxLevel; ++l) {
-            e->img_bufs.emplace_back();
-            if (int r = e->img_bufs.back().ensure(std::max<int64_t>((int64_t)vw.W[l] * vw.H[l], 1))) return r;
-            uint32_t* buf = e->img_bufs.back().p;
+            const uint64_t off = level_off[(size_t)v * maxLevel + l];
+            uint32_t* buf = reinterpret_cast<uint32_t*>(e->pyr.p + off);
             vw.img[l] = buf;
+            vw.img_off[l] = (uint32_t)off;
             if (l == 0) mvsk_rgb_to_rgba(e->tmp_bytes.p, buf, (int64_t)n0, st);
             else mvsk_pyr_down(vw.img[l - 1], vw.W[l - 1], vw.H[l - 1], buf, vw.W[l], vw.H[l], st);
         }
@@ -450,6 +465,12 @@
     return MVS_OK;
 }
 
+int mvs_engine_sampler_launches(mvs_engine* e, int64_t out[4]) {
+    if (!e || !out) return MVS_ERR_ARG;
+    for (int k = 0; k < 4; ++k) out[k] = e->sampler_launches[k];
+    return MVS_OK;
+}
+
 int mvs_engine_last_timing(mvs_engine* e, mvs_timing* t) {
     if (!e || !t) return MVS_ERR_ARG;
     *t = e->timing;
@@ -501,7 +522,8 @@
     }
     HIPCHK(hipMemsetAsync(e->tmp_i.p, 0, (size_t)(n + 1) * sizeof(int32_t), st));
     const DParams p = current_params(e);
-    mvsk_probe(p, op, n, e->tmp_rec_in.p, e->tmp_f_in.p, e->tmp_rec_out.p, e->tmp_f_out.p, e->tmp_i.p, rs, st);
+    const int probe_sampler = mvsk_probe(p, op, n, e->tmp_rec_in.p, e->tmp_f_in.p, e->tmp_rec_out.p, e->tmp_f_out.p, e->tmp_i.p, rs, st);
+    if (probe_sampler >= 0) e->sampler_launches[2 + probe_sampler] += 1;
     if (out_rec && (op == MVS_PROBE_PREPROCESS || op == MVS_PROBE_REFINE || op == MVS_PROBE_POSTPROCESS || op == MVS_PROBE_REFINE_X))
         HIPCHK(hipMemcpyAsync(out_rec, e->tmp_rec_out.p, (size_t)n * sizeof(mvs_patch), hipMemcpyDeviceToHost, st));
     if (out_f && (op == MVS_PROBE_NCC || op == MVS_PROBE_COST || op == MVS_PROBE_MATH || op == MVS_PROBE_REFINE_X))
diff --git a/mvskit_amd/csrc/mvs_engine_impl.h b/mvskit_amd/csrc/mvs_engine_impl.h
--- a/mvskit_amd/csrc/mvs_engine_impl.h
+++ b/mvskit_amd/csrc/mvs_engine_impl.h
@@ -120,7 +120,8 @@
     bool have_views = false;
     std::vector<DView> hviews;
     DevBuf<DView> dviews;
-    std::vector<DevBuf<uint32_t>> img_bufs;
+    DevBuf<uint8_t> pyr;
+    bool pyr_narrow = false;
     std::vector<DevBuf<uint8_t>> mask_bufs;
     int total_cells = 0;
     DevBuf<DPatch> pool, pool_alt;
@@ -155,6 +156,7 @@
     int64_t sweep_pairs[6] = {0, 0, 0, 0, 0, 0};
     int64_t sweep_repeats[2] = {0, 0};
     int64_t sweep_kernels[2] = {0, 0};
+    int64_t sampler_launches[4] = {0, 0, 0, 0};
     int64_t retried_cells = 0;
     int64_t pass_retried = 0;
     SweepArgs sa{};
diff --git a/mvskit_amd/csrc/mvs_engine_pass.cpp b/mvskit_amd/csrc/mvs_engine_pass.cpp
--- a/mvskit_amd/csrc/mvs_engine_pass.cpp
+++ b/mvskit_amd/csrc/mvs_engine_pass.cpp
@@ -227,7 +227,7 @@
     HIPCHK(hipEventRecord(e->ev[1], st));
     Range rg_sweep(pass & 1 ? "mvs:sweep colour 1" : "mvs:sweep colour 0");
     const int sweep_kernel = mvsk_sweep(p, a, rs, st);
-    if (sweep_kernel >= 0) e->sweep_kernels[sweep_kernel] += 1;
+    if (sweep_kernel >= 0) { e->sweep_kernels[sweep_kernel & 1] += 1; e->sampler_launches[(sweep_kernel >> 1) & 1] += 1; }
     e->pass_retried = 0;
     if (want_vgrid(e)) {
         int32_t nretry = 0;
diff --git a/mvskit_amd/csrc/mvs_kernels.h b/mvskit_amd/csrc/mvs_kernels.h
--- a/mvskit_amd/csrc/mvs_kernels.h
+++ b/mvskit_amd/csrc/mvs_kernels.h
@@ -49,7 +49,7 @@
 void mvsk_gather_i32(const int32_t* src, const int32_t* idx, int32_t* out, int64_t n, hipStream_t st);
 void mvsk_scatter_i32(int32_t* dst, const int32_t* idx, const int32_t* val, int64_t n, hipStream_t st);
 void mvsk_groups_kill(const DParams& prm, const int* parent, const int* size, int threshold, uint8_t* kill, hipStream_t st);
-void mvsk_probe(const DParams& prm, int op, int64_t n, const DPatch* in, const float* in_f, DPatch* out, float* out_f, int32_t* out_i, const RefineSel& rs,
+int mvsk_probe(const DParams& prm, int op, int64_t n, const DPatch* in, const float* in_f, DPatch* out, float* out_f, int32_t* out_i, const RefineSel& rs,
                 hipStream_t st);
 void mvsk_ply_select(const DPatch* pool, const int32_t* base, int64_t i0, int64_t i1, int32_t* idx, hipStream_t st);
 void mvsk_ply_colour(const DPatch* pool, const int32_t* idx, int64_t n, const DView* views, int nviews, int level, int ascii, uint32_t* rgb, int32_t* len,
diff --git a/mvskit_amd/csrc/mvs_kernels.hip b/mvskit_amd/csrc/mvs_kernels.hip
--- a/mvskit_amd/csrc/mvs_kernels.hip
+++ b/mvskit_amd/csrc/mvs_kernels.hip
@@ -716,6 +716,12 @@
     extern __shared__ float s_texs[];
     sweep_resident<false, WaveCtxFull>(prm, a, s_scratch, s_pend, s_texs, 0, 0.0f);
 }
+__global__ __launch_bounds__(64, MVS_SWEEP_WAVES) void k_sweep_full_ofs(DParams prm, SweepArgs a) {
+    __shared__ int s_scratch[192];
+    __shared__ __attribute__((aligned(16))) int s_pend[MVS_PEND_INTS];
+    extern __shared__ float s_texs[];
+    sweep_resident<false, WaveCtxFullOfs>(prm, a, s_scratch, s_pend, s_texs, 0, 0.0f);
+}
 __global__ __launch_bounds__(64, MVS_SWEEP_WAVES) void k_sweep_simplex(DParams prm, SweepArgs a, int max_evals, float xtol) {
     __shared__ int s_scratch[192];
     __shared__ __attribute__((aligned(16))) int s_pend[MVS_PEND_INTS];
@@ -993,7 +999,7 @@
                 f.tlx = __shfl(fpre.tlx, src); f.tly = __shfl(fpre.tly, src);
                 f.dxx = __shfl(fpre.dxx, src); f.dxy = __shfl(fpre.dxy, src); f.dyx = __shfl(fpre.dyx, src); f.dyy = __shfl(fpre.dyy, src);
                 f.w = __shfl(fpre.w, src); f.ok = __shfl(fpre.ok, src);
-                f.img_lo = (unsigned)__shfl((int)fpre.img_lo, src); f.img_hi = (unsigned)__shfl((int)fpre.img_hi, src);
+                f.a_lo = (unsigned)__shfl((int)fpre.a_lo, src); f.a_hi = (unsigned)__shfl((int)fpre.a_hi, src);
                 if (!mine) { f.tlx = f.tly = f.dxx = f.dxy = f.dyx = f.dyy = 0.0f; f.ok = 0; }
             }
             WC_ADD(wc, 7)
@@ -1231,6 +1237,16 @@
     refine_patch(prm, wc, c, 0u, 0u, (uint32_t)i, 0u);
     store_cand(out + i, wc, c, 1, (int)i);
 }
+__global__ __launch_bounds__(64, MVS_SWEEP_WAVES) void k_probe_refine_ofs(DParams prm, int64_t n, const DPatch* __restrict__ in, DPatch* __restrict__ out) {
+    const int64_t i = blockIdx.x;
+    if (i >= n) return;
+    WaveCtxOfs wc;
+    static_cast<WaveCtx&>(wc) = make_wave_ctx(prm);
+    Cand c;
+    load_cand(in + i, wc, c);
+    refine_patch(prm, wc, c, 0u, 0u, (uint32_t)i, 0u);
+    store_cand(out + i, wc, c, 1, (int)i);
+}
 __global__ __launch_bounds__(64, MVS_SWEEP_WAVES) void k_probe_refine_simplex(DParams prm, int64_t n, const DPatch* __restrict__ in, DPatch* __restrict__ out,
                                                                               float* __restrict__ out_f, int32_t* __restrict__ out_i, int max_evals, float xtol) {
     const int64_t i = blockIdx.x;
@@ -1317,6 +1333,10 @@
     const char* p = getenv("MVS_SWEEP_FULLWINDOW");
     return cls_full_window(prm.wsz) && !(p && atoi(p) == 0);
 }
+static bool sampler_narrow(const DParams& prm) {
+    const char* p = getenv("MVS_SAMPLER_WIDE");
+    return prm.pyr32 && !(p && atoi(p) != 0);
+}
 int mvsk_sweep(const DParams& prm, const SweepArgs& a, const RefineSel& rs, hipStream_t st) {
     const int64_t nloc = a.job_hi - a.job_lo;
     if (nloc <= 0) return -1;
@@ -1333,7 +1353,11 @@
     }
     const SweepArgs b = sweep_args_with_switches(a);
     if (rs.simplex) hipLaunchKernelGGL(k_sweep_simplex, dim3((unsigned)nblocks), dim3(64), lds, st, prm, b, rs.max_evals, rs.xtol);
-    else if (sweep_full_window(prm)) { hipLaunchKernelGGL(k_sweep_full, dim3((unsigned)nblocks), dim3(64), lds, st, prm, b); return 1; }
+    else if (sweep_full_window(prm)) {
+        if (sampler_narrow(prm)) { hipLaunchKernelGGL(k_sweep_full_ofs, dim3((unsigned)nblocks), dim3(64), lds, st, prm, b); return 3; }
+        hipLaunchKernelGGL(k_sweep_full, dim3((unsigned)nblocks), dim3(64), lds, st, prm, b);
+        return 1;
+    }
     else hipLaunchKernelGGL(k_sweep, dim3((unsigned)nblocks), dim3(64), lds, st, prm, b);
     return 0;
 }
@@ -1447,12 +1471,17 @@
 void mvsk_groups_kill(const DParams& prm, const int* parent, const int* size, int threshold, uint8_t* kill, hipStream_t st) {
     if (prm.pool_n > 0) hipLaunchKernelGGL(k_groups_kill, dim3(nblk(prm.pool_n, 256)), dim3(256), 0, st, prm, parent, size, threshold, kill);
 }
-void mvsk_probe(const DParams& prm, int op, int64_t n, const DPatch* in, const float* in_f, DPatch* out, float* out_f, int32_t* out_i, const RefineSel& rs,
+int mvsk_probe(const DParams& prm, int op, int64_t n, const DPatch* in, const float* in_f, DPatch* out, float* out_f, int32_t* out_i, const RefineSel& rs,
                 hipStream_t st) {
     if (n > 0 && (op == 2 || op == 6) && rs.simplex) {
         hipLaunchKernelGGL(k_probe_refine_simplex, dim3((unsigned)n), dim3(64), MVS_FRAME_LDS_BYTES, st, prm, n, in, out, out_f, out_i, rs.max_evals, rs.xtol);
-        return;
-    }
-    if (n > 0 && op == 2) { hipLaunchKernelGGL(k_probe_refine, dim3((unsigned)n), dim3(64), MVS_FRAME_LDS_BYTES, st, prm, n, in, out); return; }
+        return -1;
+    }
+    if (n > 0 && op == 2) {
+        if (sampler_narrow(prm)) { hipLaunchKernelGGL(k_probe_refine_ofs, dim3((unsigned)n), dim3(64), MVS_FRAME_LDS_BYTES, st, prm, n, in, out); return 1; }
+        hipLaunchKernelGGL(k_probe_refine, dim3((unsigned)n), dim3(64), MVS_FRAME_LDS_BYTES, st, prm, n, in, out);
+        return 0;
+    }
     if (n > 0) hipLaunchKernelGGL(k_probe, dim3((unsigned)n), dim3(64), mvsk_sweep_lds_bytes(prm), st, prm, op, n, in, in_f, out, out_f, out_i);
-}
+    return -1;
+}
diff --git a/mvskit_amd/csrc/mvs_types.h b/mvskit_amd/csrc/mvs_types.h
--- a/mvskit_amd/csrc/mvs_types.h
+++ b/mvskit_amd/csrc/mvs_types.h
@@ -47,8 +47,9 @@
     const uint8_t* mask;
     int32_t gw, gh;
     int32_t cell_base;
-    int32_t pad;
+    uint32_t img_off[MVS_MAXLEV];
 };
+static_assert(sizeof(DView) % 8 == 0, "DView is an array element with 8-byte members");
 
 struct DParams {
     int32_t nviews, level, csize, wsize, wsz, minImageNum, tau, cap, max_propag, depth, enable_check, view_propagation;
@@ -75,6 +76,7 @@
     const float4* geo;
     const uint8_t* geo_ref;
     const unsigned long long* dpgrid;
+    const uint8_t* pyr32;
 };
 
 #ifndef MVS_COUNTER_SLOTS
diff --git a/mvskit_amd/engine.py b/mvskit_amd/engine.py
--- a/mvskit_amd/engine.py
+++ b/mvskit_amd/engine.py
@@ -28,6 +28,7 @@
     "mvs_default_seed_points", "mvs_engine_seed_points", "mvs_engine_seed_points_hypotheses", "mvs_engine_depth_ranges",
     "mvs_default_maps_config", "mvs_engine_render_maps", "mvs_engine_fused_points",
     "mvs_engine_tsdf", "mvs_engine_extract_mesh", "mvs_engine_mesh", "mvs_engine_sweep_pairs", "mvs_engine_sweep_repeats", "mvs_engine_sweep_kernels",
+    "mvs_engine_sampler_launches",
     "mvs_default_mesh_colouring", "mvs_engine_mesh_normals", "mvs_engine_mesh_colours",
     "mvs_default_mesh_pruning", "mvs_default_mesh_smoothing", "mvs_engine_mesh_components", "mvs_engine_mesh_prune", "mvs_engine_mesh_smooth",
     "mvs_default_mesh_decimation", "mvs_engine_mesh_decimate",
@@ -210,6 +211,8 @@
         L.mvs_engine_sweep_repeats.argtypes = [vp, C.POINTER(C.c_int64)]
     if hasattr(L, "mvs_engine_sweep_kernels"):
         L.mvs_engine_sweep_kernels.argtypes = [vp, C.POINTER(C.c_int64)]
+    if hasattr(L, "mvs_engine_sampler_launches"):
+        L.mvs_engine_sampler_launches.argtypes = [vp, C.POINTER(C.c_int64)]
     if hasattr(L, "mvs_engine_tsdf"):
         L.mvs_engine_tsdf.argtypes = [vp, C.POINTER(MapsConfig), C.POINTER(Volume), vp, vp]
         L.mvs_engine_extract_mesh.argtypes = [vp, C.POINTER(Volume), vp, vp, C.c_int64, vp, C.c_int64, vp, C.POINTER(C.c_int64), C.POINTER(C.c_int64)]
@@ -678,6 +681,13 @@
         out = (C.c_int64 * 2)()
         self._check(self.L.mvs_engine_sweep_kernels(self.h, out))
         return dict(zip(self.SWEEP_KERNEL_KEYS, (int(x) for x in out)))
+
+    SAMPLER_LAUNCH_KEYS = ("sweep_wide", "sweep_narrow", "refine_wide", "refine_narrow")
+
+    def sampler_launches(self):
+        out = (C.c_int64 * 4)()
+        self._check(self.L.mvs_engine_sampler_launches(self.h, out))
+        return dict(zip(self.SAMPLER_LAUNCH_KEYS, (int(x) for x in out)))
 
     def depth_normal_map(self, view, kind):
         gw, gh = self.grid_dims(view)
```

Result: faster. 33.35 million, median of 6 (+2.2%).
